# leopard-ai/betty

Measured on AMD Instinct MI355X. Metric: hypergradient-steps/sec (CG K=20, 10M inner params), higher is better.
Workload: dtype f32

## Files before the change

betty_amd/_native.py:

```python
from __future__ import annotations

import ctypes
import os
from ctypes import POINTER, c_char_p, c_double, c_float, c_int, c_int32, c_int64, c_size_t, c_void_p

_HERE = os.path.dirname(os.path.abspath(__file__))
LIB_PATH = os.environ.get("BHG_LIB") or os.path.join(_HERE, "csrc", "libbhg.so")
AB_LIB_PATH = os.environ.get("BHG_AB_LIB") or os.path.join(_HERE, "csrc", "libbhg_ab.so")

BHG_CHUNK_ELEMS = 4096
BHG_FLAT_ALIGN = 64
BHG_CG_AUTO, BHG_CG_STREAM, BHG_CG_RESIDENT = 0, 1, 2
BHG_CG_GLOBAL_CHAIN, BHG_CG_GLOBAL_UPDATE, BHG_CG_GLOBAL_DOTS = 0, 1, 2
BHG_CG_FX_BEGIN, BHG_CG_FX_CHAIN, BHG_CG_FX_GRAM, BHG_CG_FX_END = 0, 1, 2, 3


class NativeLibraryError(RuntimeError):
    """libbhg.so is missing or a call into it failed."""


class Chunk(ctypes.Structure):

    _fields_ = [
        ("flat_off", c_int64),
        ("src_off", c_int64),
        ("tensor", c_int32),
        ("len", c_int32),
    ]


BHG_MLP_MAX_LAYERS = 32


class Mlp(ctypes.Structure):

    _fields_ = [
        ("L", c_int32),
        ("B", c_int32),
        ("Bp", c_int32),
        ("dims", c_int32 * (BHG_MLP_MAX_LAYERS + 1)),
        ("W", c_void_p * BHG_MLP_MAX_LAYERS),
        ("h", c_void_p * BHG_MLP_MAX_LAYERS),
        ("mask", c_void_p * BHG_MLP_MAX_LAYERS),
        ("delta", c_void_p * BHG_MLP_MAX_LAYERS),
        ("prob", c_void_p),
        ("sd", c_void_p),
        ("Rh", c_void_p * BHG_MLP_MAX_LAYERS),
        ("Rd", c_void_p * BHG_MLP_MAX_LAYERS),
        ("partial", c_void_p),
        ("partial_floats", c_size_t),
        ("ridge2", c_float),
        ("prepacked", c_int32),
    ]


_PP = POINTER(c_void_p)
_CH = c_void_p

SYMBOLS = {
    "bhg_version": (c_int, []),
    "bhg_last_error": (c_char_p, []),
    "bhg_layout_flat_size": (c_int64, [POINTER(c_int64), c_int]),
    "bhg_layout_num_chunks": (c_int64, [POINTER(c_int64), c_int]),
    "bhg_layout_build": (c_int, [POINTER(c_int64), c_int, POINTER(c_int64), POINTER(Chunk)]),
    "bhg_workspace_bytes": (c_size_t, [c_int]),
    "bhg_flatten": (c_int, [_PP, c_int, _CH, c_int, c_void_p, c_float, c_void_p, c_void_p]),
    "bhg_scatter": (c_int, [c_void_p, _PP, c_int, _CH, c_int, c_float, c_void_p, c_void_p]),
    "bhg_neumann_init": (c_int, [_PP, c_int, _CH, c_int, c_void_p, c_void_p, c_void_p, c_void_p]),
    "bhg_neumann_step": (
        c_int,
        [_PP, c_int, _CH, c_int, c_void_p, c_void_p, c_float, c_float, c_float, c_void_p, c_void_p],
    ),
    "bhg_cg_init": (c_int, [_PP, c_int, _CH, c_int, c_void_p, c_void_p, c_void_p, c_void_p, c_void_p]),
    "bhg_cg_init_masked": (c_int, [_PP, c_int, _CH, c_int, c_void_p, c_void_p, c_void_p, ctypes.c_uint64, c_void_p, c_void_p]),
    "bhg_cg_step": (
        c_int,
        [_PP, c_int, _CH, c_int, c_void_p, c_void_p, c_void_p, c_float, c_int, c_float, c_float, c_int, c_void_p, c_void_p],
    ),
    "bhg_cg_phase": (
        c_int,
        [c_int, _PP, c_int, _CH, c_int, c_void_p, c_void_p, c_void_p, c_float, c_int, c_float, c_float, c_void_p, c_void_p],
    ),
    "bhg_cg_partials_dev": (c_void_p, [c_void_p, c_int, c_int]),
    "bhg_cg_partials_count": (c_int, []),
    "bhg_cg_resident_capacity_chunks": (c_int, []),
    "bhg_cg_resident_ok": (c_int, []),
    "bhg_cg_resident_usable": (c_int, [c_int]),
    "bhg_cg_scalars_dev": (c_void_p, [c_void_p]),
    "bhg_cg_timeout_flag_dev": (c_void_p, [c_void_p]),
    "bhg_scale_flat": (c_int, [c_void_p, c_int64, c_float, c_void_p]),
    "bhg_darts_eps": (c_int, [_PP, c_int, _CH, c_int, c_double, c_void_p, c_void_p, c_void_p, c_void_p]),
    "bhg_axpy_multi": (c_int, [_PP, _PP, c_int, _CH, c_int, c_void_p, c_float, c_void_p, c_void_p]),
    "bhg_fd_perturb": (c_int, [_PP, c_void_p, _PP, c_int, _CH, c_int, c_void_p, c_float, c_void_p, c_void_p]),
    "bhg_cg_step_fd": (
        c_int,
        [_PP, _PP, c_void_p, c_int, _CH, c_int, c_void_p, c_void_p, c_void_p, c_float, c_int, c_float, c_float, c_int, c_void_p, c_void_p],
    ),
    "bhg_neumann_step_fd": (
        c_int,
        [_PP, _PP, c_void_p, c_int, _CH, c_int, c_void_p, c_void_p, c_float, c_float, c_float, c_void_p, c_void_p],
    ),
    "bhg_sama_adam_precondition": (
        c_int,
        [_PP, _PP, _PP, _PP, c_int, _CH, c_int, c_void_p, c_double, c_double, c_double, c_double, c_void_p, c_void_p],
    ),
    "bhg_debug_set": (c_int, [c_char_p, c_int]),
    "bhg_debug_unset": (c_int, [c_char_p]),
    "bhg_debug_reset": (None, []),
    "bhg_debug_key_count": (c_int, []),
    "bhg_debug_key_name": (c_char_p, [c_int]),
    "bhg_is_ab_build": (c_int, []),
    "bhg_timing_enable": (c_int, [c_int]),
    "bhg_timing_read": (c_int, [c_int, POINTER(c_double), POINTER(c_int)]),
    "bhg_logreg_prepare": (c_int, [c_void_p, c_void_p, c_void_p, c_int, c_int, c_void_p]),
    "bhg_logreg_tmp_floats": (c_size_t, [c_int, c_int]),
    "bhg_logreg_hvp": (
        c_int,
        [c_void_p, c_void_p, c_void_p, c_void_p, c_void_p, c_void_p, c_int, c_int, c_void_p],
    ),
    "bhg_mlp_partial_floats": (c_size_t, [POINTER(Mlp)]),
    "bhg_mlp_hvp": (c_int, [POINTER(Mlp), _PP, _PP, c_void_p]),
    "bhg_mlp_hvp_mode": (c_int, [POINTER(Mlp), _PP, _PP, c_int, c_void_p]),
    "bhg_mlp_supports_native_prepare": (c_int, [POINTER(Mlp)]),
    "bhg_mlp_forward": (c_int, [POINTER(Mlp), _PP, c_void_p, c_void_p, c_void_p]),
    "bhg_mlp_backward": (c_int, [POINTER(Mlp), c_void_p, c_void_p]),
    "bhg_mlp_mixed_coeff": (c_int, [POINTER(Mlp), _PP, c_void_p, c_void_p, c_void_p]),
    "bhg_mlp_supports_fused_solve": (c_int, [POINTER(Mlp)]),
    "bhg_mlp_fused_ws_bytes": (c_size_t, [POINTER(Mlp)]),
    "bhg_mlp_cg_solve": (
        c_int,
        [POINTER(Mlp), c_void_p, c_void_p, c_void_p, POINTER(c_int64), _CH, c_int, c_int, c_float, c_float, c_void_p,
         c_void_p, c_size_t, c_void_p],
    ),
    "bhg_mlp_cg_state_mask": (ctypes.c_uint64, [POINTER(Mlp), c_int]),
    "bhg_mlp_cg_solve_rhs": (
        c_int,
        [POINTER(Mlp), c_void_p, c_void_p, c_void_p, POINTER(c_int64), _CH, c_int, c_int, c_float, c_float, c_void_p,
         c_void_p, c_size_t, _PP, c_void_p],
    ),
    "bhg_mlp_cg_global_phase": (
        c_int,
        [POINTER(Mlp), c_void_p, c_void_p, c_void_p, POINTER(c_int64), _CH, c_int, c_int, c_int, c_int, c_int, c_void_p, c_float,
         c_float, c_void_p, c_void_p, c_size_t, c_void_p],
    ),
    "bhg_mlp_fx_supported": (c_int, [POINTER(Mlp), c_int]),
    "bhg_mlp_fx_ws_bytes": (c_size_t, [POINTER(Mlp), c_int]),
    "bhg_mlp_fx_const_floats": (c_size_t, [POINTER(Mlp)]),
    "bhg_mlp_fx_slab_floats": (c_size_t, [POINTER(Mlp)]),
    "bhg_mlp_fx_scal_doubles": (c_size_t, [POINTER(Mlp)]),
    "bhg_mlp_cg_fx_phase": (
        c_int,
        [POINTER(Mlp), _PP, c_int, c_int, c_int, c_int, c_int, c_void_p, c_void_p, c_void_p, c_float, c_float, c_void_p, c_size_t,
         c_void_p, c_size_t, c_void_p],
    ),
    "bhg_mlp_neumann_fx_phase": (
        c_int,
        [POINTER(Mlp), _PP, c_int, c_int, c_int, c_int, c_int, c_void_p, c_void_p, c_void_p, c_float, c_float, c_void_p, c_size_t,
         c_void_p, c_size_t, c_void_p],
    ),
    "bhg_mlp_cg_mixed_coeff": (c_int, [POINTER(Mlp), c_void_p, c_void_p, c_float, c_void_p, c_size_t, c_void_p]),
    "bhg_mlp_timeout_flag_dev": (c_void_p, [POINTER(Mlp), c_void_p]),
    "bhg_mlp_stage_batch": (c_int, [POINTER(Mlp), c_void_p, c_void_p, c_void_p, c_void_p]),
    "bhg_mlp_supports_packed_prepare": (c_int, [POINTER(Mlp)]),
    "bhg_mlp_forward_packed": (c_int, [POINTER(Mlp), _PP, c_void_p, c_void_p, c_void_p, c_size_t, c_void_p]),
    "bhg_mlp_backward_packed": (c_int, [POINTER(Mlp), c_void_p, c_void_p, c_size_t, c_void_p]),
    "bhg_mwn_max_hidden": (c_int, []),
    "bhg_mlp_fd_ws_bytes": (c_size_t, [POINTER(c_int), c_int, c_int]),
    "bhg_mlp_fd_forward": (
        c_int,
        [c_void_p, c_void_p, c_int, POINTER(c_int), c_int, _PP, _PP, c_void_p, c_int, c_void_p, c_void_p, c_void_p, c_size_t, c_void_p],
    ),
    "bhg_mwn_fd_vjp": (
        c_int,
        [c_void_p, c_void_p, c_int, c_void_p, c_void_p, c_void_p, c_void_p, c_int, c_void_p, c_int, c_void_p, c_void_p, c_void_p, c_void_p,
         c_void_p],
    ),
    "bhg_quad_fd": (c_int, [_PP, _PP, _PP, c_int, _CH, c_int, c_void_p, c_float, c_int, c_int, c_int, c_void_p]),
    "bhg_mwn_forward": (c_int, [c_void_p, c_int, c_void_p, c_void_p, c_void_p, c_void_p, c_int, c_void_p, c_void_p, c_void_p]),
    "bhg_mwn_backward": (
        c_int,
        [c_void_p, c_void_p, c_int, c_void_p, c_void_p, c_void_p, c_void_p, c_int, c_float, c_void_p, c_void_p, c_void_p, c_void_p, c_void_p],
    ),
    "bhg_mlp_neumann_solve": (
        c_int,
        [POINTER(Mlp), c_void_p, c_void_p, c_void_p, POINTER(c_int64), c_int, c_float, c_float, c_void_p, c_size_t, POINTER(c_int), c_void_p],
    ),
    "bhg_mlp_wsk_launches": (c_int64, []),
    "bhg_mlp_hoist_launches": (c_int64, []),
    "bhg_mlp_proj_iterations": (c_int64, []),
    "bhg_mlp_lin_launches": (c_int64, []),
    "bhg_mlp_neumann_mixed_coeff": (c_int, [POINTER(Mlp), _PP, c_void_p, c_void_p, c_float, c_int, c_int, c_void_p, c_size_t, c_void_p]),
    "bhg_mlp_plan_describe": (c_int, [POINTER(Mlp), c_int, c_int, ctypes.c_char_p, c_size_t]),
    "bhg_copy2d": (c_int, [c_void_p, c_int64, c_void_p, c_int64, c_int64, c_int64, c_void_p]),
    "bhg_bn_ws_bytes": (c_size_t, [c_int]),
    "bhg_bn_backward_vjp": (
        c_int,
        [c_void_p, c_void_p, c_void_p, c_void_p, c_void_p, c_void_p, c_void_p, c_void_p, c_int, c_int, c_int, c_void_p, c_void_p, c_void_p,
         c_void_p, c_size_t, c_void_p],
    ),
}

_libs = {}
_current = [None]


_PY_ENV = {"BHG_LIB", "BHG_AB_LIB", "BHG_HVP_GRAPH", "BHG_ALL_RANKS_ON_GPU0"}
_warned_env = [False]


def _warn_legacy_env() -> None:
    if _warned_env[0]:
        return
    _warned_env[0] = True
    stale = sorted(k for k in os.environ if k.startswith("BHG_") and k not in _PY_ENV)
    if stale:
        import warnings

        warnings.warn("betty_amd: environment variable(s) " + ", ".join(stale) + " are IGNORED — libbhg reads no environment variable. "
                      "Measurement arms are selected with betty_amd._native.use_ab() + debug_set(key, int) (bench.py --debug KEY=INT) "
                      "on the measurement build libbhg_ab.so.", RuntimeWarning, stacklevel=3)


def _bind(path: str) -> ctypes.CDLL:
    lib = _libs.get(path)
    if lib is not None:
        return lib
    _warn_legacy_env()
    if not os.path.exists(path):
        raise NativeLibraryError(
            f"{path} not found: the HIP extension has not been built. Run "
            "`python -c 'import __graft_entry__ as g; g.build()'` or `make -C betty_amd/csrc`. "
            "betty_amd has no CPU fallback."
        )
    lib = ctypes.CDLL(path)
    for name, (restype, argtypes) in SYMBOLS.items():
        try:
            fn = getattr(lib, name)
        except AttributeError as exc:
            raise NativeLibraryError(f"{path} does not export {name}") from exc
        fn.restype = restype
        fn.argtypes = argtypes
    _libs[path] = lib
    return lib


def load() -> ctypes.CDLL:
    return _bind(_current[0] or LIB_PATH)


def current_lib_path() -> str:
    return _current[0] or LIB_PATH


def is_ab() -> bool:
    return bool(load().bhg_is_ab_build())


def use_ab(on: bool = True) -> None:
    if on:
        _bind(AB_LIB_PATH)
        _current[0] = AB_LIB_PATH
    else:
        _current[0] = None


def check(rc: int, what: str) -> None:
    if rc != 0:
        msg = load().bhg_last_error()
        raise NativeLibraryError(f"{what} failed with code {rc}: {msg.decode() if msg else ''}")


def _debug_key(key: str) -> bytes:
    k = key.strip()
    if k.upper().startswith("BHG_"):
        k = k[4:]
    return k.lower().encode()


def debug_set(key: str, value) -> None:
    lib = load()
    if value is not None and not lib.bhg_is_ab_build():
        raise NativeLibraryError(f"bhg_debug_set({key}): the product libbhg.so carries no measurement arm — call "
                                 "betty_amd._native.use_ab() first (libbhg_ab.so; the `bhg_debug` fixture and `bench.py --debug` do)")
    if value is None:
        check(lib.bhg_debug_unset(_debug_key(key)), f"bhg_debug_unset({key})")
    else:
        check(lib.bhg_debug_set(_debug_key(key), int(value)), f"bhg_debug_set({key})")


def debug_reset() -> None:
    load().bhg_debug_reset()


def debug_keys():
    lib = load()
    return [lib.bhg_debug_key_name(i).decode() for i in range(lib.bhg_debug_key_count())]


def ptr_array(ptrs):
    arr = (c_void_p * len(ptrs))(*ptrs)
    return ctypes.cast(arr, _PP), arr


def plan_describe(dims, B: int, algo: str = "cg", keep_solution: bool = False) -> dict:
    lib = load()
    d = Mlp()
    d.L, d.B, d.Bp = len(dims) - 1, int(B), (int(B) + 127) // 128 * 128
    for i, v in enumerate(dims):
        d.dims[i] = int(v)
    buf = ctypes.create_string_buffer(2048)
    check(lib.bhg_mlp_plan_describe(ctypes.byref(d), {"cg": 0, "neumann": 1}[algo], 1 if keep_solution else 0, buf, 2048), "bhg_mlp_plan_describe")
    out, text = {}, buf.value.decode()
    import re

    for key, quoted, plain in re.findall(r'(\w+)=(?:"([^"]*)"|(\S+))', text):
        val = quoted if quoted else plain
        out[key] = int(val) if re.fullmatch(r"-?\d+", val) else val
    return out
```

betty_amd/csrc/bhg_common.hpp:

```cpp
#pragma once
#include <hip/hip_runtime.h>
#include <stdint.h>
#include <stddef.h>
#include <stdio.h>
#include <string.h>

#include "bhg.h"

namespace bhg {

constexpr int kThreads = 256;
constexpr int kWaves = kThreads / 64;
constexpr int kChunk = BHG_CHUNK_ELEMS;
constexpr int kVecPerThread = kChunk / (kThreads * 4);
constexpr int kMaxBlocks = 1024;
constexpr int kInlineT = 32;
constexpr int kWriterT = 448;

constexpr size_t kWsScal = 0;
constexpr size_t kWsPartP = 128;
constexpr size_t kWsPartR = kWsPartP + 8 * kMaxBlocks;
constexpr size_t kWsBarrier = kWsPartR + 16 * kMaxBlocks;
constexpr size_t kWsTables = kWsBarrier + 256;
inline size_t ws_bytes(int T) {
  size_t b = kWsTables + 4 * sizeof(void*) * (size_t)(T > 0 ? T : 0);
  return (b + 255) & ~(size_t)255;
}

enum { S_RR_OLD = 0, S_PHP = 1, S_ALPHA = 2, S_RR_NEW = 3, S_BETA = 4, S_PP = 5 , S_ALPHA_RING = 10 ,
       S_NPART0 = 8  };

#define BHG_DBG_KEYS(X)                                                                                                      \
  X(mlp_wsk) X(mlp_wsk_maxk) X(mlp_wsk_depth) X(mlp_wsk_lds) X(wsl_depth) X(no_nt_slabs) X(gemm_no_xpose) X(mlp_no_fast)      \
  X(mlp_tn) X(split_target) X(split_cap) X(mlp_no_head) X(gram_ksplit) X(gram_kchunk) X(proj_graw_split) X(mlp_proj)         \
  X(mlp_hoist) X(hoist_wgs) X(proj_step_alone) X(mlp_no_side) X(mlp_no_fuse) X(mlp_no_outer_all) X(neumann_side)             \
  X(hoist_staged_mink) X(proj_alpha_alone) X(proj_small_alone) X(outer_order_by_work) X(outer_no_pre) X(outer_stagger)       \
  X(mlp_no_fused_solve) X(cg_eager_p) X(cg_x_every_iter) X(neumann_p_every_iter) X(head_no_prefetch) X(cg_spin_limit)        \
  X(packed_chain) X(packed_depth) X(packed_gram) X(proj_max_ratio) X(proj_ws_cap_mb) X(alpha_in_hoist) X(graw_v2) X(wskp_ragged) X(pstep_v2) X(pstep_unroll) X(rnew_in_graw) X(graw_cols) X(lin_first) X(lin_prio) X(lin_nub) X(lin_order) X(lin_update_next) X(lin_withhold_beta) X(neumann_vnew) X(cg_rhs_direct) X(packed_prepare) X(lin_deep) X(graw_kloop) X(lin_update_in_head) X(xcd_pairs) X(headu_head_first) X(fx_ksplit)
enum DbgKey : int {
#define BHG_DBG_ENUM(n) DBG_##n,
  BHG_DBG_KEYS(BHG_DBG_ENUM)
#undef BHG_DBG_ENUM
  DBG_COUNT
};
constexpr int kDbgUnset = INT32_MIN;
#ifdef BHG_AB
extern int g_dbg[DBG_COUNT];
inline bool dbg_is_set(DbgKey k) { return g_dbg[k] != kDbgUnset; }
inline int dbg(DbgKey k, int dflt) { return g_dbg[k] == kDbgUnset ? dflt : g_dbg[k]; }
#else
constexpr bool dbg_is_set(DbgKey) { return false; }
constexpr int dbg(DbgKey, int dflt) { return dflt; }
#endif

constexpr int kStampKernels = 4, kStampBlocks = 4096, kStampSlots = 8;
#ifdef BHG_STAMPS
#ifdef __HIPCC__
#define BHG_STAMP(kid, slot)                                                                                            \
  do {                                                                                                                  \
    if (threadIdx.x == 0 && blockIdx.x < ::bhg::kStampBlocks) {                                                         \
      unsigned long long* sp_ = ::bhg::d_stamps;                                                                        \
      if (sp_) sp_[((kid) * ::bhg::kStampBlocks + blockIdx.x) * ::bhg::kStampSlots + (slot)] = wall_clock64();          \
    }                                                                                                                   \
  } while (0)
#endif
#else
#define BHG_STAMP(kid, slot) do { } while (0)
#endif

void set_error(const char* fmt, ...);
#define BHG_HIP_CHECK(expr)                                                        \
  do {                                                                             \
    hipError_t _e = (expr);                                                        \
    if (_e != hipSuccess) {                                                        \
      ::bhg::set_error("%s failed: %s (%s:%d)", #expr, hipGetErrorString(_e), __FILE__, \
                       __LINE__);                                                  \
      return BHG_ERR_HIP;                                                          \
    }                                                                              \
  } while (0)
#define BHG_REQUIRE(cond, msg)                                                     \
  do {                                                                             \
    if (!(cond)) {                                                                 \
      ::bhg::set_error("%s: %s", __func__, msg);                                   \
      return BHG_ERR_ARG;                                                          \
    }                                                                              \
  } while (0)

struct PtrTab {
  const void* const* dev;
  const void* inl[kInlineT];
};

int make_table(PtrTab* out, const void* const* host_ptrs, int T, void* ws, int slot,
               hipStream_t stream);

bool span_begin(int kind, hipEvent_t* a, hipEvent_t* b);

#ifdef __HIPCC__
__device__ __forceinline__ float* tab_ptr(const PtrTab& t, int i) {
  const void* p = t.dev ? t.dev[i] : t.inl[i];
  return (float*)p;
}

__device__ __forceinline__ float4 ld4(const float* __restrict__ base, int e, int len) {
  if (e + 4 <= len) return *reinterpret_cast<const float4*>(base + e);
  float4 r = make_float4(0.f, 0.f, 0.f, 0.f);
  if (e < len) r.x = base[e];
  if (e + 1 < len) r.y = base[e + 1];
  if (e + 2 < len) r.z = base[e + 2];
  return r;
}
__device__ __forceinline__ void st4(float* __restrict__ base, int e, int len, float4 v) {
  if (e + 4 <= len) {
    *reinterpret_cast<float4*>(base + e) = v;
    return;
  }
  if (e < len) base[e] = v.x;
  if (e + 1 < len) base[e + 1] = v.y;
  if (e + 2 < len) base[e + 2] = v.z;
}

template <int BYTES>
__device__ __forceinline__ void kernarg_warm() {
  typedef const __attribute__((address_space(4))) unsigned* KP;
  KP kp = (KP)__builtin_amdgcn_kernarg_segment_ptr();
  unsigned acc = 0;
#pragma unroll
  for (int o = 0; o < BYTES; o += 64) acc |= kp[o / 4];
  asm volatile("" ::"s"(acc));
}
template <int U>
__device__ __forceinline__ double sum_strided(const double* __restrict__ p, const int n, const int t, const int stride) {
  double acc = 0.0;
  for (int i0 = t; i0 < n; i0 += U * stride) {
    double v[U];
#pragma unroll
    for (int u = 0; u < U; ++u) {
      const int i = i0 + u * stride;
      v[u] = p[i < n ? i : n - 1];
    }
#pragma unroll
    for (int u = 0; u < U; ++u)
      if (i0 + u * stride < n) acc += v[u];
  }
  return acc;
}

template <int U>
struct StridedRegs { double v[U]; };
template <int U>
__device__ __forceinline__ void strided_load(StridedRegs<U>& r, const double* __restrict__ p, const int n, const int t, const int stride,
                                             const double* __restrict__ dummy) {
  const double* q = (p && n > 0) ? p : dummy;
  const int last = (p && n > 0) ? n - 1 : 0;
#pragma unroll
  for (int u = 0; u < U; ++u) {
    const int i = t + u * stride;
    r.v[u] = q[i < n && i <= last ? i : last];
  }
}
template <int U>
__device__ __forceinline__ double strided_sum(const StridedRegs<U>& r, const int n, const int t, const int stride) {
  double acc = 0.0;
#pragma unroll
  for (int u = 0; u < U; ++u)
    if (t + u * stride < n) acc += r.v[u];
  return acc;
}

template <int CTRL>
__device__ __forceinline__ double dpp_mov_f64(const double v) {
  const unsigned long long u = __builtin_bit_cast(unsigned long long, v);
  const unsigned lo = (unsigned)__builtin_amdgcn_mov_dpp((int)(unsigned)u, CTRL, 0xf, 0xf, true);
  const unsigned hi = (unsigned)__builtin_amdgcn_mov_dpp((int)(unsigned)(u >> 32), CTRL, 0xf, 0xf, true);
  return __builtin_bit_cast(double, ((unsigned long long)hi << 32) | (unsigned long long)lo);
}
__device__ __forceinline__ double readlane_f64(const double v, const int lane) {
  const unsigned long long u = __builtin_bit_cast(unsigned long long, v);
  const unsigned lo = (unsigned)__builtin_amdgcn_readlane((int)(unsigned)u, lane);
  const unsigned hi = (unsigned)__builtin_amdgcn_readlane((int)(unsigned)(u >> 32), lane);
  return __builtin_bit_cast(double, ((unsigned long long)hi << 32) | (unsigned long long)lo);
}
__device__ __forceinline__ double wave_sum(double v) {
  v += dpp_mov_f64<0xB1>(v);
  v += dpp_mov_f64<0x4E>(v);
  v += dpp_mov_f64<0x141>(v);
  v += dpp_mov_f64<0x140>(v);
  const double r0 = readlane_f64(v, 0), r1 = readlane_f64(v, 16), r2 = readlane_f64(v, 32), r3 = readlane_f64(v, 48);
  return (r0 + r1) + (r2 + r3);
}
template <int CTRL>
__device__ __forceinline__ float dpp_mov_f32(const float v) {
  return __builtin_bit_cast(float, __builtin_amdgcn_mov_dpp(__builtin_bit_cast(int, v), CTRL, 0xf, 0xf, true));
}
__device__ __forceinline__ float wave_sum_f32(float v) {
  v += dpp_mov_f32<0xB1>(v);
  v += dpp_mov_f32<0x4E>(v);
  v += dpp_mov_f32<0x141>(v);
  v += dpp_mov_f32<0x140>(v);
  const float r0 = __builtin_bit_cast(float, __builtin_amdgcn_readlane(__builtin_bit_cast(int, v), 0));
  const float r1 = __builtin_bit_cast(float, __builtin_amdgcn_readlane(__builtin_bit_cast(int, v), 16));
  const float r2 = __builtin_bit_cast(float, __builtin_amdgcn_readlane(__builtin_bit_cast(int, v), 32));
  const float r3 = __builtin_bit_cast(float, __builtin_amdgcn_readlane(__builtin_bit_cast(int, v), 48));
  return (r0 + r1) + (r2 + r3);
}
__device__ __forceinline__ void block_sum3(double& a, double& b, double& c, double* red) {
  const double wa = wave_sum(a), wb = wave_sum(b), wc = wave_sum(c);
  const int lane = threadIdx.x & 63, w = threadIdx.x >> 6;
  __syncthreads();
  if (lane == 0) { red[w] = wa; red[kWaves + w] = wb; red[2 * kWaves + w] = wc; }
  __syncthreads();
  double sa = 0.0, sb = 0.0, sc = 0.0;
#pragma unroll
  for (int i = 0; i < kWaves; ++i) { sa += red[i]; sb += red[kWaves + i]; sc += red[2 * kWaves + i]; }
  a = sa; b = sb; c = sc;
}
__device__ __forceinline__ double block_sum(double v, double* red) {
  v = wave_sum(v);
  const int lane = threadIdx.x & 63, w = threadIdx.x >> 6;
  __syncthreads();
  if (lane == 0) red[w] = v;
  __syncthreads();
  double s = 0.0;
#pragma unroll
  for (int i = 0; i < kWaves; ++i) s += red[i];
  return s;
}
__device__ __forceinline__ double sum_partials(const double* __restrict__ part, int n,
                                               double* red) {
  double a = 0.0;
  for (int i = threadIdx.x; i < n; i += kThreads) a += part[i];
  return block_sum(a, red);
}
#endif

}
```

betty_amd/csrc/bhg_mlp.hip:

```cpp
#include <stdlib.h>
#include <vector>


#include "bhg_common.hpp"

#ifdef BHG_STAMPS
namespace bhg { __device__ unsigned long long* d_stamps = nullptr; }
#endif

namespace bhg {
namespace {
#include "mlp/gemm.inc"

#include "mlp/outer.inc"

#include "mlp/scalars.inc"

#include "mlp/head.inc"

#include "mlp/wsk.inc"

#include "mlp/wskp.inc"

inline int wsk_mode(int chain_mode, int unfused_hint) {
  if (dbg_is_set(DBG_mlp_wsk)) return dbg(DBG_mlp_wsk, 0);
  if (chain_mode == FUSE_CG) return 2;
  if (chain_mode == FUSE_NEUMANN) return 3;
  return unfused_hint;
}
inline bool wsk_wanted(int mode, int pairs, int K) {
  if (mode == 1) return true;
  if (mode != 2 && mode != 3) return false;
  return pairs * K <= dbg(DBG_mlp_wsk_maxk, 1024);
}
inline int wsk_depth() {
  const int d = dbg(DBG_mlp_wsk_depth, 3);
  return d == 2 ? 2 : 3;
}
inline bool wsk_eligible(const WskArgs& a) {
  if (a.pairs < 1 || a.pairs > 2) return false;
  bool ok = a.M % 32 == 0 && a.N % 32 == 0 && a.K % 32 == 0 && a.K >= 32;
  for (int i = 0; i < a.pairs; ++i) ok = ok && (a.pr[i].lda & 3) == 0 && (a.pr[i].ldb & 3) == 0;
  return ok;
}
int64_t g_wsk_launches = 0;
int64_t g_hoist_launches = 0;
int64_t g_proj_iterations = 0;
int64_t g_lin_launches = 0;
template <int LB>
void launch_gemm_wsk(const WskArgs& a_in, hipStream_t st, bool staged = false) {
  WskArgs a = a_in;
  ++g_wsk_launches;
  a.ntm = a.M / 32;
  a.ntn = a.N / 32;
  bool bf = false;
  for (int i = 0; i < a.pairs; ++i) bf = bf || a.pr[i].mix != 0;
  const dim3 grid(a.ntm * a.ntn), block(64 * kWskWaves);
  const int d = wsk_depth();
  const bool force_staged = dbg(DBG_mlp_wsk_lds, 0) != 0;
  if ((staged || force_staged) && !bf) {
    const int lds = (int)(sizeof(float) * kWslWaveFloats * kWskWaves);
    static bool attr_done = false;
    if (!attr_done) {
      (void)hipFuncSetAttribute(reinterpret_cast<const void*>(k_gemm_wsk<LB, false, 2, true>), hipFuncAttributeMaxDynamicSharedMemorySize, lds);
      attr_done = true;
    }
#ifdef BHG_AB
    const int wsl_depth = dbg(DBG_wsl_depth, 2);
    if (wsl_depth == 3) {
      static bool attr3 = false;
      if (!attr3) {
        (void)hipFuncSetAttribute(reinterpret_cast<const void*>(k_gemm_wsk<LB, false, 3, true>), hipFuncAttributeMaxDynamicSharedMemorySize, lds);
        attr3 = true;
      }
      hipLaunchKernelGGL((k_gemm_wsk<LB, false, 3, true>), grid, block, lds, st, a);
      return;
    }
#endif
    hipLaunchKernelGGL((k_gemm_wsk<LB, false, 2, true>), grid, block, lds, st, a);
    return;
  }
#define BHG_WSK(BFV, DV) hipLaunchKernelGGL((k_gemm_wsk<LB, BFV, DV>), grid, block, 0, st, a)
  if (bf) {
    if (d == 2 || LB == LAYOUT_RC) BHG_WSK(true, 2); else BHG_WSK(true, LB == LAYOUT_RC ? 2 : 3);
  } else {
#ifdef BHG_AB
    if (d == 2) BHG_WSK(false, 2); else
#endif
    BHG_WSK(false, 3);
  }
#undef BHG_WSK
}

#ifdef BHG_AB
void launch_wsk_group(const WskGroupArgs& g, int blocks, hipStream_t st) {
  const int lds = (int)(sizeof(float) * kWslWaveFloats * kWskWaves);
  static bool attr_done = false;
  if (!attr_done) {
    (void)hipFuncSetAttribute(reinterpret_cast<const void*>(k_wsk_group<2>), hipFuncAttributeMaxDynamicSharedMemorySize, lds);
#ifdef BHG_AB
    (void)hipFuncSetAttribute(reinterpret_cast<const void*>(k_wsk_group<3>), hipFuncAttributeMaxDynamicSharedMemorySize, lds);
#endif
    attr_done = true;
  }
#ifdef BHG_AB
  const int wsl_depth = dbg(DBG_wsl_depth, 2);
  if (wsl_depth == 3) { hipLaunchKernelGGL(k_wsk_group<3>, dim3(blocks), dim3(64 * kWskWaves), lds, st, g); return; }
#endif
  hipLaunchKernelGGL(k_wsk_group<2>, dim3(blocks), dim3(64 * kWskWaves), lds, st, g);
}
#endif

int chip_cus() {
  static int cus[64];
  int dev = 0;
  if (hipGetDevice(&dev) != hipSuccess || dev < 0 || dev >= 64) { (void)hipGetLastError(); return 256; }
  if (cus[dev] > 0) return cus[dev];
  int n = 0;
  if (hipDeviceGetAttribute(&n, hipDeviceAttributeMultiprocessorCount, dev) != hipSuccess || n <= 0) { (void)hipGetLastError(); n = 256; }
  return cus[dev] = n;
}
inline void wskp_tiling(WskpProb* q, bool ragged) {
  q->nfull = q->RA / 32;
  q->nstrip = 0;
  q->pairs = dbg(DBG_xcd_pairs, 1);
  if (!ragged || q->raw || q->nsplit != 1 || q->RB % 64 != 0) return;
  int nf = q->B / 32, rem = q->B % 32;
  if (rem > 16) { ++nf; rem = 0; }
  if (nf == 0) return;
  q->nfull = nf;
  q->nstrip = rem > 0 ? q->RB / 64 : 0;
}
struct WskpBuilder {
  WskpArgs g{};
  int blk = 0;
  bool add(const WskpProb& q_in) {
    if (g.n >= kWskpMax) return false;
    g.p[g.n++] = q_in;
    return true;
  }
  void tile(bool ragged) {
    blk = 0;
    for (int i = 0; i < g.n; ++i) {
      WskpProb& q = g.p[i];
      wskp_tiling(&q, ragged);
      g.blk0[i] = blk;
      blk += (((q.nfull * (q.RB / 32) + q.nstrip) * q.nsplit) + 7) & ~7;
    }
  }
  void launch(hipStream_t st) {
    if (!g.n) return;
    const int mode = dbg(DBG_wskp_ragged, 1);
    tile(mode == 2);
    if (mode == 1 && blk > chip_cus()) tile(true);
    g.blk0[g.n] = blk;
    const int d = dbg(DBG_packed_depth, 2);
    bool riders = g.n <= 3;
    for (int i = 1; i < g.n && riders; ++i) {
      const WskpProb& r = g.p[i];
      riders = r.raw && r.nsplit == 1 && r.RA == g.p[0].RA && r.RB == g.p[0].RA && r.B == g.p[0].B && !r.bias && !r.mask && !r.addend &&
               !r.partT2 && r.nstrip == 0 && r.nfull == r.RA / 32;
    }
    if (riders) {
      WskpcArgs c{};
      c.a = g.p[0];
      c.na = g.n >= 2 ? g.blk0[1] : blk;
      if (g.n >= 2) { c.r0 = {g.p[1].Ap, g.p[1].Bq, g.p[1].out, g.p[1].outp, g.p[1].K, 0}; c.nr0 = (g.n == 3 ? g.blk0[2] : blk) - g.blk0[1]; }
      if (g.n == 3) c.r1 = {g.p[2].Ap, g.p[2].Bq, g.p[2].out, g.p[2].outp, g.p[2].K, 0};
#ifdef BHG_AB
      if (d != 2) hipLaunchKernelGGL(k_wskpc<3>, dim3(blk), dim3(64 * kWskpWaves), 0, st, c); else
#endif
      hipLaunchKernelGGL(k_wskpc<2>, dim3(blk), dim3(64 * kWskpWaves), 0, st, c);
    } else {
#ifdef BHG_AB
      if (d != 2) hipLaunchKernelGGL(k_wskp<3>, dim3(blk), dim3(64 * kWskpWaves), 0, st, g); else
#endif
      hipLaunchKernelGGL(k_wskp<2>, dim3(blk), dim3(64 * kWskpWaves), 0, st, g);
    }
    (void)d;
    g = WskpArgs{};
    blk = 0;
  }
};

template <int LA, int LB>
void launch_gemm(const GemmArgs& a_in, int tn, hipStream_t st) {
  GemmArgs a = a_in;
  const bool nt_slabs = dbg(DBG_no_nt_slabs, 0) == 0;
  a.nt_out = (nt_slabs && (a.splits > 1 || a.out_rows > 0)) ? 1 : 0;
  const bool xpose = dbg(DBG_gemm_no_xpose, 0) == 0;
  a.xpose_out = xpose ? 1 : 0;
  dim3 grid((a.N + tn - 1) / tn, (a.M + kTM - 1) / kTM, a.splits);
  bool fast = a.M % kTM == 0 && a.N % tn == 0 && a.K % kTK == 0;
  bool bf = false;
  for (int i = 0; i < a.pairs; ++i) {
    fast = fast && (a.pr[i].lda & 3) == 0 && (a.pr[i].ldb & 3) == 0;
    bf = bf || a.pr[i].mix != 0;
  }
  if (bf)
    for (int i = 0; i < a.pairs; ++i)
      if (!a.pr[i].mix) a.pr[i].B2 = a.pr[i].B;
  const bool no_fast = dbg(DBG_mlp_no_fast, 0) != 0;
  if (no_fast) fast = false;
#define BHG_GEMM(TNV, F, BFV) hipLaunchKernelGGL((k_gemm<LA, LB, TNV, F, BFV>), grid, dim3(256), 0, st, a)
#ifdef BHG_AB
  if (tn == 64) {
    if (bf) { if (fast) BHG_GEMM(64, true, true); else BHG_GEMM(64, false, true); }
    else    { if (fast) BHG_GEMM(64, true, false); else BHG_GEMM(64, false, false); }
  } else
#endif
  {
    if (bf) { if (fast) BHG_GEMM(32, true, true); else BHG_GEMM(32, false, true); }
    else    { if (fast) BHG_GEMM(32, true, false); else BHG_GEMM(32, false, false); }
  }
#undef BHG_GEMM
}
inline int skinny_tile_n() {
  const int tn = dbg(DBG_mlp_tn, 32);
  return tn == 64 ? 64 : 32;
}

void launch_reduce_mask(hipStream_t st, const float* part, int splits, int slab, const float* bias,
                        const float* mask, float* out, int rows, int N, int B, float* relu_mask_out = nullptr,
                        float* outp = nullptr) {
  if ((N & 3) == 0) {
    int blocks = (slab / 4 + 255) / 256;
    if (blocks > 2048) blocks = 2048;
    hipLaunchKernelGGL(k_reduce_mask<4>, dim3(blocks), dim3(256), 0, st, part, splits, slab, bias, mask, out, rows, N, B,
                       relu_mask_out, outp);
  } else {
    int blocks = (slab + 255) / 256;
    if (blocks > 2048) blocks = 2048;
    hipLaunchKernelGGL(k_reduce_mask<1>, dim3(blocks), dim3(256), 0, st, part, splits, slab, bias, mask, out, rows, N, B,
                       relu_mask_out, (float*)nullptr);
  }
}

int pick_splits(int tiles, int K, int pairs) {
  const int ksteps = (K + kTK - 1) / kTK;
  const int target = dbg(DBG_split_target, 768);
  int s = (target + tiles - 1) / tiles;
  if (s > ksteps) s = ksteps;
  const int cap = dbg(DBG_split_cap, 16);
  if (s > cap) s = cap;
  if (s < 1) s = 1;
  if (ksteps % s != 0) {
    for (int d = 1; d <= 2; ++d) {
      if (s - d >= 1 && ksteps % (s - d) == 0) { s -= d; break; }
      if (s + d <= cap && s + d <= ksteps && ksteps % (s + d) == 0) { s += d; break; }
    }
  }
  return s;
}

#include "mlp/recurrence.inc"

#include "mlp/proj.inc"

#include "mlp/graw.inc"

#include "mlp/pstep.inc"
#include "mlp/wskpl.inc"
#include "mlp/headu.inc"

void launch_wskpu(const WskpProb& q_in, const PstepArgs& ps, int nu, hipStream_t st) {
  WskpuArgs u{};
  WskpProb q = q_in;
  const int mode = dbg(DBG_wskp_ragged, 1);
  wskp_tiling(&q, mode == 2);
  int blk = (((q.nfull * (q.RB / 32) + q.nstrip) * q.nsplit) + 7) & ~7;
  if (mode == 1 && blk > chip_cus()) {
    wskp_tiling(&q, true);
    blk = (((q.nfull * (q.RB / 32) + q.nstrip) * q.nsplit) + 7) & ~7;
  }
  u.c.a = q; u.c.na = blk;
  u.nu = nu; u.ps = ps;
  hipLaunchKernelGGL((k_wskpu<2, 4>), dim3(nu + blk), dim3(64 * kWskpWaves), 0, st, u);
}

struct SideState {
  hipStream_t side;
  hipEvent_t ev_rd[BHG_MLP_MAX_LAYERS];
  hipEvent_t ev_join;
};
int side_state(SideState** out) {
  static SideState per_device[64];
  int dev = 0;
  BHG_HIP_CHECK(hipGetDevice(&dev));
  BHG_REQUIRE(dev >= 0 && dev < 64, "device index out of range");
  SideState& ss = per_device[dev];
  if (!ss.side) {
    BHG_HIP_CHECK(hipStreamCreateWithFlags(&ss.side, hipStreamNonBlocking));
    const unsigned fl = hipEventDisableTiming | hipEventDisableSystemFence;
    for (int i = 0; i < BHG_MLP_MAX_LAYERS; ++i) BHG_HIP_CHECK(hipEventCreateWithFlags(&ss.ev_rd[i], fl));
    BHG_HIP_CHECK(hipEventCreateWithFlags(&ss.ev_join, fl));
#define BHG_OUTER_LDS(F, M) \
    BHG_HIP_CHECK(hipFuncSetAttribute(reinterpret_cast<const void*>(k_outer<F, M>), hipFuncAttributeMaxDynamicSharedMemorySize, 96 * 1024))
    BHG_OUTER_LDS(true, FUSE_NONE); BHG_OUTER_LDS(false, FUSE_NONE);
    BHG_OUTER_LDS(true, FUSE_CG); BHG_OUTER_LDS(false, FUSE_CG);
    BHG_OUTER_LDS(true, FUSE_NEUMANN); BHG_OUTER_LDS(false, FUSE_NEUMANN);
#undef BHG_OUTER_LDS
#ifdef BHG_AB
    BHG_HIP_CHECK(hipFuncSetAttribute(reinterpret_cast<const void*>(k_outer_all<FUSE_CG, false>), hipFuncAttributeMaxDynamicSharedMemorySize, 96 * 1024));
    BHG_HIP_CHECK(hipFuncSetAttribute(reinterpret_cast<const void*>(k_outer_all<FUSE_NEUMANN, false>), hipFuncAttributeMaxDynamicSharedMemorySize, 96 * 1024));
#endif
    BHG_HIP_CHECK(hipFuncSetAttribute(reinterpret_cast<const void*>(k_outer_all<FUSE_CG, true>), hipFuncAttributeMaxDynamicSharedMemorySize, 96 * 1024));
    BHG_HIP_CHECK(hipFuncSetAttribute(reinterpret_cast<const void*>(k_outer_all<FUSE_NEUMANN, true>), hipFuncAttributeMaxDynamicSharedMemorySize, 96 * 1024));
// ... 1265 lines not shown
  c->scal = reinterpret_cast<double*>(wsb + kWsScal);
  c->partR0 = reinterpret_cast<const double*>(wsb + kWsPartR);
  c->n_init = n_chunks < kMaxBlocks ? n_chunks : kMaxBlocks;
  for (int i = 0; i < 2 * m->L; ++i) c->dir[i] = p + starts[i];
  c->pgrid = n_chunks < kMaxBlocks ? n_chunks : kMaxBlocks;
  const bool eager = dbg(DBG_cg_eager_p, 0) != 0;
  c->lazy = global || !eager;
  BetaArgs& ba = c->ba;
  ba = BetaArgs{};
  int small_total = 0;
  {
    const bool head = use_head(m);
    ba.stride = c->w.nRR; ba.n = c->w.nRR; ba.scal = c->scal; ba.r = r; ba.p = p;
    for (int l = 0; l < m->L; ++l) {
      ba.off[ba.nt] = starts[2 * l + 1]; ba.len[ba.nt] = m->dims[l + 1]; small_total += ba.len[ba.nt]; ++ba.nt;
    }
    if (head) {
      ba.off[ba.nt] = starts[2 * (m->L - 1)]; ba.len[ba.nt] = m->dims[m->L] * m->dims[m->L - 1]; small_total += ba.len[ba.nt]; ++ba.nt;
    }
  }
  c->bgrid = small_total > 0 ? (small_total + kThreads - 1) / kThreads : 1;
  c->hplan.ok = false;
  if (c->lazy && hoist_mode() != 0) hoist_plan(m, &c->hplan);
  c->hoist = c->lazy && c->hplan.ok;
  c->proj_level = (!c->hoist || !c->hplan.proj_ok || proj_mode() == 0 || global) ? 0 : ((proj_mode() == 9 || x) ? 1 : 2);
  c->lin = c->proj_level == 2 && c->hplan.lin_ok && packed_chain_on(c->w) && dbg(DBG_packed_gram, 1) != 0 && dbg(DBG_graw_v2, 1) != 0 &&
           graw_batch_ok(m->Bp) && dbg(DBG_proj_small_alone, 0) == 0 && dbg(DBG_alpha_in_hoist, 1) != 0 && dbg(DBG_rnew_in_graw, 1) != 0 &&
           c->ba.nt <= 16 && proj_step_merged() && dbg(DBG_pstep_v2, 1) != 0 && dbg(DBG_lin_first, 1) != 0;
  c->lin_head = c->lin && m->L == 4 && dbg(DBG_lin_update_next, 1) != 0 && dbg(DBG_lin_update_in_head, 1) != 0 && dbg(DBG_lin_nub, 0) == 0 &&
                m->dims[m->L] <= 12 && m->dims[m->L - 1] <= 512 && dbg(DBG_head_no_prefetch, 0) == 0;
}
static int cg_iteration(CgCtx* c, int k, int gphase, double* php, double inv_world, hipStream_t st) {
  const bhg_mlp* m = c->m;
  FusedWs& w = c->w;
  const int K = c->K;
  const bool lazy = c->lazy, hoist = c->hoist;
  hipEvent_t ta, tb, tc, td;
  const bool timed = gphase == 0 && span_begin(BHG_TIMING_MLP_HVP, &ta, &tb);
  const bool timed_it = gphase == 0 && span_begin(BHG_TIMING_MLP_CG_ITER, &tc, &td);
  if (timed_it) BHG_HIP_CHECK(hipEventRecord(tc, st));
  if (lazy && k > 0 && gphase != 2) {
    c->ba.part = w.partRR[k & 1];
    if (!hoist || c->proj_level == 1) hipLaunchKernelGGL(k_cg_beta, dim3(c->bgrid), dim3(kThreads), 0, st, c->ba);
  }
  if (timed) BHG_HIP_CHECK(hipEventRecord(ta, st));
  ChainMode cm{};
  cm.mode = FUSE_CG;
  cm.fa = c->r; cm.fb = c->x; cm.fd = c->p; cm.starts = c->starts;
  cm.shift = c->shift; cm.cg_alpha = c->cg_alpha;
  cm.apply_out = k == K - 1; cm.out_scale = -c->cg_alpha;
  cm.ws = &w; cm.scal = c->scal;
  cm.partRR_old = c->partR0;
  cm.nRR_old = k == 0 ? c->n_init : 0;
  cm.partPP = k == 0 ? c->partR0 : w.partPP;
  cm.nPP = k == 0 ? c->n_init : (lazy ? 0 : c->pgrid);
  cm.partRR_new = w.partRR[(k + 1) & 1];
  cm.lazy = lazy;
  const bool x_every = dbg(DBG_cg_x_every_iter, 0) != 0;
  cm.x_mode = (lazy && !x_every) ? ((k & 1) ? 2 : (k + 1 < K ? 1 : 0)) : 0;
  if (!c->x) cm.x_mode = 1;
  cm.skip_outputs = (!c->x && k == K - 1) ? 1 : 0;
  cm.first = k == 0;
  cm.kpar = k & 1;
  cm.hoist = hoist ? &c->hplan : nullptr;
  cm.beta = &c->ba; cm.beta_blocks = c->bgrid;
  cm.proj = c->proj_level;
  cm.gphase = gphase; cm.php = php; cm.inv_world = inv_world;
  cm.second = k == 1;
  if (c->proj_level == 2 && proj_step_merged())
    c->dir[1] = k == 0 ? static_cast<const void*>(c->p + c->starts[1]) : static_cast<const void*>(w.pb0[k & 1]);
  if (c->lin) c->dir[3] = k == 0 ? static_cast<const void*>(c->p + c->starts[3]) : static_cast<const void*>(w.pb1[k & 1]);
  cm.lin = c->lin ? 1 : 0;
  cm.lin_head = c->lin_head ? 1 : 0;
  cm.rhs = c->rhs;
  if (int rc = run_chain(m, c->dir, cm, st)) return rc;
  if (timed) BHG_HIP_CHECK(hipEventRecord(tb, st));
#ifdef BHG_AB
  if (!lazy && k + 1 < K)
    hipLaunchKernelGGL(k_cg_pdir, dim3(c->pgrid), dim3(kThreads), 0, st, c->chunks_dev, c->n_chunks, (const float*)c->r, c->p,
                       (const double*)w.partRR[(k + 1) & 1], w.nRR, w.partPP, c->scal);
#endif
  if (timed_it) BHG_HIP_CHECK(hipEventRecord(td, st));
  return BHG_OK;
}

int bhg_mlp_cg_solve(const bhg_mlp* m, float* x, float* r, float* p, const int64_t* starts,
                     const bhg_chunk* chunks_dev, int n_chunks, int K, float cg_alpha, float hvp_shift, void* ws,
                     void* fws, size_t fws_bytes, void* stream) {
  return bhg_mlp_cg_solve_rhs(m, x, r, p, starts, chunks_dev, n_chunks, K, cg_alpha, hvp_shift, ws, fws, fws_bytes, nullptr, stream);
}

unsigned long long bhg_mlp_cg_state_mask(const bhg_mlp* m, int has_x) {
  if (!m || m->L < 1 || m->L > BHG_MLP_MAX_LAYERS || 2 * m->L > 64 || has_x || !bhg_mlp_supports_fused_solve(m)) return ~0ull;
  HoistPlan hp;
  hp.ok = false;
  if (dbg(DBG_cg_eager_p, 0) == 0 && hoist_mode() != 0) hoist_plan(m, &hp);
  const bool level2 = hp.ok && hp.proj_ok && proj_mode() != 0 && proj_mode() != 9;
  if (!level2 || dbg(DBG_cg_rhs_direct, 1) == 0) return ~0ull;
  unsigned long long mask = 0ull;
  for (int l = 0; l < m->L; ++l) mask |= 1ull << (2 * l + 1);
  mask |= 1ull << (2 * (m->L - 1));
  return mask;
}

int bhg_mlp_cg_solve_rhs(const bhg_mlp* m, float* x, float* r, float* p, const int64_t* starts,
                         const bhg_chunk* chunks_dev, int n_chunks, int K, float cg_alpha, float hvp_shift, void* ws,
                         void* fws, size_t fws_bytes, const void* const* rhs, void* stream) {
  if (int rc = solve_common_checks(m, starts, fws, fws_bytes)) return rc;
  BHG_REQUIRE(r && p && ws && chunks_dev, "NULL argument");
  BHG_REQUIRE(K >= 0 && n_chunks > 0, "bad size");
  if (K == 0) return BHG_OK;
  hipStream_t st = static_cast<hipStream_t>(stream);
  CgCtx c;
  cg_ctx_init(&c, m, x, r, p, starts, chunks_dev, n_chunks, K, cg_alpha, hvp_shift, ws, fws, false);
  BHG_REQUIRE(!rhs || c.proj_level == 2, "rhs names the right-hand side for the FULLY PROJECTED solver only (see bhg_mlp_cg_state_mask)");
  if (rhs)
    for (int l = 0; l + 1 < m->L; ++l) BHG_REQUIRE(rhs[2 * l] && ((uintptr_t)rhs[2 * l] & 15) == 0, "rhs tensors must be 16-byte aligned device pointers");
  c.rhs = rhs;
  if (c.hoist && packed_chain_on(c.w) && !m->prepacked)
    if (int rc = pack_operands(m, c.w, st)) return rc;
  for (int k = 0; k < K; ++k)
    if (int rc = cg_iteration(&c, k, 0, nullptr, 1.0, st)) return rc;
  BHG_HIP_CHECK(hipGetLastError());
  return BHG_OK;
}

int bhg_mlp_cg_global_phase(const bhg_mlp* m, float* x, float* r, float* p, const int64_t* starts, const bhg_chunk* chunks_dev,
                            int n_chunks, int k, int K, int phase, int world, double* php, float cg_alpha, float hvp_shift,
                            void* ws, void* fws, size_t fws_bytes, void* stream) {
  if (int rc = solve_common_checks(m, starts, fws, fws_bytes)) return rc;
  BHG_REQUIRE(r && p && ws && chunks_dev && php, "NULL argument");
  BHG_REQUIRE(K > 0 && k >= 0 && k < K && n_chunks > 0 && world >= 1, "bad size");
  BHG_REQUIRE(phase == BHG_CG_GLOBAL_CHAIN || phase == BHG_CG_GLOBAL_UPDATE || phase == BHG_CG_GLOBAL_DOTS, "unknown phase");
  hipStream_t st = static_cast<hipStream_t>(stream);
  CgCtx c;
  cg_ctx_init(&c, m, x, r, p, starts, chunks_dev, n_chunks, K, cg_alpha, hvp_shift, ws, fws, true);
  if (phase == BHG_CG_GLOBAL_DOTS) {
    BHG_REQUIRE(k + 1 < K, "the last iteration has no direction update");
    int grid = n_chunks < c.w.nRR ? n_chunks : c.w.nRR;
    if (grid > kMaxBlocks) grid = kMaxBlocks;
    hipLaunchKernelGGL(k_cg_global_dots, dim3(grid), dim3(kThreads), 0, st, chunks_dev, n_chunks, (const float*)r, (const float*)p,
                       c.w.partRR[(k + 1) & 1], c.w.nRR, c.w.nRR);
    BHG_HIP_CHECK(hipGetLastError());
    return BHG_OK;
  }
  if (k == 0 && phase == BHG_CG_GLOBAL_CHAIN && c.hoist && packed_chain_on(c.w) && !m->prepacked)
    if (int rc = pack_operands(m, c.w, st)) return rc;
  if (int rc = cg_iteration(&c, k, phase == BHG_CG_GLOBAL_CHAIN ? 1 : 2, php, 1.0 / (double)world, st)) return rc;
  BHG_HIP_CHECK(hipGetLastError());
  return BHG_OK;
}

int bhg_mlp_fx_supported(const bhg_mlp* m, int world) {
  if (!m || m->L < 1 || m->L > BHG_MLP_MAX_LAYERS || m->Bp <= 0 || m->Bp % kTM != 0 || !bhg_mlp_supports_fused_solve(m)) return 0;
  FxPlan fp;
  fx_plan(m, world, &fp);
  return fp.ok && dbg(DBG_packed_chain, 1) != 0 ? 1 : 0;
}
size_t bhg_mlp_fx_ws_bytes(const bhg_mlp* m, int world) {
  if (!bhg_mlp_fx_supported(m, world)) return 0;
  FxPlan fp; fx_plan(m, world, &fp);
  FxWs x; fx_carve(m, fp, nullptr, &x);
  return x.bytes;
}
size_t bhg_mlp_fx_const_floats(const bhg_mlp* m) {
  if (!bhg_mlp_fx_supported(m, 1)) return 0;
  FxPlan fp; fx_plan(m, 1, &fp);
  return fp.const_floats;
}
size_t bhg_mlp_fx_slab_floats(const bhg_mlp* m) {
  if (!bhg_mlp_fx_supported(m, 1)) return 0;
  FxPlan fp; fx_plan(m, 1, &fp);
  return fp.slab_floats;
}
size_t bhg_mlp_fx_scal_doubles(const bhg_mlp* m) {
  if (!bhg_mlp_fx_supported(m, 1)) return 0;
  FxPlan fp; fx_plan(m, 1, &fp);
  return fp.scal_doubles;
}
static int fx_phase(int algo, const bhg_mlp* m, const void* const* rhs, int k, int K, int phase, int world, int rank, float* const_all,
                    float* slab_all, double* scal_all, float alpha, float hvp_shift, void* fws, size_t fws_bytes, void* xws, size_t xws_bytes,
                    void* stream) {
  if (int rc = check_mlp(m)) return rc;
  const bool neumann = algo == 1;
  BHG_REQUIRE(world >= 1 && rank >= 0 && rank < world, "bad world size / rank");
  BHG_REQUIRE(bhg_mlp_fx_supported(m, world), "this network does not take the factor-exchange form (bhg_mlp_fx_supported)");
  BHG_REQUIRE(phase == BHG_CG_FX_BEGIN || phase == BHG_CG_FX_CHAIN || phase == BHG_CG_FX_GRAM || phase == BHG_CG_FX_END, "unknown phase");
  BHG_REQUIRE(K > 0 && k >= 0 && (k < K || (neumann && k == K && (phase == BHG_CG_FX_CHAIN || phase == BHG_CG_FX_END))), "bad iteration index");
  BHG_REQUIRE(const_all && slab_all && scal_all && fws && xws, "NULL argument");
  BHG_REQUIRE(m->partial && m->partial_floats >= bhg_mlp_partial_floats(m), "split-K scratch too small");
  BHG_REQUIRE(fws_bytes >= bhg_mlp_fused_ws_bytes(m), "fused workspace too small");
  BHG_REQUIRE(xws_bytes >= bhg_mlp_fx_ws_bytes(m, world), "factor-exchange workspace too small");
  hipStream_t st = static_cast<hipStream_t>(stream);
  FxPlan fp;
  fx_plan(m, world, &fp);
  FusedWs w;
  carve_fused_ws(m, fws, &w);
  FxWs x;
  fx_carve(m, fp, xws, &x);
  const bhg_mlp ml = fx_local(m, fp, slab_all, rank);
  double* scal_mine = scal_all + (size_t)rank * fp.scal_doubles;
  if (phase == BHG_CG_FX_BEGIN) {
    BHG_REQUIRE(k == 0, "BEGIN belongs to iteration 0");
    return fx_begin(m, fp, const_all, rank, st);
  }
  if (phase == BHG_CG_FX_CHAIN) {
    if (k == 0) {
      BHG_REQUIRE(rhs, "iteration 0 reads the right-hand side");
      for (int l = 0; l + 1 < m->L; ++l) BHG_REQUIRE(rhs[2 * l] && ((uintptr_t)rhs[2 * l] & 15) == 0, "rhs tensors must be 16-byte aligned device pointers");
      for (int i = 0; i < 2 * m->L; ++i) BHG_REQUIRE(rhs[i], "rhs holds 2 L device pointers");
      if (int rc = fx_first(m, &ml, fp, w, x, rhs, const_all, rank, st, neumann)) return rc;
    } else {
      if (int rc = fx_step(&ml, fp, w, x, scal_all, k - 1, false, alpha, hvp_shift, st, neumann)) return rc;
    }
    return fx_chain(&ml, fp, w, x, k & 1, st, neumann && k == K);
  }
  if (phase == BHG_CG_FX_GRAM) {
    BHG_REQUIRE(k < K, "GRAM belongs to iterations 0 .. K-1");
    return fx_gram(&ml, fp, w, x, slab_all, const_all, scal_mine, k & 1, hvp_shift, st);
  }
  BHG_REQUIRE(k == (neumann ? K : K - 1), "END belongs to the last iteration");
  return fx_step(&ml, fp, w, x, scal_all, k, true, alpha, hvp_shift, st, neumann);
}
int bhg_mlp_cg_fx_phase(const bhg_mlp* m, const void* const* rhs, int k, int K, int phase, int world, int rank, float* const_all,
                        float* slab_all, double* scal_all, float cg_alpha, float hvp_shift, void* fws, size_t fws_bytes, void* xws,
                        size_t xws_bytes, void* stream) {
  return fx_phase(0, m, rhs, k, K, phase, world, rank, const_all, slab_all, scal_all, cg_alpha, hvp_shift, fws, fws_bytes, xws, xws_bytes, stream);
}
int bhg_mlp_neumann_fx_phase(const bhg_mlp* m, const void* const* rhs, int k, int K, int phase, int world, int rank, float* const_all,
                             float* slab_all, double* scal_all, float alpha, float hvp_shift, void* fws, size_t fws_bytes, void* xws,
                             size_t xws_bytes, void* stream) {
  return fx_phase(1, m, rhs, k, K, phase, world, rank, const_all, slab_all, scal_all, alpha, hvp_shift, fws, fws_bytes, xws, xws_bytes, stream);
}

int bhg_mlp_neumann_solve(const bhg_mlp* m, float* v0, float* v1, float* p, const int64_t* starts, int K, float alpha,
                          float hvp_shift, void* fws, size_t fws_bytes, int* projected_out, void* stream) {
  if (int rc = solve_common_checks(m, starts, fws, fws_bytes)) return rc;
  BHG_REQUIRE(v0 && v1, "NULL argument");
  BHG_REQUIRE(K >= 0, "bad size");
  BHG_REQUIRE(p || use_head(m), "the accumulator-free Neumann solver needs the narrow-head kernels");
  hipStream_t st = static_cast<hipStream_t>(stream);
  FusedWs w;
  carve_fused_ws(m, fws, &w);
  HoistPlan hplan;
  hplan.ok = false;
  const bool want_proj = !p && K > 0 && proj_mode() != 0 && hoist_mode() != 0;
  if (hoist_mode() == 2 || want_proj) hoist_plan(m, &hplan);
  const bool proj = want_proj && hplan.ok && hplan.proj_ok && use_head(m);
  if (projected_out) *projected_out = proj ? 1 : 0;
  if (hplan.ok && K > 0 && packed_chain_on(w) && !m->prepacked)
    if (int rc = pack_operands(m, w, st)) return rc;
  for (int k = 0; k < K; ++k) {
    float* vin = (k & 1) ? v1 : v0;
    float* vout = (k & 1) ? v0 : v1;
    const void* dir[2 * BHG_MLP_MAX_LAYERS];
    for (int i = 0; i < 2 * m->L; ++i) dir[i] = vin + starts[i];
    hipEvent_t ta, tb;
    const bool timed = span_begin(BHG_TIMING_MLP_HVP, &ta, &tb);
    if (timed) BHG_HIP_CHECK(hipEventRecord(ta, st));
    ChainMode cm{};
    cm.mode = FUSE_NEUMANN;
    cm.fa = vout; cm.fb = p; cm.fd = vin; cm.starts = starts;
    cm.alpha = alpha; cm.shift = hvp_shift;
    cm.apply_out = k == K - 1; cm.out_scale = -alpha;
    const bool p_every = dbg(DBG_neumann_p_every_iter, 0) != 0;
    cm.x_mode = p_every ? 0 : ((k & 1) ? 2 : (k + 1 < K ? 1 : 0));
    cm.first = k == 0;
    if (!p) { cm.x_mode = 1; cm.rzx_acc = w.rzx; }
    cm.ws = &w;
    cm.hoist = hplan.ok ? &hplan : nullptr;
    cm.proj = proj ? 1 : 0;
    cm.nk = k;
    if (int rc = run_chain(m, dir, cm, st)) return rc;
    if (timed) BHG_HIP_CHECK(hipEventRecord(tb, st));
  }
  if (proj) {
    float* vin = (K & 1) ? v1 : v0;
    const void* dir[2 * BHG_MLP_MAX_LAYERS];
    for (int i = 0; i < 2 * m->L; ++i) dir[i] = vin + starts[i];
    ChainMode cm{};
    cm.mode = FUSE_NEUMANN;
    cm.fa = (K & 1) ? v0 : v1; cm.fb = nullptr; cm.fd = vin; cm.starts = starts;
    cm.alpha = alpha; cm.shift = hvp_shift;
    cm.x_mode = 1; cm.rzx_acc = w.rzx; cm.first = 0;
    cm.ws = &w; cm.hoist = &hplan; cm.proj = 1; cm.stop_after_head = 1; cm.nk = K;
    if (int rc = run_chain(m, dir, cm, st)) return rc;
  }
  return BHG_OK;
}

int bhg_mlp_cg_mixed_coeff(const bhg_mlp* m, const int64_t* labels, float* coeff, float cg_alpha, void* fws,
                           size_t fws_bytes, void* stream) {
  if (int rc = check_mlp(m)) return rc;
  BHG_REQUIRE(labels && coeff && fws, "NULL argument");
  BHG_REQUIRE(fws_bytes >= bhg_mlp_fused_ws_bytes(m), "fused workspace too small");
  FusedWs w;
  carve_fused_ws(m, fws, &w);
  hipLaunchKernelGGL(k_coeff_from_rzx, dim3((m->Bp + kThreads - 1) / kThreads), dim3(kThreads), 0, static_cast<hipStream_t>(stream),
                     (const double*)w.rzx, m->prob, labels, coeff, m->Bp, m->dims[m->L], m->B, -cg_alpha, 0.f);
  BHG_HIP_CHECK(hipGetLastError());
  return BHG_OK;
}

static int check_head_problem(const bhg_mlp* m) {
  BHG_REQUIRE(m, "NULL descriptor");
  BHG_REQUIRE(m->L >= 1 && m->L <= BHG_MLP_MAX_LAYERS, "unsupported layer count");
  BHG_REQUIRE(m->Bp > 0 && m->Bp % kTM == 0 && m->B >= 1 && m->B <= m->Bp, "Bp must be a multiple of 128 rows >= B");
  BHG_REQUIRE(m->partial && m->partial_floats >= bhg_mlp_partial_floats(m), "split-K scratch too small");
  return BHG_OK;
}
static bool narrow_head(const bhg_mlp* m) { return m->dims[m->L] <= kSmallC && (m->dims[m->L - 1] & 3) == 0; }

int bhg_mlp_supports_native_prepare(const bhg_mlp* m) {
  return m && m->L >= 1 && m->L <= BHG_MLP_MAX_LAYERS && m->Bp > 0 && m->Bp % kTM == 0;
}

}
namespace bhg {
namespace {
__global__ __launch_bounds__(kThreads) void k_softmax_ce_rows(float* __restrict__ z, const int64_t* __restrict__ labels,
                                                              float* __restrict__ ce, int C, int B) {
  __shared__ double red[kWaves];
  __shared__ float redf[kWaves];
  const int b = blockIdx.x, t = threadIdx.x;
  float* row = z + (int64_t)b * C;
  if (b >= B) {
    for (int c = t; c < C; c += kThreads) row[c] = 0.f;
    if (t == 0) ce[b] = 0.f;
    return;
  }
  float mx = -INFINITY;
  for (int c = t; c < C; c += kThreads) mx = fmaxf(mx, row[c]);
  for (int o = 32; o > 0; o >>= 1) mx = fmaxf(mx, __shfl_xor(mx, o));
  if ((t & 63) == 0) redf[t >> 6] = mx;
  __syncthreads();
  mx = redf[0];
  for (int w = 1; w < kWaves; ++w) mx = fmaxf(mx, redf[w]);
  double s = 0.0;
  for (int c = t; c < C; c += kThreads) s += (double)expf(row[c] - mx);
  s = block_sum(s, red);
  const float lse = mx + logf((float)s);
  const float zy = row[(int)labels[b]];
  __syncthreads();
  for (int c = t; c < C; c += kThreads) row[c] = expf(row[c] - lse);
  if (t == 0) ce[b] = lse - zy;
}
__global__ __launch_bounds__(kThreads) void k_coeff_rows(const float* __restrict__ prob, const float* __restrict__ rz,
                                                         const int64_t* __restrict__ labels, float* __restrict__ coeff, int C, int B) {
  __shared__ double red[kWaves];
  const int b = blockIdx.x, t = threadIdx.x;
  if (b >= B) { if (t == 0) coeff[b] = 0.f; return; }
  const int y = (int)labels[b];
  double s = 0.0;
  for (int c = t; c < C; c += kThreads) s += (double)((prob[(int64_t)b * C + c] - (c == y ? 1.f : 0.f)) * rz[(int64_t)b * C + c]);
  s = block_sum(s, red);
  if (t == 0) coeff[b] = (float)(s / (double)B);
}
}
}
using namespace bhg;
extern "C" {

int bhg_mlp_forward(const bhg_mlp* m, const void* const* bias, const int64_t* labels, float* ce, void* stream) {
  if (int rc = check_head_problem(m)) return rc;
  BHG_REQUIRE(bias && labels && ce, "NULL argument");
  hipStream_t st = static_cast<hipStream_t>(stream);
  const int L = m->L, Bp = m->Bp, B = m->B;
  for (int l = 0; l < L; ++l) {
    const int K = m->dims[l], N = m->dims[l + 1];
    const float* b = static_cast<const float*>(bias[l]);
    if (l == L - 1 && narrow_head(m)) {
      launch_head_forward(st, Bp, nullptr, m->h[l], m->W[l] , m->W[l], b, nullptr, nullptr,
                          const_cast<float*>(m->prob), K, N, B, HEAD_LOGITS, labels, ce, nullptr, nullptr, nullptr);
      break;
    }
    GemmArgs a{};
    a.pr[0] = {m->h[l], m->W[l], K, K};
    a.pairs = 1;
    a.M = Bp; a.N = N; a.K = K;
    const int tn = skinny_tile_n();
    a.splits = pick_splits((N + tn - 1) / tn, K, 1);
    a.out = m->partial; a.ldo = N; a.out_rows = Bp;
    launch_gemm<LAYOUT_KC, LAYOUT_KC>(a, tn, st);
    if (l == L - 1) {
      launch_reduce_mask(st, m->partial, a.splits, Bp * N, b, nullptr, const_cast<float*>(m->prob), Bp, N, B);
      hipLaunchKernelGGL(k_softmax_ce_rows, dim3(Bp), dim3(kThreads), 0, st, const_cast<float*>(m->prob), labels, ce, N, B);
      break;
    }
    launch_reduce_mask(st, m->partial, a.splits, Bp * N, b, nullptr, const_cast<float*>(m->h[l + 1]), Bp, N, B,
                       const_cast<float*>(m->mask[l]));
  }
  BHG_HIP_CHECK(hipGetLastError());
  return BHG_OK;
}

int bhg_mlp_backward(const bhg_mlp* m, const int64_t* labels, void* stream) {
  if (int rc = check_head_problem(m)) return rc;
  BHG_REQUIRE(labels, "NULL argument");
  hipStream_t st = static_cast<hipStream_t>(stream);
  const int L = m->L, Bp = m->Bp, B = m->B;
  const int C = m->dims[L];
  hipLaunchKernelGGL(k_delta_top, dim3((Bp * C + 255) / 256), dim3(256), 0, st, m->prob, m->sd, labels,
                     const_cast<float*>(m->delta[L - 1]), Bp, C, B);
  for (int l = L - 1; l >= 1; --l) {
    const int K = m->dims[l + 1], N = m->dims[l];
    if (l == L - 1 && narrow_head(m)) {
      const int blocks = (Bp * (N / 4) + 255) / 256;
      hipLaunchKernelGGL(k_head_backward, dim3(blocks), dim3(256), 0, st, (const float*)nullptr, m->delta[l], m->W[l],
                         (const float*)nullptr, m->mask[l - 1], const_cast<float*>(m->delta[l - 1]), N, K, B, Bp);
      continue;
    }
    GemmArgs a{};
    a.pr[0] = {m->delta[l], m->W[l], K, N};
    a.pairs = 1;
    a.M = Bp; a.N = N; a.K = K;
    const int tn = skinny_tile_n();
    a.splits = pick_splits((N + tn - 1) / tn, K, 1);
    a.out = m->partial; a.ldo = N; a.out_rows = Bp;
    launch_gemm<LAYOUT_KC, LAYOUT_RC>(a, tn, st);
    launch_reduce_mask(st, m->partial, a.splits, Bp * N, nullptr, m->mask[l - 1], const_cast<float*>(m->delta[l - 1]), Bp,
                       N, B);
  }
  BHG_HIP_CHECK(hipGetLastError());
  return BHG_OK;
}

int bhg_mlp_supports_packed_prepare(const bhg_mlp* m) {
  if (!bhg_mlp_supports_native_prepare(m) || !bhg_mlp_supports_fused_solve(m) || dbg(DBG_packed_prepare, 1) == 0) return 0;
  HoistPlan hp;
  hoist_plan(m, &hp);
  return hp.ok && dbg(DBG_packed_chain, 1) != 0 ? 1 : 0;
}

int bhg_mlp_forward_packed(const bhg_mlp* m, const void* const* bias, const int64_t* labels, float* ce, void* fws, size_t fws_bytes,
                           void* stream) {
  if (int rc = check_head_problem(m)) return rc;
  BHG_REQUIRE(narrow_head(m), "the packed once-per-step passes need a narrow classifier head (<= 256 classes, feature width % 4 == 0)");
  BHG_REQUIRE(bias && labels && ce && fws, "NULL argument");
  BHG_REQUIRE(bhg_mlp_supports_packed_prepare(m), "this network does not take the packed form (bhg_mlp_supports_packed_prepare)");
  BHG_REQUIRE(fws_bytes >= bhg_mlp_fused_ws_bytes(m), "fused workspace too small");
  hipStream_t st = static_cast<hipStream_t>(stream);
  const int L = m->L, Bp = m->Bp, B = m->B;
  FusedWs w;
  carve_fused_ws(m, fws, &w);
  if (int rc = pack_operands(m, w, st, true)) return rc;
  {
    const int K = m->dims[0], N = m->dims[1];
    GemmArgs a{};
    a.pr[0] = {m->h[0], m->W[0], K, K};
    a.pairs = 1;
    a.M = Bp; a.N = N; a.K = K;
    const int tn = skinny_tile_n();
    a.splits = pick_splits((N + tn - 1) / tn, K, 1);
    a.out = m->partial; a.ldo = N; a.out_rows = Bp;
    launch_gemm<LAYOUT_KC, LAYOUT_KC>(a, tn, st);
    launch_reduce_mask(st, m->partial, a.splits, Bp * N, static_cast<const float*>(bias[0]), nullptr, const_cast<float*>(m->h[1]), Bp, N, B,
                       const_cast<float*>(m->mask[0]), w.hpk[1]);
  }
  for (int l = 1; l + 1 < L; ++l) {
    WskpfArgs f{};
    WskpProb& q = f.a;
    q.Ap = w.hpk[l]; q.Bq = w.Wf[l]; q.RA = Bp; q.RB = m->dims[l + 1]; q.K = m->dims[l]; q.B = B; q.nsplit = 1;
    q.bias = static_cast<const float*>(bias[l]);
    q.out = const_cast<float*>(m->h[l + 1]);
    q.outp = l + 2 < L ? w.hpk[l + 1] : nullptr;
    f.relu_mask = const_cast<float*>(m->mask[l]);
    wskp_tiling(&q, false);
    const int blk = q.nfull * (q.RB / 32) + q.nstrip;
    hipLaunchKernelGGL(k_wskpf<2>, dim3(blk), dim3(64 * kWskpWaves), 0, st, f);
  }
  launch_head_forward(st, Bp, nullptr, m->h[L - 1], m->W[L - 1] , m->W[L - 1], static_cast<const float*>(bias[L - 1]),
                      nullptr, nullptr, const_cast<float*>(m->prob), m->dims[L - 1], m->dims[L], B, HEAD_LOGITS, labels, ce, nullptr,
                      nullptr, nullptr);
  BHG_HIP_CHECK(hipGetLastError());
  return BHG_OK;
}

int bhg_mlp_backward_packed(const bhg_mlp* m, const int64_t* labels, void* fws, size_t fws_bytes, void* stream) {
  if (int rc = check_head_problem(m)) return rc;
  BHG_REQUIRE(narrow_head(m), "the packed once-per-step passes need a narrow classifier head (<= 256 classes, feature width % 4 == 0)");
  BHG_REQUIRE(labels && fws, "NULL argument");
  BHG_REQUIRE(bhg_mlp_supports_packed_prepare(m), "this network does not take the packed form (bhg_mlp_supports_packed_prepare)");
  BHG_REQUIRE(fws_bytes >= bhg_mlp_fused_ws_bytes(m), "fused workspace too small");
  hipStream_t st = static_cast<hipStream_t>(stream);
  const int L = m->L, Bp = m->Bp, B = m->B;
  const int C = m->dims[L];
  FusedWs w;
  carve_fused_ws(m, fws, &w);
  hipLaunchKernelGGL(k_delta_top, dim3((Bp * C + 255) / 256), dim3(256), 0, st, m->prob, m->sd, labels,
                     const_cast<float*>(m->delta[L - 1]), Bp, C, B);
  {
    const int l = L - 1, K = m->dims[l + 1], N = m->dims[l];
    const int blocks = (Bp * (N / 4) + 255) / 256;
    hipLaunchKernelGGL(k_head_backward, dim3(blocks), dim3(256), 0, st, (const float*)nullptr, m->delta[l], m->W[l],
                       (const float*)nullptr, m->mask[l - 1], const_cast<float*>(m->delta[l - 1]), N, K, B, Bp, w.dpk[l - 1]);
  }
  for (int l = L - 2; l >= 1; --l) {
    WskpBuilder wb;
    WskpProb q{};
    q.Ap = w.dpk[l]; q.Bq = w.Wb[l]; q.RA = Bp; q.RB = m->dims[l]; q.K = m->dims[l + 1]; q.B = B; q.nsplit = 1;
    q.mask = m->mask[l - 1]; q.out = const_cast<float*>(m->delta[l - 1]);
    q.outp = l >= 2 ? w.dpk[l - 1] : nullptr;
    wb.add(q);
    wb.launch(st);
  }
  BHG_HIP_CHECK(hipGetLastError());
  return BHG_OK;
}

__global__ __launch_bounds__(256) void k_stage_batch(const float* __restrict__ x, const int64_t* __restrict__ y, float* __restrict__ h0,
                                                     int64_t* __restrict__ labels, int64_t n4, int B) {
  for (int64_t i = (int64_t)blockIdx.x * 256 + threadIdx.x; i < n4; i += (int64_t)gridDim.x * 256)
    reinterpret_cast<float4*>(h0)[i] = reinterpret_cast<const float4*>(x)[i];
  if (blockIdx.x == 0)
    for (int b = threadIdx.x; b < B; b += 256) labels[b] = y[b];
}
int bhg_mlp_stage_batch(const bhg_mlp* m, const float* x, const int64_t* y, int64_t* labels, void* stream) {
  if (int rc = check_mlp(m)) return rc;
  BHG_REQUIRE(x && y && labels && m->h[0], "NULL argument");
  BHG_REQUIRE((m->dims[0] & 3) == 0 && ((uintptr_t)x & 15) == 0, "the input batch must be 16-byte aligned with a width that is a multiple of 4");
  const int64_t n4 = (int64_t)m->B * m->dims[0] / 4;
  int blocks = (int)((n4 + 255) / 256);
  if (blocks > 2048) blocks = 2048;
  if (blocks < 1) blocks = 1;
  hipLaunchKernelGGL(k_stage_batch, dim3(blocks), dim3(256), 0, static_cast<hipStream_t>(stream), x, y, const_cast<float*>(m->h[0]), labels, n4, m->B);
  BHG_HIP_CHECK(hipGetLastError());
  return BHG_OK;
}

int bhg_mlp_mixed_coeff(const bhg_mlp* m, const void* const* dir, const int64_t* labels, float* coeff, void* stream) {
  if (int rc = check_head_problem(m)) return rc;
  BHG_REQUIRE(dir && labels && coeff, "NULL argument");
  hipStream_t st = static_cast<hipStream_t>(stream);
  const int L = m->L, Bp = m->Bp, B = m->B;
  for (int l = 0; l < L; ++l) {
    const int K = m->dims[l], N = m->dims[l + 1];
    const float* V = static_cast<const float*>(dir[2 * l]);
    const float* c = static_cast<const float*>(dir[2 * l + 1]);
    if (l == L - 1 && narrow_head(m)) {
      launch_head_forward(st, Bp, l > 0 ? (const float*)m->Rh[l - 1] : nullptr, m->h[l], m->W[l], V, c, m->prob, nullptr,
                          nullptr, K, N, B, HEAD_COEFF, labels, coeff, nullptr, nullptr, nullptr);
      break;
    }
    GemmArgs a{};
    a.pr[0] = {m->h[l], V, K, K};
    a.pairs = 1;
    if (l > 0) { a.pr[1] = {m->Rh[l - 1], m->W[l], K, K}; a.pairs = 2; }
    a.M = Bp; a.N = N; a.K = K;
    const int tn = skinny_tile_n();
    a.splits = pick_splits((N + tn - 1) / tn, K, a.pairs);
    a.out = m->partial; a.ldo = N; a.out_rows = Bp;
    launch_gemm<LAYOUT_KC, LAYOUT_KC>(a, tn, st);
    if (l == L - 1) {
      launch_reduce_mask(st, m->partial, a.splits, Bp * N, c, nullptr, m->Rd[l], Bp, N, B);
      hipLaunchKernelGGL(k_coeff_rows, dim3(Bp), dim3(kThreads), 0, st, m->prob, (const float*)m->Rd[l], labels, coeff, N, B);
      break;
    }
    launch_reduce_mask(st, m->partial, a.splits, Bp * N, c, m->mask[l], m->Rh[l], Bp, N, B);
  }
  BHG_HIP_CHECK(hipGetLastError());
  return BHG_OK;
}

int bhg_mlp_plan_describe(const bhg_mlp* m, int algo, int keep_solution, char* buf, size_t buf_bytes) {
  if (int rc = check_mlp(m)) return rc;
  BHG_REQUIRE(buf && buf_bytes >= 64, "output buffer too small");
  BHG_REQUIRE(algo == 0 || algo == 1, "algo: 0 = cg, 1 = neumann");
  const int L = m->L;
  const bool fused = bhg_mlp_supports_fused_solve(m) != 0;
  HoistPlan hp;
  hoist_plan(m, &hp);
  const char* form = "unfused";
  int hoist = 0, proj_level = 0, lin = 0, lin_head = 0, upd_first = 0;
  const char* closing = "k_outer_all";
  if (fused) {
    int64_t numel[2 * BHG_MLP_MAX_LAYERS], starts[2 * BHG_MLP_MAX_LAYERS];
    for (int l = 0; l < L; ++l) { numel[2 * l] = (int64_t)m->dims[l] * m->dims[l + 1]; numel[2 * l + 1] = m->dims[l + 1]; }
    const int64_t nch = bhg_layout_num_chunks(numel, 2 * L);
    std::vector<bhg_chunk> chunks((size_t)(nch > 0 ? nch : 1));
    if (int rc = bhg_layout_build(numel, 2 * L, starts, chunks.data())) return rc;
    float* const fake = reinterpret_cast<float*>((uintptr_t)1 << 30);
    if (algo == 0) {
      static CgCtx c;
      cg_ctx_init(&c, m, keep_solution ? fake : nullptr, fake, fake, starts, nullptr, (int)nch, 2, 1.f, 0.f, fake, fake, false);
      hoist = c.hoist ? 1 : 0; proj_level = c.proj_level; lin = c.lin ? 1 : 0; lin_head = c.lin_head ? 1 : 0;
      upd_first = (c.lin && L > 4) ? 1 : 0;
      form = !c.lazy ? "classic-eager" : (!c.hoist ? "classic" : (c.proj_level == 0 ? "hoisted" : (c.proj_level == 1 ? "projected-keep-state" :
             (c.lin ? (c.lin_head ? "six-launch (k_wskpl .. k_headu .. k_graw)" : "six-launch-class (k_wskpl first, recurrences beside the chain)") :
              "fully-projected (k_pstep launch)"))));
      if (c.proj_level >= 1) closing = graw_batch_ok(m->Bp) ? (m->Bp == 128 ? "k_graw" : "k_grawk") : "k_hoist+k_proj_update";
    } else {
      const bool want_proj = !keep_solution && proj_mode() != 0 && hoist_mode() != 0;
      const bool proj = want_proj && hp.ok && hp.proj_ok && use_head(m);
      hoist = (hp.ok && (hoist_mode() == 2 || want_proj)) ? 1 : 0;
      proj_level = proj ? 1 : 0;
      form = proj ? "projected-neumann (update inside k_graw)" : (hoist ? "hoisted" : "classic");
      if (proj) closing = graw_batch_ok(m->Bp) ? (m->Bp == 128 ? "k_graw" : "k_grawk") : "k_hoist+k_proj_update";
    }
  }
  size_t gram = 0;
  if (hp.ok && hp.proj_ok)
    for (int l = 0; l + 1 < L; ++l) gram += (size_t)m->Bp * m->Bp * (l >= 1 ? (2 + 2 * kGramSplitMax + 6) : 2);
  const int n = snprintf(buf, buf_bytes,
                         "algo=%s keep_solution=%d fused=%d form=\"%s\" hoist=%d proj_level=%d lin=%d lin_head=%d upd_first=%d closing=%s "
                         "plan_ok=%d proj_ok=%d lin_ok=%d hoist_products=%d hoist_wgs=%d gram_floats=%zu fused_ws_bytes=%zu narrow_head=%d packed_prepare=%d "
                         "global_form=%s fx_slab_bytes=%zu fx_ws_bytes_world8=%zu",
                         algo == 0 ? "cg" : "neumann", keep_solution ? 1 : 0, fused ? 1 : 0, form, hoist, proj_level, lin, lin_head, upd_first, closing,
                         hp.ok ? 1 : 0, hp.proj_ok ? 1 : 0, hp.lin_ok ? 1 : 0, hp.n, hp.ok ? hp.blk0[hp.n] : 0, gram,
                         fused ? bhg_mlp_fused_ws_bytes(m) : (size_t)0, narrow_head(m) ? 1 : 0, bhg_mlp_supports_packed_prepare(m),
                         (algo == 0 && !keep_solution && bhg_mlp_fx_supported(m, 1)) ? "factor-exchange" : (fused ? "one-pass" : "sharded"),
                         sizeof(float) * bhg_mlp_fx_slab_floats(m), bhg_mlp_fx_ws_bytes(m, 8));
  BHG_REQUIRE(n > 0 && (size_t)n < buf_bytes, "output buffer too small");
  return BHG_OK;
}

#ifdef BHG_STAMPS
static unsigned long long* g_stamps_dev = nullptr;
int bhg_debug_stamps_enable(int on) {
  const size_t bytes = sizeof(unsigned long long) * bhg::kStampKernels * bhg::kStampBlocks * bhg::kStampSlots;
  if (on && !g_stamps_dev) {
    BHG_HIP_CHECK(hipMalloc(&g_stamps_dev, bytes));
  }
  if (g_stamps_dev) BHG_HIP_CHECK(hipMemset(g_stamps_dev, 0, bytes));
  unsigned long long* p = on ? g_stamps_dev : nullptr;
  BHG_HIP_CHECK(hipMemcpyToSymbol(HIP_SYMBOL(bhg::d_stamps), &p, sizeof(p)));
  return BHG_OK;
}
int bhg_debug_stamps_read(unsigned long long* host, size_t count) {
  BHG_REQUIRE(g_stamps_dev && host, "stamps are not enabled");
  const size_t total = (size_t)bhg::kStampKernels * bhg::kStampBlocks * bhg::kStampSlots;
  BHG_HIP_CHECK(hipDeviceSynchronize());
  BHG_HIP_CHECK(hipMemcpy(host, g_stamps_dev, sizeof(unsigned long long) * (count < total ? count : total), hipMemcpyDeviceToHost));
  return BHG_OK;
}
#endif

}

#ifndef BHG_LAYOUT_PAD
#define BHG_LAYOUT_PAD 8
#endif
namespace bhg {
namespace {
#define BHG_STR2(x) #x
#define BHG_STR(x) BHG_STR2(x)
__global__ __attribute__((aligned(16384))) void k_layout_anchor() {
#if BHG_LAYOUT_PAD > 0
  asm volatile(".rept " BHG_STR(BHG_LAYOUT_PAD) " * 64 - 8\n s_nop 0\n .endr");
#endif
}
}
}
```

betty_amd/csrc/bhg_mwn.hip:

```cpp
#include "bhg_common.hpp"

namespace bhg {
namespace {

constexpr int kMwnMaxH = 2048;
constexpr int kMwnChunk = 1024;

__device__ __forceinline__ float mwn_sigmoid(float z) { return 1.f / (1.f + expf(-z)); }

__global__ __launch_bounds__(kThreads) void k_mwn_forward(const float* __restrict__ ce, int B, const float* __restrict__ w1,
                                                          const float* __restrict__ b1, const float* __restrict__ w2,
                                                          const float* __restrict__ b2, int H, float* __restrict__ s,
                                                          float* __restrict__ sd) {
  extern __shared__ float sp[];
  for (int j = threadIdx.x; j < H; j += kThreads) { sp[j] = w1[j]; sp[H + j] = b1[j]; sp[2 * H + j] = w2[j]; }
  __syncthreads();
  const int i = blockIdx.x * kThreads + threadIdx.x;
  if (i >= B) return;
  const float c = ce[i];
  float z = b2[0];
  for (int j = 0; j < H; ++j) {
    const float a = fmaf(sp[j], c, sp[H + j]);
    z = fmaf(sp[2 * H + j], a > 0.f ? a : 0.f, z);
  }
  const float v = mwn_sigmoid(z);
  if (s) s[i] = v;
  if (sd) sd[i] = v / (float)B;
}

__global__ __launch_bounds__(kThreads) void k_mwn_backward(const float* __restrict__ ce, const float* __restrict__ coeff, int B,
                                                           const float* __restrict__ w1, const float* __restrict__ b1,
                                                           const float* __restrict__ w2, const float* __restrict__ b2, int H,
                                                           float scale, float* __restrict__ gw1, float* __restrict__ gb1,
                                                           float* __restrict__ gw2, float* __restrict__ gb2) {
  extern __shared__ float sp[];
  __shared__ float red[kWaves];
  float* sdz = sp + 3 * H;
  float* sce = sdz + kMwnChunk;
  for (int j = threadIdx.x; j < H; j += kThreads) { sp[j] = w1[j]; sp[H + j] = b1[j]; sp[2 * H + j] = w2[j]; }
  const float bias2 = b2[0];
  constexpr int kPer = kMwnMaxH / kThreads;
  float a_w1[kPer], a_b1[kPer], a_w2[kPer];
#pragma unroll
  for (int u = 0; u < kPer; ++u) a_w1[u] = a_b1[u] = a_w2[u] = 0.f;
  float a_b2 = 0.f;
  constexpr int kSPer = kMwnChunk / kThreads;
  float c_pre[kSPer], k_pre[kSPer];
#pragma unroll
  for (int u = 0; u < kSPer; ++u) {
    const int t = threadIdx.x + kThreads * u;
    c_pre[u] = ce[t < B ? t : 0];
    k_pre[u] = coeff[t < B ? t : 0];
  }
  __syncthreads();
  for (int i0 = 0; i0 < B; i0 += kMwnChunk) {
    const int n = B - i0 < kMwnChunk ? B - i0 : kMwnChunk;
#pragma unroll
    for (int u = 0; u < kSPer; ++u) {
      const int t = threadIdx.x + kThreads * u;
      if (t >= n) continue;
      const float c = i0 == 0 ? c_pre[u] : ce[i0 + t];
      const float kc = i0 == 0 ? k_pre[u] : coeff[i0 + t];
      float z = bias2;
      for (int j = 0; j < H; ++j) {
        const float a = fmaf(sp[j], c, sp[H + j]);
        z = fmaf(sp[2 * H + j], a > 0.f ? a : 0.f, z);
      }
      const float v = mwn_sigmoid(z);
      const float dz = kc * (v * (1.f - v));
      sdz[t] = dz;
      sce[t] = c;
      a_b2 += dz;
    }
    __syncthreads();
#pragma unroll
    for (int u = 0; u < kPer; ++u) {
      const int j = threadIdx.x + kThreads * u;
      if (j < H) {
        const float wj = sp[j], bj = sp[H + j], vj = sp[2 * H + j];
        for (int t = 0; t < n; ++t) {
          const float c = sce[t], dz = sdz[t];
          const float a = fmaf(wj, c, bj);
          const bool on = a > 0.f;
          a_w2[u] = fmaf(dz, on ? a : 0.f, a_w2[u]);
          const float g1 = on ? dz * vj : 0.f;
          a_b1[u] += g1;
          a_w1[u] = fmaf(g1, c, a_w1[u]);
        }
      }
    }
    __syncthreads();
  }
#pragma unroll
  for (int u = 0; u < kPer; ++u) {
    const int j = threadIdx.x + kThreads * u;
    if (j < H) { gw1[j] = scale * a_w1[u]; gb1[j] = scale * a_b1[u]; gw2[j] = scale * a_w2[u]; }
  }
#pragma unroll
  for (int off = 32; off > 0; off >>= 1) a_b2 += __shfl_down(a_b2, off, 64);
  if ((threadIdx.x & 63) == 0) red[threadIdx.x >> 6] = a_b2;
  __syncthreads();
  if (threadIdx.x == 0) gb2[0] = scale * ((red[0] + red[1]) + (red[2] + red[3]));
}

int check_mwn(const float* ce, int B, const float* w1, const float* b1, const float* w2, const float* b2, int H) {
  BHG_REQUIRE(ce && w1 && b1 && w2 && b2, "NULL argument");
  BHG_REQUIRE(B >= 1 && H >= 1 && H <= kMwnMaxH, "the closed-form meta-weight-net takes 1 <= hidden width <= 2048");
  return BHG_OK;
}

}
}

using namespace bhg;

extern "C" {

int bhg_mwn_max_hidden(void) { return kMwnMaxH; }

int bhg_mwn_forward(const float* ce, int B, const float* w1, const float* b1, const float* w2, const float* b2, int H, float* s,
                    float* sd, void* stream) {
  if (int rc = check_mwn(ce, B, w1, b1, w2, b2, H)) return rc;
  BHG_REQUIRE(s || sd, "no output requested");
  hipLaunchKernelGGL(k_mwn_forward, dim3((B + kThreads - 1) / kThreads), dim3(kThreads), sizeof(float) * 3 * (size_t)H,
                     static_cast<hipStream_t>(stream), ce, B, w1, b1, w2, b2, H, s, sd);
  BHG_HIP_CHECK(hipGetLastError());
  return BHG_OK;
}

int bhg_mwn_backward(const float* ce, const float* coeff, int B, const float* w1, const float* b1, const float* w2, const float* b2,
                     int H, float scale, float* gw1, float* gb1, float* gw2, float* gb2, void* stream) {
  if (int rc = check_mwn(ce, B, w1, b1, w2, b2, H)) return rc;
  BHG_REQUIRE(coeff && gw1 && gb1 && gw2 && gb2, "NULL argument");
  hipLaunchKernelGGL(k_mwn_backward, dim3(1), dim3(kThreads), sizeof(float) * (3 * (size_t)H + 2 * kMwnChunk),
                     static_cast<hipStream_t>(stream), ce, coeff, B, w1, b1, w2, b2, H, scale, gw1, gb1, gw2, gb2);
  BHG_HIP_CHECK(hipGetLastError());
  return BHG_OK;
}

}
```

betty_amd/hypergradient/_mlp_hip.py:

```python
from __future__ import annotations

import ctypes
import weakref

import torch

from .. import _native

TILE_M = 128

_BUFFERS = weakref.WeakKeyDictionary()



class _Buffers:

    def __init__(self, dims, BP, device, lib):
        L = len(dims) - 1
        self.BP = BP
        self.dims, self.L = dims, L
        z = lambda *shape: torch.zeros(*shape, dtype=torch.float32, device=device)
        self.h = [z(BP, dims[l]) for l in range(L)]
        self.mask = [z(BP, dims[l + 1]) for l in range(L - 1)]
        self.delta = [z(BP, dims[l + 1]) for l in range(L)]
        self.prob = z(BP, dims[L])
        self.sd = z(BP)
        self.ce = z(BP)
        self.coeff = z(BP)
        self.labels = torch.zeros(BP, dtype=torch.int64, device=device)
        self.Rh = [z(BP, dims[l + 1]) for l in range(L - 1)]
        self.Rd = [z(BP, dims[l + 1]) for l in range(L)]
        d = _native.Mlp()
        d.L, d.Bp = L, BP
        for i, v in enumerate(dims):
            d.dims[i] = v
        for l in range(L):
            d.h[l] = self.h[l].data_ptr()
            d.delta[l] = self.delta[l].data_ptr()
            d.Rd[l] = self.Rd[l].data_ptr()
            if l + 1 < L:
                d.mask[l] = self.mask[l].data_ptr()
                d.Rh[l] = self.Rh[l].data_ptr()
        d.prob, d.sd = self.prob.data_ptr(), self.sd.data_ptr()
        d.ridge2 = 0.0
        d.B = 1
        n_part = int(lib.bhg_mlp_partial_floats(ctypes.byref(d)))
        self.partial = torch.empty(max(n_part, 1), dtype=torch.float32, device=device)
        d.partial, d.partial_floats = self.partial.data_ptr(), n_part
        self.desc = d
        self.out = None
        self.native_prepare = bool(lib.bhg_mlp_supports_native_prepare(ctypes.byref(d)))


def _stream() -> int:
    return int(torch.cuda.current_stream().cuda_stream)


def _native_weight_net(lib, wn, upper, device):
    if wn is None:
        return None
    slots = wn.slots(list(upper))
    ts = [t.detach() for t in wn.tensors()]
    if (slots is None or ts[0].shape[0] > int(lib.bhg_mwn_max_hidden())
            or not all(t.is_cuda and t.device == device and t.dtype == torch.float32 and t.is_contiguous() for t in ts)):
        return None
    return ts, slots


def _flat_upper(upper, slots, device):
    sizes = [p.numel() for p in upper]
    flat = torch.empty(sum(sizes), dtype=torch.float32, device=device)
    views, off = [], 0
    for p, n in zip(upper, sizes):
        views.append(flat[off: off + n].view(p.shape))
        off += n
    return flat, views, [views[i] for i in slots]


class FusedSolve:

    __slots__ = ("kind", "alpha", "K", "layout", "v_last", "materialised", "projected")

    def __init__(self, kind, alpha, K, layout, v_last=None, materialised=True, projected=0):
        self.kind, self.alpha, self.K, self.layout, self.v_last, self.materialised = kind, alpha, K, layout, v_last, materialised
        self.projected = projected

    def __bool__(self):
        return True


class HipMLPState:
    def __init__(self, spec, x, y):
        if not x.is_cuda:
            raise _native.NativeLibraryError("WeightedCEMLP(impl='hip') needs CUDA/HIP tensors; there is no CPU fallback")
        self.lib = lib = _native.load()
        self.spec = spec
        Ws = [lin.weight.detach() for lin in spec.layers]
        bs = [lin.bias.detach() for lin in spec.layers]
        L, B = len(Ws), x.shape[0]
        BP = (B + TILE_M - 1) // TILE_M * TILE_M
        if L > _native.BHG_MLP_MAX_LAYERS:
            raise ValueError("too many layers")
        for t in Ws + bs:
            if t.dtype != torch.float32 or not t.is_contiguous() or t.data_ptr() % 16 != 0:
                raise ValueError("weights and biases must be contiguous, 16-byte aligned fp32 tensors")
        dims = tuple([Ws[0].shape[1]] + [W.shape[0] for W in Ws])
        key = (dims, BP, str(x.device))
        owner = _BUFFERS.setdefault(spec.layers[0], {})
        buf = owner.get(key)
        if buf is None:
            buf = owner[key] = _Buffers(dims, BP, x.device, lib)
        self.buf, self.B, self.L, self.Ws = buf, B, L, Ws
        d = buf.desc
        d.B = B
        for l in range(L):
            d.W[l] = Ws[l].data_ptr()
        self.desc = d
        if getattr(buf, "last_B", B) > B:
            buf.h[0][B:].zero_()
        buf.last_B = B
        xs, ys = x.detach().reshape(B, -1), y.detach().reshape(-1)
        same_dev = (xs.device == buf.h[0].device and ys.device == xs.device and xs.is_cuda
                    and torch.cuda.current_device() == (xs.device.index if xs.device.index is not None else torch.cuda.current_device()))
        if (same_dev and xs.dtype == torch.float32 and xs.is_contiguous() and xs.data_ptr() % 16 == 0 and dims[0] % 4 == 0
                and ys.dtype == torch.int64 and ys.is_contiguous()):
            _native.check(lib.bhg_mlp_stage_batch(ctypes.byref(d), xs.data_ptr(), ys.data_ptr(), buf.labels.data_ptr(), _stream()),
                          "bhg_mlp_stage_batch")
        else:
            buf.h[0][:B].copy_(xs.to(torch.float32))
            buf.labels[:B].copy_(ys)

        d.prepacked = 0
        self.packed_prepare = bool(buf.native_prepare and lib.bhg_mlp_supports_packed_prepare(ctypes.byref(d)))
        if self.packed_prepare:
            fws = self._fused_ws(x.device)
            bias_tab, self._bias_keep = _native.ptr_array([b.data_ptr() for b in bs])
            _native.check(lib.bhg_mlp_forward_packed(ctypes.byref(d), bias_tab, buf.labels.data_ptr(), buf.ce.data_ptr(), fws.data_ptr(),
                                                     fws.numel(), _stream()), "bhg_mlp_forward_packed")
            ce = buf.ce[:B]
        elif buf.native_prepare:
            bias_tab, self._bias_keep = _native.ptr_array([b.data_ptr() for b in bs])
            _native.check(lib.bhg_mlp_forward(ctypes.byref(d), bias_tab, buf.labels.data_ptr(), buf.ce.data_ptr(), _stream()),
                          "bhg_mlp_forward")
            ce = buf.ce[:B]
        else:
            raise _native.NativeLibraryError("bhg_mlp_supports_native_prepare refused this network (layer count / batch padding): there is no ATen path")
        native = _native_weight_net(lib, spec.weight_net, spec.prev.trainable_parameters(), x.device)
        self.native_upper, self.sample_weight = native is not None, None
        if self.native_upper:
            self._wn, self._upper_slots = native
            ts = self._wn
            _native.check(lib.bhg_mwn_forward(buf.ce.data_ptr(), B, ts[0].data_ptr(), ts[1].data_ptr(), ts[2].data_ptr(), ts[3].data_ptr(),
                                              ts[0].shape[0], None, buf.sd.data_ptr(), _stream()), "bhg_mwn_forward")
        else:
            self.sample_weight = spec.weight_fn(ce.detach().clone())
            buf.sd[:B].copy_(self.sample_weight.detach().reshape(-1).to(torch.float32) / B)
        if self.packed_prepare:
            _native.check(lib.bhg_mlp_backward_packed(ctypes.byref(d), buf.labels.data_ptr(), buf.fws.data_ptr(), buf.fws.numel(), _stream()),
                          "bhg_mlp_backward_packed")
            d.prepacked = 1
        else:
            _native.check(lib.bhg_mlp_backward(ctypes.byref(d), buf.labels.data_ptr(), _stream()), "bhg_mlp_backward")
        if buf.out is None:
            buf.out = []
            for lin in spec.layers:
                buf.out += [torch.empty_like(lin.weight), torch.empty_like(lin.bias)]
            buf.out_tab, buf.out_keep = _native.ptr_array([t.data_ptr() for t in buf.out])
        self.out = buf.out
        self._out_tab = buf.out_tab

    def upper_vjp(self, coeff, upper, scale: float = 1.0, retain_graph: bool = False, with_flat: bool = False):
        if not self.native_upper:
            sw = self.sample_weight
            out = list(torch.autograd.grad(sw, upper, grad_outputs=coeff.reshape(sw.shape), retain_graph=retain_graph, allow_unused=retain_graph))
            return (out, None) if with_flat else out
        ts, B = self._wn, self.B
        H = ts[0].shape[0]
        flat, views, g = _flat_upper(upper, self._upper_slots, ts[0].device)
        coeff = coeff if (coeff.dtype == torch.float32 and coeff.is_contiguous()) else coeff.to(torch.float32).contiguous()
        _native.check(
            self.lib.bhg_mwn_backward(self.buf.ce.data_ptr(), coeff.data_ptr(), B, ts[0].data_ptr(), ts[1].data_ptr(), ts[2].data_ptr(),
                                      ts[3].data_ptr(), H, float(scale), g[0].data_ptr(), g[1].data_ptr(), g[2].data_ptr(),
                                      g[3].data_ptr(), _stream()), "bhg_mwn_backward")
        return (views, flat) if with_flat else views

    @staticmethod
    def _dir_table(direction_views):
        dirs = []
        for t in direction_views:
            if not (t.is_cuda and t.dtype == torch.float32 and t.is_contiguous() and t.data_ptr() % 16 == 0):
                t = t.detach().to(torch.float32).contiguous().clone()
            dirs.append(t)
        tab, keep = _native.ptr_array([t.data_ptr() for t in dirs])
        return tab, (dirs, keep)

    def hvp(self, direction_views):
        self._solve = None
        key = tuple(map(id, direction_views))
        cached = getattr(self, "_dir_cache", None)
        if cached is None or cached[0] != key:
            tab, keep = self._dir_table(direction_views)
            cached = (key, tab, keep, list(direction_views))
            self._dir_cache = cached if all(a is b for a, b in zip(keep[0], direction_views)) else None
        mode = 3 if getattr(getattr(self.spec.curr, "config", None), "type", None) == "neumann" else 0
        _native.check(self.lib.bhg_mlp_hvp_mode(ctypes.byref(self.desc), cached[1], self._out_tab, mode, _stream()), "bhg_mlp_hvp_mode")
        return self.out

    def fused_supported(self, layout) -> bool:
        if not self.lib.bhg_mlp_supports_fused_solve(ctypes.byref(self.desc)):
            return False
        want = []
        for W in self.Ws:
            want += [W.numel(), W.shape[0]]
        return tuple(want) == tuple(layout.numels) and str(layout.device) == str(self.Ws[0].device)

    def _fused_ws(self, device):
        buf = self.buf
        if getattr(buf, "fws", None) is None:
            n = int(self.lib.bhg_mlp_fused_ws_bytes(ctypes.byref(self.desc)))
            buf.fws = torch.zeros(max(n, 256), dtype=torch.uint8, device=device)
            addr = self.lib.bhg_mlp_timeout_flag_dev(ctypes.byref(self.desc), buf.fws.data_ptr())
            if addr:
                off = int(addr) - buf.fws.data_ptr()
                buf.fws_flag = buf.fws[off: off + 4].view(torch.int32)
                from ..backend import get_backend

                get_backend().watch_fused_workspace(buf.fws_flag)
        return buf.fws

    def _fused_args(self, layout):
        fws = self._fused_ws(layout.device)
        starts = (ctypes.c_int64 * len(layout.starts))(*layout.starts)
        return fws, starts

    def cg_state_mask(self):
        mask = int(self.lib.bhg_mlp_cg_state_mask(ctypes.byref(self.desc), 0))
        return None if mask == (1 << 64) - 1 else mask

    def cg_solve(self, layout, x, r, p, K: int, cg_alpha: float, shift: float, keep_x: bool = True, rhs=None) -> FusedSolve:
        fws, starts = self._fused_args(layout)
        rhs_tab, _rhs_keep = (None, None) if rhs is None else _native.ptr_array([t.data_ptr() for t in rhs])
        _native.check(
            self.lib.bhg_mlp_cg_solve_rhs(ctypes.byref(self.desc), x.data_ptr() if keep_x else None, r.data_ptr(), p.data_ptr(), starts,
                                          layout.chunks_dev.data_ptr(), layout.n_chunks, int(K), float(cg_alpha), float(shift),
                                          layout.workspace.data_ptr(), fws.data_ptr(), fws.numel(), rhs_tab, _stream()),
            "bhg_mlp_cg_solve_rhs",
        )
        self._rhs_keep = (rhs, _rhs_keep)
        self._solve = FusedSolve("cg", float(cg_alpha), int(K), layout, materialised=keep_x)
        return self._solve

    solution_free = True

    def cg_global_phase(self, layout, x, r, p, k: int, K: int, phase: int, world: int, php, cg_alpha: float, shift: float,
                        keep_x: bool = True) -> None:
        fws, starts = self._fused_args(layout)
        if k == 0 and phase == _native.BHG_CG_GLOBAL_CHAIN:
            self._solve = None
        _native.check(
            self.lib.bhg_mlp_cg_global_phase(ctypes.byref(self.desc), x.data_ptr() if keep_x else None, r.data_ptr(), p.data_ptr(),
                                             starts, layout.chunks_dev.data_ptr(), layout.n_chunks, int(k), int(K), int(phase),
                                             int(world), php.data_ptr(), float(cg_alpha), float(shift),
                                             layout.workspace.data_ptr(), fws.data_ptr(), fws.numel(), _stream()),
            "bhg_mlp_cg_global_phase",
        )

    def cg_global_finish(self, layout, K: int, cg_alpha: float, keep_x: bool = True) -> FusedSolve:
        self._solve = FusedSolve("cg", float(cg_alpha), int(K), layout, materialised=keep_x)
        return self._solve

    def fx_supported(self, layout, world: int) -> bool:
        return bool(self.fused_supported(layout) and self.lib.bhg_mlp_fx_supported(ctypes.byref(self.desc), int(world)))

    def fx_buffers(self, world: int):
        buf = self.buf
        held = getattr(buf, "fx", None)
        if held is None:
            held = buf.fx = {}
        got = held.get(world)
        if got is None:
            d, lib, dev = ctypes.byref(self.desc), self.lib, buf.h[0].device
            z = lambda n, dt: torch.zeros(int(n), dtype=dt, device=dev)
            got = held[world] = {
                "const": z(world * lib.bhg_mlp_fx_const_floats(d), torch.float32).view(world, -1),
                "slab": z(world * lib.bhg_mlp_fx_slab_floats(d), torch.float32).view(world, -1),
                "scal": z(world * lib.bhg_mlp_fx_scal_doubles(d), torch.float64).view(world, -1),
                "xws": z(max(int(lib.bhg_mlp_fx_ws_bytes(d, world)), 256), torch.uint8),
            }
        return got

    def _fx_phase(self, symbol: str, rhs, k: int, K: int, phase: int, world: int, rank: int, alpha: float, shift: float) -> None:
        b = self.fx_buffers(world)
        fws = self._fused_ws(self.buf.h[0].device)
        if phase == _native.BHG_CG_FX_BEGIN:
            self._solve = None
            self._fx_rhs = _native.ptr_array([t.data_ptr() for t in rhs]) + (list(rhs),)
        _native.check(
            getattr(self.lib, symbol)(ctypes.byref(self.desc), self._fx_rhs[0], int(k), int(K), int(phase), int(world), int(rank),
                                      b["const"].data_ptr(), b["slab"].data_ptr(), b["scal"].data_ptr(), float(alpha), float(shift),
                                      fws.data_ptr(), fws.numel(), b["xws"].data_ptr(), b["xws"].numel(), _stream()),
            symbol,
        )

    def cg_fx_phase(self, rhs, k: int, K: int, phase: int, world: int, rank: int, cg_alpha: float, shift: float) -> None:
        self._fx_phase("bhg_mlp_cg_fx_phase", rhs, k, K, phase, world, rank, cg_alpha, shift)

    def neumann_fx_phase(self, rhs, k: int, K: int, phase: int, world: int, rank: int, alpha: float, shift: float) -> None:
        self._fx_phase("bhg_mlp_neumann_fx_phase", rhs, k, K, phase, world, rank, alpha, shift)

    def neumann_fx_finish(self, layout, K: int, alpha: float) -> FusedSolve:
        self._solve = FusedSolve("neumann", float(alpha), int(K), layout, v_last=None, materialised=False, projected=1)
        return self._solve

    def cg_fx_finish(self, layout, K: int, cg_alpha: float) -> FusedSolve:
        self._solve = FusedSolve("cg", float(cg_alpha), int(K), layout, materialised=False)
        return self._solve

    def neumann_solve(self, layout, v0, v1, p, K: int, alpha: float, shift: float, keep_p: bool = True) -> FusedSolve:
        fws, starts = self._fused_args(layout)
        projected = ctypes.c_int(0)
        _native.check(
            self.lib.bhg_mlp_neumann_solve(ctypes.byref(self.desc), v0.data_ptr(), v1.data_ptr(), p.data_ptr() if keep_p else None,
                                           starts, int(K), float(alpha), float(shift), fws.data_ptr(), fws.numel(), ctypes.byref(projected),
                                           _stream()),
            "bhg_mlp_neumann_solve",
        )
        self._solve = FusedSolve("neumann", float(alpha), int(K), layout, v_last=v0 if K % 2 == 0 else v1, materialised=keep_p)
        self._solve.projected = int(projected.value)
        return self._solve

    def mixed_coeff(self, dir_views, solve: FusedSolve = None):
        buf = self.buf
        if solve is not None and solve is not getattr(self, "_solve", None):
            raise RuntimeError("stale fused-solve token: another solve or a hand-driven HVP has reused this state's workspace")
        if solve is not None and solve.kind == "neumann" and not solve.materialised:
            lay, v_last = solve.layout, solve.v_last
            if v_last is None:
                tab, _keep = None, None
            else:
                views = [v_last[s: s + n] for s, n in zip(lay.starts, lay.numels)]
                tab, _keep = self._dir_table(views)
            _native.check(
                self.lib.bhg_mlp_neumann_mixed_coeff(ctypes.byref(self.desc), tab, buf.labels.data_ptr(), buf.coeff.data_ptr(),
                                                     solve.alpha, solve.K, int(getattr(solve, "projected", 0)), buf.fws.data_ptr(),
                                                     buf.fws.numel(), _stream()),
                "bhg_mlp_neumann_mixed_coeff",
            )
        elif solve is not None and solve.kind == "cg":
            _native.check(
                self.lib.bhg_mlp_cg_mixed_coeff(ctypes.byref(self.desc), buf.labels.data_ptr(), buf.coeff.data_ptr(), solve.alpha,
                                                buf.fws.data_ptr(), buf.fws.numel(), _stream()),
                "bhg_mlp_cg_mixed_coeff",
            )
        else:
            tab, _keep = self._dir_table(dir_views)
            _native.check(
                self.lib.bhg_mlp_mixed_coeff(ctypes.byref(self.desc), tab, buf.labels.data_ptr(), buf.coeff.data_ptr(), _stream()),
                "bhg_mlp_mixed_coeff",
            )
        coeff = buf.coeff[:self.B]
        return coeff if self.native_upper else coeff.clone()


PAD_WIDTHS_TO_32 = True
_TWINS = weakref.WeakKeyDictionary()


def _pad32(n: int) -> int:
    return (int(n) + 31) // 32 * 32


def padded_dims(dims):
    return tuple(_pad32(d) for d in dims[:-1]) + (int(dims[-1]),)


class _TwinLayer:

    __slots__ = ("weight", "bias", "__weakref__")

    def __init__(self, out_f, in_f, device):
        self.weight = torch.zeros(out_f, in_f, dtype=torch.float32, device=device)
        self.bias = torch.zeros(out_f, dtype=torch.float32, device=device)


class _Twin:
    def __init__(self, dims, pdims, device):
        self.layers = [_TwinLayer(pdims[l + 1], pdims[l], device) for l in range(len(dims) - 1)]
        self.x = None
        self.dirs = [t for lay in self.layers for t in (torch.zeros_like(lay.weight), torch.zeros_like(lay.bias))]
        self.rhs = [torch.zeros_like(t) for t in self.dirs]


def _copy2d(lib, dst, ldd, src, lds, rows, cols):
    _native.check(lib.bhg_copy2d(dst.data_ptr(), int(ldd), src.data_ptr(), int(lds), int(rows), int(cols), _stream()), "bhg_copy2d")


class _TwinSpec:

    def __init__(self, spec, twin):
        self._spec, self.layers = spec, twin.layers

    def __getattr__(self, name):
        return getattr(self._spec, name)


class PaddedHipMLPState:

    solution_free = True

    def __init__(self, spec, x, y):
        if not x.is_cuda:
            raise _native.NativeLibraryError("WeightedCEMLP(impl='hip') needs CUDA/HIP tensors; there is no CPU fallback")
        self.lib = lib = _native.load()
        self.spec = spec
        real = [lin for lin in spec.layers]
        self.real_Ws = [lin.weight.detach() for lin in real]
        self.real_bs = [lin.bias.detach() for lin in real]
        for t in self.real_Ws + self.real_bs:
            if t.dtype != torch.float32 or not t.is_contiguous():
                raise ValueError("weights and biases must be contiguous fp32 tensors")
        dims = tuple([self.real_Ws[0].shape[1]] + [W.shape[0] for W in self.real_Ws])
        self.dims, self.pdims = dims, padded_dims(dims)
        self.shapes = [s for W in self.real_Ws for s in ((W.shape[0], W.shape[1]), (1, W.shape[0]))]
        self.pcols = [c for l in range(len(dims) - 1) for c in (self.pdims[l], self.pdims[l + 1])]
        owner = _TWINS.setdefault(spec.layers[0], {})
        key = (self.pdims, str(x.device))
        twin = owner.get(key)
        if twin is None:
            twin = owner[key] = _Twin(dims, self.pdims, x.device)
        self.twin = twin
        for l, (W, b) in enumerate(zip(self.real_Ws, self.real_bs)):
            _copy2d(lib, twin.layers[l].weight, self.pdims[l], W, dims[l], W.shape[0], W.shape[1])
            _copy2d(lib, twin.layers[l].bias, self.pdims[l + 1], b, dims[l + 1], 1, b.shape[0])
        B = x.shape[0]
        xs = x.detach().reshape(B, -1)
        xs = xs if (xs.dtype == torch.float32 and xs.is_contiguous()) else xs.to(torch.float32).contiguous()
        if twin.x is None or twin.x.shape[0] != B:
            twin.x = torch.zeros(B, self.pdims[0], dtype=torch.float32, device=x.device)
        _copy2d(lib, twin.x, self.pdims[0], xs, dims[0], B, dims[0])
        self.inner = HipMLPState(_TwinSpec(spec, twin), twin.x, y)
        self.B = B
        self.out = None

    @property
    def native_upper(self):
        return self.inner.native_upper

    @property
    def sample_weight(self):
        return self.inner.sample_weight

    def upper_vjp(self, *a, **k):
        return self.inner.upper_vjp(*a, **k)

    def _pad(self, tensors, into):
        for t, dst, (rows, cols), ldd in zip(tensors, into, self.shapes, self.pcols):
            if not (t.is_cuda and t.dtype == torch.float32 and t.is_contiguous()):
                t = t.detach().to(torch.float32).contiguous()
            _copy2d(self.lib, dst, ldd, t, cols, rows, cols)
        return into

    def _unpad(self, padded, into):
        for src, t, (rows, cols), lds in zip(padded, into, self.shapes, self.pcols):
            _copy2d(self.lib, t, cols, src, lds, rows, cols)
        return into

    def _real_views(self, layout, flat):
        like = [t for W, b in zip(self.real_Ws, self.real_bs) for t in (W, b)]
        return layout.views(flat, like)

    def _twin_layout(self):
        from ..backend import get_backend

        return get_backend().layout(self.twin.dirs)

    def hvp(self, direction_views):
        out_p = self.inner.hvp(self._pad(direction_views, self.twin.dirs))
        if self.out is None:
            self.out = [torch.empty_like(t) for W, b in zip(self.real_Ws, self.real_bs) for t in (W, b)]
        return self._unpad(out_p, self.out)

    def fused_supported(self, layout) -> bool:
        want = [n for W in self.real_Ws for n in (W.numel(), W.shape[0])]
        return (tuple(want) == tuple(layout.numels) and str(layout.device) == str(self.real_Ws[0].device)
                and self.inner.fused_supported(self._twin_layout()))

    def cg_solve(self, layout, x, r, p, K: int, cg_alpha: float, shift: float, keep_x: bool = True, rhs=None) -> FusedSolve:
        from ..backend import get_backend

        be, play = get_backend(), self._twin_layout()
        self._pad(self._real_views(layout, r), self.twin.rhs)
        px, pr, pp = play.state(3)
        skip_x = not keep_x
        mask = self.inner.cg_state_mask() if skip_x else None
        ts = be.cg_init(play, self.twin.rhs, None if skip_x else px, pr, pp, keep_mask=mask) if mask is not None else \
            be.cg_init(play, self.twin.rhs, None if skip_x else px, pr, pp)
        token = self.inner.cg_solve(play, px, pr, pp, K, cg_alpha, shift, keep_x=keep_x, rhs=ts if mask is not None else None)
        if keep_x:
            self._unpad(play.views(px, self.twin.dirs), self._real_views(layout, x))
        return token

    def neumann_solve(self, layout, v0, v1, p, K: int, alpha: float, shift: float, keep_p: bool = True) -> FusedSolve:
        from ..backend import get_backend

        be, play = get_backend(), self._twin_layout()
        self._pad(self._real_views(layout, v0), self.twin.rhs)
        pv0, pv1, pp = play.state(3)
        be.neumann_init(play, self.twin.rhs, pv0, pp if keep_p else None)
        token = self.inner.neumann_solve(play, pv0, pv1, pp, K, alpha, shift, keep_p=keep_p)
        self._twin_p = (token, play, pp) if keep_p else None
        if keep_p:
            self._unpad(play.views(pp, self.twin.dirs), self._real_views(layout, p))
        return token

    def mixed_coeff(self, dir_views, solve: FusedSolve = None):
        if solve is not None:
            held = getattr(self, "_twin_p", None)
            if solve.kind == "neumann" and solve.materialised and held is not None and held[0] is solve:
                return self.inner.mixed_coeff(held[1].views(held[2], self.twin.dirs), solve)
            return self.inner.mixed_coeff(None, solve)
        return self.inner.mixed_coeff(self._pad(dir_views, self.twin.dirs))


def make_state(spec, x, y):
    Ws = [lin.weight for lin in spec.layers]
    dims = tuple([Ws[0].shape[1]] + [W.shape[0] for W in Ws])
    if (PAD_WIDTHS_TO_32 and spec.pad_widths and len(Ws) >= 3 and dims[-1] <= 256 and padded_dims(dims) != dims and x.is_cuda):
        return PaddedHipMLPState(spec, x, y)
    return HipMLPState(spec, x, y)


_FD_WS = weakref.WeakKeyDictionary()


def fd_hop(spec, vector, eps32, two_eps, x, y, upper, sync: bool, restore: bool):
    lib = _native.load()
    params = [t for lin in spec.layers for t in (lin.weight, lin.bias)]
    L, B = len(spec.layers), int(x.shape[0])
    dims = [spec.layers[0].weight.shape[1]] + [lin.weight.shape[0] for lin in spec.layers]
    dims_c = (ctypes.c_int * len(dims))(*dims)
    dev = params[0].device
    xs = x.detach().reshape(B, -1)
    xs = xs if (xs.dtype == torch.float32 and xs.is_contiguous()) else xs.to(torch.float32).contiguous()
    ys = y.detach().reshape(-1).to(device=dev, dtype=torch.int64).contiguous()
    dirs = [v if (v.dtype == torch.float32 and v.is_contiguous()) else v.detach().to(torch.float32).contiguous() for v in vector]
    owner = _FD_WS.setdefault(spec.layers[0], {})
    key = (tuple(dims), B, str(dev))
    ws = owner.get(key)
    if ws is None:
        n = int(lib.bhg_mlp_fd_ws_bytes(dims_c, L, B))
        if n <= 0:
            raise _native.NativeLibraryError(f"bhg_mlp_fd_ws_bytes refused widths {dims} at batch {B}")
        ws = owner[key] = torch.empty(n, dtype=torch.uint8, device=dev)
    ce = torch.empty(2, B, dtype=torch.float32, device=dev)
    eps = eps32 if (eps32.dtype == torch.float32 and eps32.device == dev) else eps32.to(device=dev, dtype=torch.float32)
    ptab, _pk = _native.ptr_array([p.data.data_ptr() for p in params])
    dtab, _dk = _native.ptr_array([d.data_ptr() for d in dirs])
    _native.check(lib.bhg_mlp_fd_forward(xs.data_ptr(), ys.data_ptr(), B, dims_c, L, ptab, dtab, eps.data_ptr(), int(restore),
                                         ce[0].data_ptr(), ce[1].data_ptr(), ws.data_ptr(), ws.numel(), _stream()), "bhg_mlp_fd_forward")
    native = _native_weight_net(lib, spec.weight_net, upper, dev)
    if native is None:
        return spec.fd_upper_autograd(ce[0], ce[1], two_eps, upper, sync)
    ts, slots = native
    if sync:
        for p in upper:
            if p.grad is None:
                p.grad = torch.zeros_like(p, memory_format=torch.contiguous_format)
            elif not (p.grad.dtype == torch.float32 and p.grad.is_contiguous()):
                p.grad = p.grad.to(torch.float32).contiguous()
        outs = [p.grad for p in upper]
        g = [outs[i] for i in slots]
    else:
        _flat, outs, g = _flat_upper(upper, slots, dev)
    _native.check(lib.bhg_mwn_fd_vjp(ce[0].data_ptr(), ce[1].data_ptr(), B, ts[0].data_ptr(), ts[1].data_ptr(), ts[2].data_ptr(),
                                     ts[3].data_ptr(), ts[0].shape[0], two_eps.data_ptr(), int(sync), g[0].data_ptr(), g[1].data_ptr(),
                                     g[2].data_ptr(), g[3].data_ptr(), _stream()), "bhg_mwn_fd_vjp")
    return None if sync else outs
```

betty_amd/hypergradient/structured.py:

```python
from __future__ import annotations

from typing import Callable, List, Optional, Sequence

import math
import warnings

import torch
import torch.nn.functional as F

from ._common import _uses_ddp, is_fsdp, precision_of


class StructureMismatchError(RuntimeError):
    """The declared closed form does not describe the problem's actual ``training_step``."""


VERIFY_STRUCTURE = True
VERIFY_RTOL = 1e-3
VERIFY_KINK_MARGIN = 1e-6
VERIFY_RTOL_ON_A_KINK = 3e-2
VERIFY_KINK_RETRIES = 3


AUTO_STRUCTURE = False
# ... 116 lines not shown
        self.curr, self.prev = curr, prev
        self.weight_net = weight_net
        self.verify = bool(verify)
        self.layers = list(layers)
        self.weight_fn = weight_fn
        self.ridge = float(ridge)
        self.hvp_shift = 2.0 * self.ridge
        self.batch = batch
        self.impl = impl
        self.fused = bool(fused)
        self.keep_solution = bool(keep_solution)
        self.pad_widths, self.expects_data_parallel_mean = True, False
        params = list(curr.parameters())
        expect = []
        for lin in self.layers:
            expect += [lin.weight, lin.bias]
        if len(params) != len(expect) or any(a is not b for a, b in zip(params, expect)):
            raise ValueError("WeightedCEMLP: curr.parameters() must be [W1, b1, W2, b2, ...] of `layers`")

    def prepare(self):
        x, y = self.batch if self.batch is not None else self.curr.cur_batch
        impl = self.impl or "hip"
        if impl == "hip":
            from ._mlp_hip import make_state

            self._state = make_state(self, x, y)
        elif impl == "torch":
            from ._mlp_torch import _TorchMLPState

            self._state = _TorchMLPState(self, x, y)
        else:
            raise ValueError(f"unknown impl {impl!r}")
        if self.verify and VERIFY_STRUCTURE:
            self._verify_against_autograd(x, y)
        return self._state.hvp

    def _autograd_second_order(self, params, upper):
        gen = torch.Generator(device="cpu").manual_seed(20240926)
        direction = [torch.randn(p.shape, generator=gen).to(device=p.device, dtype=p.dtype) for p in params]
        devs = [params[0].device] if params and params[0].is_cuda else []
        with torch.random.fork_rng(devices=devs), torch.enable_grad():
            loss = self.curr.training_step_exec(self.batch if self.batch is not None else self.curr.cur_batch)
            grads = torch.autograd.grad(loss, params, create_graph=True)
            dot = sum((g * d).sum() for g, d in zip(grads, direction))
            second = torch.autograd.grad(dot, params + upper, allow_unused=True)
        return direction, second[:len(params)], second[len(params):]

    def _estimate_ridge(self) -> float:
        params = list(self.curr.parameters())
        direction, hv_auto, _ = self._autograd_second_order(params, list(self.prev.trainable_parameters()))
        hv0 = [h.detach().clone() for h in self._state.hvp(direction)]
        num = sum(float(((a.double() - b.double()) * d.double()).sum()) for a, b, d in zip(hv_auto, hv0, direction))
        den = sum(float((d.double() ** 2).sum()) for d in direction)
        c = num / den
        res = sum(float(((a.double() - b.double() - c * d.double()) ** 2).sum()) for a, b, d in zip(hv_auto, hv0, direction)) ** 0.5
        ref = sum(float((a.double() ** 2).sum()) for a in hv_auto) ** 0.5
        if c <= 0.0 or res > VERIFY_RTOL * max(ref, 1e-300) or c * den ** 0.5 <= 1e-5 * ref:
            return 0.0
        rho = 0.5 * c
        for digits in range(1, 7):
            r = round(rho, digits)
            if r > 0 and abs(r - rho) <= 2e-4 * rho:
                return float(r)
        return float(rho)

    def _verify_against_autograd(self, x, y):
        params = list(self.curr.parameters())
        key = (tuple(tuple(p.shape) for p in params), int(x.shape[0]), self.ridge, type(self._state).__name__)
        done = self.curr.__dict__.setdefault("_bhg_structure_verified", set()) if hasattr(self.curr, "__dict__") else set()
        if key in done:
            return
        upper = list(self.prev.trainable_parameters())
        direction, hv_auto, mixed_auto = self._autograd_second_order(params, upper)
        hv = [h.detach().clone() + self.hvp_shift * d for h, d in zip(self._state.hvp(direction), direction)]
        coeff = self._state.mixed_coeff(direction)
        mixed = self._state.upper_vjp(coeff, upper, retain_graph=True)
        mixed = [torch.zeros_like(p) if g is None else g for g, p in zip(mixed, upper)]

        def rel(got, want):
            num = sum(float(((a.double() - (b.double() if b is not None else 0.0)) ** 2).sum()) for a, b in zip(got, want)) ** 0.5
            den = sum(float((b.double() ** 2).sum()) for b in want if b is not None) ** 0.5
            return num / den if den > 0 else num

        e_hvp, e_mix = rel(hv, hv_auto), rel(mixed, mixed_auto)
        tol, relaxed = VERIFY_RTOL, False
        if precision_of(self.curr) in ("fp16", "bf16"):
            tol = max(tol, 5e-2)
        if not (e_hvp <= tol and e_mix <= tol):
            with torch.no_grad():
                h, margin = x.detach().reshape(x.shape[0], -1).to(self.layers[0].weight.dtype), float("inf")
                for lin in self.layers[:-1]:
                    a = torch.addmm(lin.bias, h, lin.weight.t())
                    margin = min(margin, float(a.abs().min() / a.abs().mean().clamp_min(1e-30)))
                    h = torch.relu(a)
            if margin < VERIFY_KINK_MARGIN:
                tol = VERIFY_RTOL_ON_A_KINK
                relaxed = True
        bad = not (e_hvp <= tol and e_mix <= tol)
        import torch.distributed as dist

        if dist.is_available() and dist.is_initialized() and dist.get_world_size() > 1:
            flag = torch.tensor([1.0 if bad else 0.0, 1.0 if relaxed else 0.0], device=params[0].device if dist.get_backend() == "nccl" else "cpu")
            dist.all_reduce(flag, op=dist.ReduceOp.MAX)
            bad, relaxed = bool(flag[0].item() > 0), bool(flag[1].item() > 0)
        if bad:
            raise StructureMismatchError(
                f"hypergradient_structure of problem {getattr(self.curr, 'name', '?')!r} declares {type(self).__name__}, but its "
                f"training_step disagrees with that closed form on a random direction: Hessian-vector product off by {e_hvp:.2e}, "
                f"mixed second derivative by {e_mix:.2e} (tolerance {tol:g}).  Typical causes: label smoothing, dropout, a "
                f"reduction other than the batch mean, a ridge that is not `ridge * sum(w^2)`, layers missing from `layers`.")
        if relaxed:
            tries = self.curr.__dict__.setdefault("_bhg_structure_relaxed", {}) if hasattr(self.curr, "__dict__") else {}
            tries[key] = tries.get(key, 0) + 1
            final = tries[key] >= VERIFY_KINK_RETRIES
            if tries[key] == 1 or final:
                warnings.warn(
                    f"betty_amd: structure check of problem {getattr(self.curr, 'name', '?')!r} passed only under the ReLU-kink tolerance "
                    f"({tol:g}; Hessian-vector product off by {e_hvp:.2e}, mixed second derivative by {e_mix:.2e}: some hidden "
                    "pre-activation of this batch sits within 1e-6 of zero) — " +
                    (f"accepted after {tries[key]} such batches" if final else "not cached, the next batch is checked again"),
                    RuntimeWarning, stacklevel=3)
            if not final:
                return
        done.add(key)

    def _fused_ready(self, K: int, layout, *methods: str, world: Optional[int] = None, skips_solution: bool = False) -> bool:
        st = self._state
        if not (K > 0 and self.fused) or (skips_solution and self.keep_solution):
            return False
        for m in methods:
            if not hasattr(st, m):
                return False
        return bool(st.fused_supported(layout) if world is None else st.fx_supported(layout, world))

    def fused_cg_ready(self, layout, K: int) -> bool:
        return self._fused_ready(K, layout, "cg_solve")

    def fused_cg_skips_solution(self, layout, K: int) -> bool:
        return self._fused_ready(K, layout, "cg_solve", skips_solution=True)

    def fused_cg_state_mask(self, layout, K: int):
        if not self._fused_ready(K, layout, "cg_solve", "cg_state_mask", skips_solution=True):
            return None
        return self._state.cg_state_mask()

    def fused_cg(self, layout, x, r, p, K: int, cg_alpha: float, rhs=None):
        if not self.fused_cg_ready(layout, K):
            return False
        return self._state.cg_solve(layout, x, r, p, K, cg_alpha, self.hvp_shift, keep_x=self.keep_solution, rhs=rhs)

    def fused_cg_global_ready(self, layout, K: int) -> bool:
        return self._fused_ready(K, layout, "cg_global_phase")

    def fused_cg_global_skips_solution(self, layout, K: int) -> bool:
        return self._fused_ready(K, layout, "cg_global_phase", skips_solution=True) and self._state.solution_free

    def cg_global_phase(self, layout, x, r, p, k: int, K: int, phase: int, world: int, php, cg_alpha: float) -> None:
        keep = not self.fused_cg_global_skips_solution(layout, K)
        self._state.cg_global_phase(layout, x, r, p, k, K, phase, world, php, cg_alpha, self.hvp_shift, keep_x=keep)

    def cg_global_finish(self, layout, K: int, cg_alpha: float):
        keep = not self.fused_cg_global_skips_solution(layout, K)
        return self._state.cg_global_finish(layout, K, cg_alpha, keep_x=keep)

    def fused_cg_fx_ready(self, layout, K: int, world: int) -> bool:
        return self._fused_ready(K, layout, "cg_fx_phase", world=world, skips_solution=True)

    def fused_neumann_fx_ready(self, layout, K: int, world: int) -> bool:
        return self._fused_ready(K, layout, "neumann_fx_phase", world=world, skips_solution=True)

    def fx_buffers(self, world: int):
        return self._state.fx_buffers(world)

    def local_batch_size(self) -> int:
        return self._state.B

    def _fx(self, method: str, *args):
        return getattr(self._state, method)(*args)

    def cg_fx_phase(self, rhs, k: int, K: int, phase: int, world: int, rank: int, cg_alpha: float) -> None:
        self._fx("cg_fx_phase", rhs, k, K, phase, world, rank, cg_alpha, self.hvp_shift)

    def cg_fx_finish(self, layout, K: int, cg_alpha: float):
        return self._fx("cg_fx_finish", layout, K, cg_alpha)

    def neumann_fx_phase(self, rhs, k: int, K: int, phase: int, world: int, rank: int, alpha: float) -> None:
        self._fx("neumann_fx_phase", rhs, k, K, phase, world, rank, alpha, self.hvp_shift)

    def neumann_fx_finish(self, layout, K: int, alpha: float):
        return self._fx("neumann_fx_finish", layout, K, alpha)

    def fused_neumann_ready(self, layout, K: int) -> bool:
        return self._fused_ready(K, layout, "neumann_solve")

    def fused_neumann_skips_solution(self, layout, K: int) -> bool:
        return self._fused_ready(K, layout, "neumann_solve", skips_solution=True)

    def fused_neumann(self, layout, v, p, K: int, alpha: float):
        if not self.fused_neumann_ready(layout, K):
            return False
        v_alt = next(t for t in layout.state(3) if t is not v and t is not p)
        return self._state.neumann_solve(layout, v, v_alt, p, K, alpha, self.hvp_shift, keep_p=self.keep_solution)

    def _fd_applies(self, layout, vector):
        curr, prev = self.curr, self.prev
        if is_fsdp(curr):
            return "fsdp"
        if precision_of(curr) != "fp32":
            return "autocast"
        params = list(curr.parameters())
        if (why := _fd_parameters_blocker(curr, params, layout, vector)) is not None:
            return why
        if _uses_ddp(prev):
            return "ddp"
        import torch.distributed as dist

        if dist.is_available() and dist.is_initialized() and dist.get_world_size() > 1:
            return "multi-rank"
        wn = self.weight_net
        if wn is not None and (wn.average_over is not None or wn.slots(list(prev.trainable_parameters())) is None):
            return "upper parameters"
        x, y = self.batch if self.batch is not None else curr.cur_batch
        if not (torch.is_tensor(x) and torch.is_tensor(y)):
            return "batch"
        tensors = params + list(vector) + [x]
        if (self.impl or "hip") == "hip":
            if not all(t.is_cuda and t.dtype == torch.float32 and t.device == params[0].device for t in tensors):
                return "not fp32 cuda"
            if not all(p.is_contiguous() for p in params) or not (1 <= x.shape[0] <= 512):
                return "shape"
        elif not all(t.dtype == torch.float32 for t in tensors):
            return "not fp32"
        return None

    def _fd_guard(self, x):
        if not (self.verify and VERIFY_STRUCTURE):
            return
        params = list(self.curr.parameters())
        head = (tuple(tuple(p.shape) for p in params), int(x.shape[0]), self.ridge)
        done = self.curr.__dict__.get("_bhg_structure_verified", set()) if hasattr(self.curr, "__dict__") else set()
        if any(k[:3] == head for k in done):
            return
        self.prepare()

    def finite_difference(self, layout, vector, eps32, eps64, sync: bool, restore: bool = True):
        vector = list(vector)
        if self._fd_applies(layout, vector) is not None:
            return NotImplemented
        x, y = self.batch if self.batch is not None else self.curr.cur_batch
        self._fd_guard(x)
        two_eps = (2.0 * eps64).to(torch.float32)
        upper = list(self.prev.trainable_parameters())
        if (self.impl or "hip") == "hip":
            from ._mlp_hip import fd_hop

            return fd_hop(self, vector, eps32, two_eps, x, y, upper, bool(sync), bool(restore))
        from ..backend import get_backend

        be = get_backend()
        weights = [p.data for p in self.curr.parameters()]
        with torch.no_grad():
            be.axpy_multi(layout, weights, vector, eps32, 1.0)
            ce_p = self._torch_ce(x, y)
            be.axpy_multi(layout, weights, vector, eps32, -2.0)
            ce_m = self._torch_ce(x, y)
            if restore:
                be.axpy_multi(layout, weights, vector, eps32, 1.0)
        return self.fd_upper_autograd(ce_p, ce_m, two_eps, upper, bool(sync))

    def _torch_ce(self, x, y):
        h = x.detach().reshape(x.shape[0], -1)
        for l, lin in enumerate(self.layers):
            h = F.linear(h, lin.weight.detach(), lin.bias.detach())
            if l + 1 < len(self.layers):
                h = torch.relu(h)
        return F.cross_entropy(h, y.reshape(-1), reduction="none")

    def fd_upper_autograd(self, ce_p, ce_m, two_eps, upper, sync: bool):
        B = ce_p.shape[0]

        def point(ce, scale=None):
            ce = ce.detach().clone()
            with torch.enable_grad():
                s = self.weight_fn(ce)
            seed = torch.full((), 1.0, dtype=ce.dtype, device=ce.device) if scale is None else 1.0 / scale
            return s, ((seed / B) * ce).reshape(s.shape)

        def zero_fill(gs):
            return [torch.zeros_like(p) if g is None else g for g, p in zip(gs, upper)]

        s_p, c_p = point(ce_p)
        g_p = zero_fill(torch.autograd.grad(s_p, upper, grad_outputs=c_p, allow_unused=True))
        if sync:
            self.prev.set_grads(upper, [-(g / two_eps) for g in g_p])
            s_m, c_m = point(ce_m, two_eps)
            torch.autograd.backward(s_m, grad_tensors=c_m, inputs=upper)
            return None
        s_m, c_m = point(ce_m)
        g_m = zero_fill(torch.autograd.grad(s_m, upper, grad_outputs=c_m, allow_unused=True))
        return [(gn - gp) / two_eps for gn, gp in zip(g_m, g_p)]

    def mixed_vjp(self, neg_x_views, sync: bool, solve=None):
        st = self._state
        coeff = st.mixed_coeff(neg_x_views, solve) if solve is not None else st.mixed_coeff(neg_x_views)
        upper = self.prev.trainable_parameters()
        if st.native_upper:
            wn = self.weight_net
            world, group = 1, None
            if sync:
                import torch.distributed as dist

                if dist.is_available() and dist.is_initialized():
                    from ..distributed import ddp_process_group_of

                    if wn.average_over is not None:
                        group = None if wn.average_over is True else wn.average_over
                        world = dist.get_world_size(group)
                    else:
                        wrapped, group = ddp_process_group_of(getattr(self.prev, "fwd", None), getattr(self.prev, "module", None))
                        if wrapped:
                            world = dist.get_world_size(group)
                        elif dist.get_world_size() > 1 and self.expects_data_parallel_mean:
                            raise RuntimeError(
                                "cg_global(sync=True) with a closed-form weight net: declare SigmoidMLPWeightNet(average_over=True) (or a "
                                "process group) or wrap the upper module in DistributedDataParallel — otherwise every rank would "
                                "accumulate the hypergradient of its own batch share only")
            grads, flat = st.upper_vjp(coeff, upper, scale=1.0 / world, with_flat=True)
            if sync:
                from ..distributed import defer_grad_sync, fence_grads, install_optimizer_fence

                fence_grads()
            if world > 1:
                if wn.overlap and sync:
                    if all(p_.grad is None for p_ in upper):
                        work = dist.all_reduce(flat, op=dist.ReduceOp.SUM, group=group, async_op=True)
                        from ..backend import get_backend

                        defer_grad_sync(work, flat, get_backend())
                        install_optimizer_fence(getattr(self.prev, "optimizer", None))
                    else:
                        dist.all_reduce(flat, op=dist.ReduceOp.SUM, group=group)
                else:
                    dist.all_reduce(flat, op=dist.ReduceOp.SUM, group=group)
            if sync:
                for p_, g_ in zip(upper, grads):
                    p_.grad = g_ if p_.grad is None else p_.grad + g_
                return None
            return grads
        if sync:
            torch.autograd.backward(st.sample_weight, grad_tensors=coeff.reshape(st.sample_weight.shape), inputs=upper)
            return None
        return list(torch.autograd.grad(st.sample_weight, upper, grad_outputs=coeff.reshape(st.sample_weight.shape)))


def _fd_parameters_blocker(curr, params, layout, vector):
    meta = list(curr.meta_trainable_parameters()) if hasattr(curr, "meta_trainable_parameters") else params
    if len(meta) != len(params) or any(a is not b for a, b in zip(meta, params)) or len(vector) != len(params):
        return "parameters"
    if tuple(layout.numels) != tuple(p.numel() for p in params) or any(v.shape != p.shape for v, p in zip(vector, params)):
        return "layout"
    return None


def _forward_has_side_effects(module) -> bool:
    for m in module.modules():
        if not m.training:
            continue
        if isinstance(m, torch.nn.modules.dropout._DropoutNd) or next(m.buffers(recurse=False), None) is not None:
            return True
    return False


def _graph_leaves(t) -> set:
    if t.grad_fn is None:
        return {id(t)} if t.requires_grad else set()
    seen, stack, leaves = set(), [t.grad_fn], set()
    while stack:
        fn = stack.pop()
        if fn is None or fn in seen:
            continue
        seen.add(fn)
        var = getattr(fn, "variable", None)
        if var is not None:
            leaves.add(id(var))
        stack.extend(nxt for nxt, _ in fn.next_functions)
    return leaves


class _QuadraticFD:

    impl: Optional[str] = None
    closed_form_fd: Optional[bool] = None
    _fd_side_effects: Optional[bool] = None

    def _quad_fd_blocker(self, layout, vector):
        curr, prev = self.curr, self.prev
        if self.closed_form_fd is False:
            return "declined"
        if is_fsdp(curr) or is_fsdp(prev):
            return "fsdp"
        if precision_of(curr) != "fp32" or torch.is_autocast_enabled("cuda") or torch.is_autocast_enabled("cpu"):
            return "autocast"
        params = list(curr.parameters())
        if not params:
            return "parameters"
        if (why := _fd_parameters_blocker(curr, params, layout, vector)) is not None:
            return why
        hip = (self.impl or "hip") == "hip"
        for t in [p.data for p in params] + list(vector):
            if t.dtype != torch.float32 or t.device != params[0].device or not t.is_contiguous():
                return "not contiguous fp32"
            if hip and not (t.is_cuda and t.data_ptr() % 16 == 0):
                return "not an aligned cuda tensor"
        if self.closed_form_fd is None:
            if self._fd_side_effects is None:
                module = getattr(curr, "module", None)
                self._fd_side_effects = not isinstance(module, torch.nn.Module) or _forward_has_side_effects(module)
            if self._fd_side_effects:
                return "the forward passes have side effects"
        return None

    def _quad_fd_launch(self, layout, vector, out, eps32, scale: float, mode: int, restore: bool, accumulate: bool):
        from ..backend import get_backend

        be = get_backend()
        weights = [p.data for p in self.curr.parameters()]
        if (self.impl or "hip") == "hip":
            be.quad_fd(layout, weights, vector, out, eps32, scale, mode, restore, accumulate)
            return
        if self.impl != "torch":
            raise ValueError(f"unknown impl {self.impl!r}")
        with torch.no_grad():
            res = [float(scale) * v for v in vector] if mode == 0 else [-(w * v) for w, v in zip(weights, vector)]
            be.axpy_multi(layout, weights, vector, eps32, 1.0)
            be.axpy_multi(layout, weights, vector, eps32, -2.0)
            if restore:
                be.axpy_multi(layout, weights, vector, eps32, 1.0)
            for o, r in zip(out, res):
                o.add_(r) if accumulate else o.copy_(r)


class LogisticRegressionL2(_QuadraticFD):

    def __init__(self, curr, prev, weight: torch.nn.Parameter, lam_fn: Callable, batch=None, impl: Optional[str] = None,
                 closed_form_fd: Optional[bool] = None):
        self.curr, self.prev, self.weight, self.lam_fn, self.batch = curr, prev, weight, lam_fn, batch
        self.impl, self.closed_form_fd = impl, closed_form_fd
        params = list(curr.parameters())
        if len(params) != 1 or params[0] is not weight:
            raise ValueError("LogisticRegressionL2: curr.parameters() must be [weight]")

    def prepare(self):
        from .. import _native

        x, _y = self.batch if self.batch is not None else self.curr.cur_batch
        if not x.is_cuda:
            raise _native.NativeLibraryError("LogisticRegressionL2 needs CUDA/HIP tensors; there is no CPU fallback")
        self.lib = _native.load()
        self.X = x.detach().to(torch.float32).contiguous()
        n, d = self.X.shape
        self.n, self.d = n, d
        self.lam = self.lam_fn()
        self.lam_d = self.lam.detach().to(torch.float32).contiguous()
        self.w = self.weight.detach().to(torch.float32).contiguous()
        self.s = torch.empty(n, device=x.device)
        self.tmp = torch.empty(int(self.lib.bhg_logreg_tmp_floats(n, d)), device=x.device)
        self.out = torch.empty(d, device=x.device)
        self._stream = lambda: int(torch.cuda.current_stream().cuda_stream)
        _native.check(self.lib.bhg_logreg_prepare(self.X.data_ptr(), self.w.data_ptr(), self.s.data_ptr(), n, d, self._stream()),
                      "bhg_logreg_prepare")
        self._native = _native
        return self.hvp

    def hvp(self, direction_views):
        (p,) = direction_views
        p = p.detach().to(torch.float32).contiguous()
        self._native.check(
            self.lib.bhg_logreg_hvp(self.X.data_ptr(), self.s.data_ptr(), self.lam_d.data_ptr(), p.data_ptr(),
                                    self.out.data_ptr(), self.tmp.data_ptr(), self.n, self.d, self._stream()),
            "bhg_logreg_hvp",
        )
        return [self.out.view(self.weight.shape)]

    def mixed_vjp(self, neg_x_views, sync: bool):
        coeff = (self.w * neg_x_views[0].reshape(-1)).reshape(self.lam.shape)
        upper = self.prev.trainable_parameters()
        if sync:
            torch.autograd.backward(self.lam, grad_tensors=coeff, inputs=upper)
            return None
        return list(torch.autograd.grad(self.lam, upper, grad_outputs=coeff))

    def finite_difference(self, layout, vector, eps32, eps64, sync: bool, restore: bool = True):
        vector = list(vector)
        if self._quad_fd_blocker(layout, vector) is not None:
            return NotImplemented
        upper = list(self.prev.trainable_parameters())
        lam = self.lam_fn()
        if not torch.is_tensor(lam) or lam.dtype != torch.float32 or lam.numel() != self.weight.numel() or lam.device != self.weight.device:
            return NotImplemented
        leaves = _graph_leaves(lam)
        if not upper or any(id(p) not in leaves for p in upper):
            return NotImplemented
        coeff = torch.empty_like(self.weight.data)
        self._quad_fd_launch(layout, vector, [coeff], eps32, 0.0, 1, bool(restore), False)
        coeff = coeff.reshape(lam.shape)
        if sync:
            torch.autograd.backward(lam, grad_tensors=coeff, inputs=upper)
            return None
        return list(torch.autograd.grad(lam, upper, grad_outputs=coeff))


class ProximalRegularized(_QuadraticFD):

    hvp_is_autograd = True

    def __init__(self, curr, prev, data_loss: Callable, reg: float, batch=None, impl: Optional[str] = None,
                 closed_form_fd: Optional[bool] = None):
        self.curr, self.prev, self.data_loss, self.reg, self.batch = curr, prev, data_loss, float(reg), batch
        self.impl, self.closed_form_fd = impl, closed_form_fd
        self.hvp_shift = 2.0 * self.reg
        inner, upper = list(curr.parameters()), list(prev.trainable_parameters())
        if len(inner) != len(upper) or any(a.shape != b.shape for a, b in zip(inner, upper)):
            raise ValueError("ProximalRegularized: upper and inner parameters must match one-to-one")

    def prepare(self):
        import warnings

        batch = self.batch if self.batch is not None else self.curr.cur_batch
        loss = self.data_loss(batch)
        with warnings.catch_warnings():
            warnings.simplefilter("ignore")
            self._in_grad = torch.autograd.grad(loss, self.curr.trainable_parameters(), create_graph=True)
        params = list(self.curr.parameters())

        def hvp(direction_views):
            return torch.autograd.grad(self._in_grad, params, grad_outputs=direction_views, retain_graph=True)

        return hvp

    def first_order_loss(self):
        return lambda: self.data_loss(self.batch if self.batch is not None else self.curr.cur_batch)

    def mixed_vjp(self, neg_x_views, sync: bool):
        self._in_grad = None
        grads = [(-2.0 * self.reg) * t for t in neg_x_views]
        if sync:
            torch.autograd.backward(list(self.prev.trainable_parameters()), grad_tensors=grads)
            return None
        return grads

    def finite_difference(self, layout, vector, eps32, eps64, sync: bool, restore: bool = True):
        vector = list(vector)
        if self._quad_fd_blocker(layout, vector) is not None:
            return NotImplemented
        upper = list(self.prev.trainable_parameters())
        if len(upper) != len(vector) or any(
                p.shape != v.shape or p.dtype != torch.float32 or p.device != v.device for p, v in zip(upper, vector)):
            return NotImplemented
        if not math.isfinite(self.reg):
            return NotImplemented
        scale = 2.0 * self.reg
        if sync:
            grads = [p.grad for p in upper]
            hip = (self.impl or "hip") == "hip"
            if not _uses_ddp(self.prev) and all(g is not None and g.dtype == torch.float32 and g.shape == p.shape and g.device == p.device
                               and g.is_contiguous() and (not hip or g.data_ptr() % 16 == 0) for g, p in zip(grads, upper)):
                self._quad_fd_launch(layout, vector, grads, eps32, scale, 0, bool(restore), True)
                return None
        out = layout.views(torch.empty(layout.flat_size, dtype=torch.float32, device=vector[0].device), vector)
        self._quad_fd_launch(layout, vector, out, eps32, scale, 0, bool(restore), False)
        if sync:
            torch.autograd.backward(upper, grad_tensors=out)
            return None
        return out
```

include/bhg.h:

```cpp
#ifndef BHG_H_
#define BHG_H_

#include <stddef.h>
#include <stdint.h>

#ifdef __cplusplus
extern "C" {
#endif

#define BHG_VERSION 1
#define BHG_CHUNK_ELEMS 4096
#define BHG_FLAT_ALIGN 64

#define BHG_OK 0
#define BHG_ERR_ARG (-1)
#define BHG_ERR_HIP (-2)
#define BHG_ERR_WS (-3)
#define BHG_ERR_CAPACITY (-4)

typedef struct bhg_chunk {
  int64_t flat_off;
  int64_t src_off;
  int32_t tensor;
  int32_t len;
} bhg_chunk;

int bhg_version(void);
const char* bhg_last_error(void);

int64_t bhg_layout_flat_size(const int64_t* numel, int T);
int64_t bhg_layout_num_chunks(const int64_t* numel, int T);
int bhg_layout_build(const int64_t* numel, int T, int64_t* starts, bhg_chunk* chunks);
size_t bhg_workspace_bytes(int T);

int bhg_flatten(const void* const* src, int T, const bhg_chunk* chunks_dev, int n_chunks,
                float* flat, float scale, void* ws, void* stream);
int bhg_scatter(const float* flat, void* const* dst, int T, const bhg_chunk* chunks_dev,
                int n_chunks, float scale, void* ws, void* stream);

int bhg_neumann_init(const void* const* vec, int T, const bhg_chunk* chunks_dev, int n_chunks,
                     float* v, float* p, void* ws, void* stream);
int bhg_neumann_step(const void* const* hvp, int T, const bhg_chunk* chunks_dev, int n_chunks,
                     float* v, float* p, float alpha, float out_scale, float hvp_shift, void* ws,
                     void* stream);

#define BHG_CG_AUTO 0
#define BHG_CG_STREAM 1
#define BHG_CG_RESIDENT 2
int bhg_cg_init(const void* const* vec, int T, const bhg_chunk* chunks_dev, int n_chunks,
                float* x, float* r, float* p, void* ws, void* stream);
int bhg_cg_init_masked(const void* const* vec, int T, const bhg_chunk* chunks_dev, int n_chunks,
                       float* x, float* r, float* p, unsigned long long keep_mask, void* ws, void* stream);
int bhg_cg_step(const void* const* hvp, int T, const bhg_chunk* chunks_dev, int n_chunks,
                float* x, float* r, float* p, float cg_alpha, int iter, float out_scale,
                float hvp_shift , int variant,
                void* ws, void* stream);
int bhg_cg_resident_capacity_chunks(void);
int bhg_cg_resident_ok(void);
int bhg_cg_resident_usable(int n_chunks);
const double* bhg_cg_scalars_dev(const void* ws);
const unsigned* bhg_cg_timeout_flag_dev(const void* ws);

int bhg_cg_phase(int phase, const void* const* hvp, int T, const bhg_chunk* chunks_dev, int n_chunks, float* x,
                 float* r, float* p, float cg_alpha, int iter, float out_scale, float hvp_shift, void* ws, void* stream);
double* bhg_cg_partials_dev(void* ws, int which, int iter);
int bhg_cg_partials_count(void);

int bhg_scale_flat(float* flat, int64_t n, float scale, void* stream);

int bhg_darts_eps(const void* const* vec, int T, const bhg_chunk* chunks_dev, int n_chunks,
                  double R, double* out_dev, float* eps_f32_dev, void* ws, void* stream);
int bhg_axpy_multi(void* const* dst, const void* const* src, int T, const bhg_chunk* chunks_dev,
                   int n_chunks, const float* coef_dev, float mul, void* ws, void* stream);

int bhg_fd_perturb(void* const* w, const float* w0_flat, const void* const* dir, int T, const bhg_chunk* chunks_dev,
                   int n_chunks, const float* eps_dev, float sign, void* ws, void* stream);
int bhg_cg_step_fd(const void* const* grad_plus, const void* const* grad_minus, const float* two_eps_dev, int T,
                   const bhg_chunk* chunks_dev, int n_chunks, float* x, float* r, float* p, float cg_alpha, int iter,
                   float out_scale, float hvp_shift, int variant, void* ws, void* stream);
int bhg_neumann_step_fd(const void* const* grad_plus, const void* const* grad_minus, const float* two_eps_dev, int T,
                        const bhg_chunk* chunks_dev, int n_chunks, float* v, float* p, float alpha, float out_scale,
                        float hvp_shift, void* ws, void* stream);

int bhg_sama_adam_precondition(const void* const* vec, const void* const* last_grad,
                               const void* const* exp_avg, const void* const* exp_avg_sq, int T,
                               const bhg_chunk* chunks_dev, int n_chunks, float* out_flat,
                               double beta1, double beta2, double eps, double lr, void* ws, void* stream);

int bhg_debug_set(const char* key, int value);
int bhg_debug_unset(const char* key);
void bhg_debug_reset(void);
int bhg_debug_key_count(void);
const char* bhg_debug_key_name(int i);
int bhg_is_ab_build(void);

#define BHG_TIMING_CG_STEP 0
#define BHG_TIMING_NEUMANN_STEP 1
#define BHG_TIMING_MLP_HVP 2
#define BHG_TIMING_MLP_CG_ITER 3
int bhg_timing_enable(int on);
int bhg_timing_read(int kind, double* total_ms, int* launches);

int bhg_logreg_prepare(const float* X, const float* w, float* s, int n, int d, void* stream);
size_t bhg_logreg_tmp_floats(int n, int d);
int bhg_logreg_hvp(const float* X, const float* s, const float* lam, const float* p, float* out,
                   float* tmp, int n, int d, void* stream);

#define BHG_MLP_MAX_LAYERS 32
typedef struct bhg_mlp {
  int32_t L, B, Bp;
  int32_t dims[BHG_MLP_MAX_LAYERS + 1];
  const float* W[BHG_MLP_MAX_LAYERS];
  const float* h[BHG_MLP_MAX_LAYERS];
  const float* mask[BHG_MLP_MAX_LAYERS];
  const float* delta[BHG_MLP_MAX_LAYERS];
  const float* prob;
  const float* sd;
  float* Rh[BHG_MLP_MAX_LAYERS];
  float* Rd[BHG_MLP_MAX_LAYERS];
  float* partial;
  size_t partial_floats;
  float ridge2;
  int32_t prepacked;
} bhg_mlp;
size_t bhg_mlp_partial_floats(const bhg_mlp* m);
int bhg_mlp_hvp(const bhg_mlp* m, const void* const* dir, void* const* out, void* stream);
int bhg_mlp_hvp_mode(const bhg_mlp* m, const void* const* dir, void* const* out, int gemm_mode, void* stream);

int bhg_mlp_supports_native_prepare(const bhg_mlp* m);
int bhg_mlp_forward(const bhg_mlp* m, const void* const* bias, const int64_t* labels, float* ce, void* stream);
int bhg_mlp_backward(const bhg_mlp* m, const int64_t* labels, void* stream);
int bhg_mlp_mixed_coeff(const bhg_mlp* m, const void* const* dir, const int64_t* labels, float* coeff, void* stream);

int bhg_mlp_supports_fused_solve(const bhg_mlp* m);
size_t bhg_mlp_fused_ws_bytes(const bhg_mlp* m);
int bhg_mlp_cg_solve(const bhg_mlp* m, float* x, float* r, float* p, const int64_t* starts,
                     const bhg_chunk* chunks_dev, int n_chunks, int K, float cg_alpha, float hvp_shift, void* ws,
                     void* fws, size_t fws_bytes, void* stream);
int bhg_mlp_neumann_solve(const bhg_mlp* m, float* v0, float* v1, float* p, const int64_t* starts, int K,
                          float alpha, float hvp_shift, void* fws, size_t fws_bytes, int* projected_out, void* stream);
#define BHG_CG_GLOBAL_CHAIN 0
#define BHG_CG_GLOBAL_UPDATE 1
#define BHG_CG_GLOBAL_DOTS 2
int bhg_mlp_cg_global_phase(const bhg_mlp* m, float* x, float* r, float* p, const int64_t* starts, const bhg_chunk* chunks_dev,
                            int n_chunks, int k, int K, int phase, int world, double* php, float cg_alpha, float hvp_shift,
                            void* ws, void* fws, size_t fws_bytes, void* stream);
#define BHG_CG_FX_BEGIN 0
#define BHG_CG_FX_CHAIN 1
#define BHG_CG_FX_GRAM 2
#define BHG_CG_FX_END 3
int bhg_mlp_fx_supported(const bhg_mlp* m, int world);
size_t bhg_mlp_fx_ws_bytes(const bhg_mlp* m, int world);
size_t bhg_mlp_fx_const_floats(const bhg_mlp* m);
size_t bhg_mlp_fx_slab_floats(const bhg_mlp* m);
size_t bhg_mlp_fx_scal_doubles(const bhg_mlp* m);
int bhg_mlp_cg_fx_phase(const bhg_mlp* m, const void* const* rhs, int k, int K, int phase, int world, int rank, float* const_all,
                        float* slab_all, double* scal_all, float cg_alpha, float hvp_shift, void* fws, size_t fws_bytes, void* xws,
                        size_t xws_bytes, void* stream);
int bhg_mlp_neumann_fx_phase(const bhg_mlp* m, const void* const* rhs, int k, int K, int phase, int world, int rank, float* const_all,
                             float* slab_all, double* scal_all, float alpha, float hvp_shift, void* fws, size_t fws_bytes, void* xws,
                             size_t xws_bytes, void* stream);
unsigned long long bhg_mlp_cg_state_mask(const bhg_mlp* m, int has_x);
int bhg_mlp_cg_solve_rhs(const bhg_mlp* m, float* x, float* r, float* p, const int64_t* starts, const bhg_chunk* chunks_dev,
                         int n_chunks, int K, float cg_alpha, float hvp_shift, void* ws, void* fws, size_t fws_bytes,
                         const void* const* rhs, void* stream);
int bhg_mlp_cg_mixed_coeff(const bhg_mlp* m, const int64_t* labels, float* coeff, float cg_alpha, void* fws,
                           size_t fws_bytes, void* stream);
int64_t bhg_mlp_wsk_launches(void);
int64_t bhg_mlp_hoist_launches(void);
int64_t bhg_mlp_proj_iterations(void);
int64_t bhg_mlp_lin_launches(void);
int bhg_mlp_neumann_mixed_coeff(const bhg_mlp* m, const void* const* v_last, const int64_t* labels, float* coeff,
                                float alpha, int K, int projected, void* fws, size_t fws_bytes, void* stream);

int bhg_mlp_stage_batch(const bhg_mlp* m, const float* x, const int64_t* y, int64_t* labels, void* stream);
int bhg_mlp_supports_packed_prepare(const bhg_mlp* m);
int bhg_mlp_forward_packed(const bhg_mlp* m, const void* const* bias, const int64_t* labels, float* ce, void* fws, size_t fws_bytes,
                           void* stream);
int bhg_mlp_backward_packed(const bhg_mlp* m, const int64_t* labels, void* fws, size_t fws_bytes, void* stream);

void* bhg_mlp_timeout_flag_dev(const bhg_mlp* m, void* fws);

int bhg_mwn_max_hidden(void);
int bhg_mwn_forward(const float* ce, int B, const float* w1, const float* b1, const float* w2, const float* b2, int H, float* s,
                    float* sd, void* stream);
int bhg_mwn_backward(const float* ce, const float* coeff, int B, const float* w1, const float* b1, const float* w2, const float* b2,
                     int H, float scale, float* gw1, float* gb1, float* gw2, float* gb2, void* stream);

int bhg_mlp_plan_describe(const bhg_mlp* m, int algo, int keep_solution, char* buf, size_t buf_bytes);

int bhg_copy2d(float* dst, int64_t ldd, const float* src, int64_t lds, int64_t rows, int64_t cols, void* stream);

size_t bhg_bn_ws_bytes(int C);
int bhg_bn_backward_vjp(const float* x, const float* gy, const float* a, const float* gamma, const float* mean, const float* invstd,
                        const float* b, const float* c, int N, int C, int HW, float* dx, float* dgy, float* dgamma, void* ws,
                        size_t ws_bytes, void* stream);

size_t bhg_mlp_fd_ws_bytes(const int* dims, int L, int B);
int bhg_mlp_fd_forward(const float* x, const int64_t* labels, int B, const int* dims, int L, void* const* params, const void* const* dir,
                       const float* eps_dev, int restore, float* ce_plus, float* ce_minus, void* ws, size_t ws_bytes, void* stream);
int bhg_mwn_fd_vjp(const float* ce_plus, const float* ce_minus, int B, const float* w1, const float* b1, const float* w2, const float* b2,
                   int H, const float* two_eps_dev, int accumulate, float* gw1, float* gb1, float* gw2, float* gb2, void* stream);

int bhg_quad_fd(void* const* w, const void* const* dir, void* const* out, int T, const bhg_chunk* chunks_dev, int n_chunks,
                const float* eps_dev, float scale, int mode, int restore, int accumulate, void* stream);

#ifdef __cplusplus
}
#endif
#endif
```

Before: 767.8.

## Fuse classifier head, meta-weight-net and first backward layer into one tail kernel

Adds a per-row tail kernel that computes head logits, softmax/CE, the closed-form meta-weight-net sample weight, the top delta and the first hidden-layer backward (with packed output), replacing several separate launches in the prepare step. Also fuses the CG mixed-coefficient computation into the MWN backward so the hypergradient hop uses one launch instead of two. The intent is to cut launch count and intermediate global round-trips per step. In exchange it adds a new code path with one block per row, which may use the GPU less efficiently than the old GEMM-style head kernels for wide features.

```diff
diff --git a/betty_amd/_native.py b/betty_amd/_native.py
--- a/betty_amd/_native.py
+++ b/betty_amd/_native.py
@@ -164,6 +164,18 @@
     "bhg_mlp_supports_packed_prepare": (c_int, [POINTER(Mlp)]),
     "bhg_mlp_forward_packed": (c_int, [POINTER(Mlp), _PP, c_void_p, c_void_p, c_void_p, c_size_t, c_void_p]),
     "bhg_mlp_backward_packed": (c_int, [POINTER(Mlp), c_void_p, c_void_p, c_size_t, c_void_p]),
+    "bhg_mlp_supports_fused_tail": (c_int, [POINTER(Mlp)]),
+    "bhg_mlp_forward_packed_hidden": (c_int, [POINTER(Mlp), _PP, c_void_p, c_size_t, c_void_p]),
+    "bhg_mlp_tail_packed": (
+        c_int,
+        [POINTER(Mlp), c_void_p, c_void_p, c_void_p, c_void_p, c_void_p, c_void_p, c_void_p, c_int, c_void_p, c_size_t, c_void_p],
+    ),
+    "bhg_mlp_backward_packed_hidden": (c_int, [POINTER(Mlp), c_void_p, c_size_t, c_void_p]),
+    "bhg_mlp_cg_mixed_mwn_backward": (
+        c_int,
+        [POINTER(Mlp), c_void_p, c_void_p, c_float, c_void_p, c_size_t, c_void_p, c_void_p, c_void_p, c_void_p, c_void_p, c_int, c_float,
+         c_void_p, c_void_p, c_void_p, c_void_p, c_void_p],
+    ),
     "bhg_mwn_max_hidden": (c_int, []),
     "bhg_mlp_fd_ws_bytes": (c_size_t, [POINTER(c_int), c_int, c_int]),
     "bhg_mlp_fd_forward": (
diff --git a/betty_amd/csrc/bhg_common.hpp b/betty_amd/csrc/bhg_common.hpp
--- a/betty_amd/csrc/bhg_common.hpp
+++ b/betty_amd/csrc/bhg_common.hpp
@@ -36,7 +36,7 @@
   X(mlp_hoist) X(hoist_wgs) X(proj_step_alone) X(mlp_no_side) X(mlp_no_fuse) X(mlp_no_outer_all) X(neumann_side)             \
   X(hoist_staged_mink) X(proj_alpha_alone) X(proj_small_alone) X(outer_order_by_work) X(outer_no_pre) X(outer_stagger)       \
   X(mlp_no_fused_solve) X(cg_eager_p) X(cg_x_every_iter) X(neumann_p_every_iter) X(head_no_prefetch) X(cg_spin_limit)        \
-  X(packed_chain) X(packed_depth) X(packed_gram) X(proj_max_ratio) X(proj_ws_cap_mb) X(alpha_in_hoist) X(graw_v2) X(wskp_ragged) X(pstep_v2) X(pstep_unroll) X(rnew_in_graw) X(graw_cols) X(lin_first) X(lin_prio) X(lin_nub) X(lin_order) X(lin_update_next) X(lin_withhold_beta) X(neumann_vnew) X(cg_rhs_direct) X(packed_prepare) X(lin_deep) X(graw_kloop) X(lin_update_in_head) X(xcd_pairs) X(headu_head_first) X(fx_ksplit)
+  X(packed_chain) X(packed_depth) X(packed_gram) X(proj_max_ratio) X(proj_ws_cap_mb) X(alpha_in_hoist) X(graw_v2) X(wskp_ragged) X(pstep_v2) X(pstep_unroll) X(rnew_in_graw) X(graw_cols) X(lin_first) X(lin_prio) X(lin_nub) X(lin_order) X(lin_update_next) X(lin_withhold_beta) X(neumann_vnew) X(cg_rhs_direct) X(packed_prepare) X(lin_deep) X(graw_kloop) X(lin_update_in_head) X(xcd_pairs) X(headu_head_first) X(fx_ksplit) X(fused_tail)
 enum DbgKey : int {
 #define BHG_DBG_ENUM(n) DBG_##n,
   BHG_DBG_KEYS(BHG_DBG_ENUM)
diff --git a/betty_amd/csrc/bhg_mlp.hip b/betty_amd/csrc/bhg_mlp.hip
--- a/betty_amd/csrc/bhg_mlp.hip
+++ b/betty_amd/csrc/bhg_mlp.hip
@@ -3,6 +3,7 @@
 
 
 #include "bhg_common.hpp"
+#include "bhg_tail.hpp"
 
 #ifdef BHG_STAMPS
 namespace bhg { __device__ unsigned long long* d_stamps = nullptr; }
@@ -1874,6 +1875,20 @@
   return BHG_OK;
 }
 
+int bhg_mlp_cg_mixed_mwn_backward(const bhg_mlp* m, const int64_t* labels, float* coeff, float cg_alpha, void* fws, size_t fws_bytes,
+                                  const float* ce, const float* w1, const float* b1, const float* w2, const float* b2, int H,
+                                  float scale, float* gw1, float* gb1, float* gw2, float* gb2, void* stream) {
+  if (int rc = check_mlp(m)) return rc;
+  BHG_REQUIRE(labels && coeff && fws, "NULL argument");
+  BHG_REQUIRE(fws_bytes >= bhg_mlp_fused_ws_bytes(m), "fused workspace too small");
+  FusedWs w;
+  carve_fused_ws(m, fws, &w);
+  MwnRzx q{};
+  q.rzx = w.rzx; q.prob = m->prob; q.labels = labels; q.coeff_out = coeff;
+  q.C = m->dims[m->L]; q.rows = m->Bp; q.scale = -cg_alpha;
+  return launch_mwn_backward_rzx(ce, q, m->B, w1, b1, w2, b2, H, scale, gw1, gb1, gw2, gb2, static_cast<hipStream_t>(stream));
+}
+
 static int check_head_problem(const bhg_mlp* m) {
   BHG_REQUIRE(m, "NULL descriptor");
   BHG_REQUIRE(m->L >= 1 && m->L <= BHG_MLP_MAX_LAYERS, "unsupported layer count");
@@ -2004,17 +2019,21 @@
   return hp.ok && dbg(DBG_packed_chain, 1) != 0 ? 1 : 0;
 }
 
-int bhg_mlp_forward_packed(const bhg_mlp* m, const void* const* bias, const int64_t* labels, float* ce, void* fws, size_t fws_bytes,
-                           void* stream) {
+int bhg_mlp_supports_fused_tail(const bhg_mlp* m) {
+  return bhg_mlp_supports_packed_prepare(m) && dbg(DBG_fused_tail, 1) != 0 ? 1 : 0;
+}
+
+}
+static int packed_checks(const bhg_mlp* m, const void* fws, size_t fws_bytes) {
   if (int rc = check_head_problem(m)) return rc;
   BHG_REQUIRE(narrow_head(m), "the packed once-per-step passes need a narrow classifier head (<= 256 classes, feature width % 4 == 0)");
-  BHG_REQUIRE(bias && labels && ce && fws, "NULL argument");
+  BHG_REQUIRE(fws, "NULL argument");
   BHG_REQUIRE(bhg_mlp_supports_packed_prepare(m), "this network does not take the packed form (bhg_mlp_supports_packed_prepare)");
   BHG_REQUIRE(fws_bytes >= bhg_mlp_fused_ws_bytes(m), "fused workspace too small");
-  hipStream_t st = static_cast<hipStream_t>(stream);
+  return BHG_OK;
+}
+static int forward_packed_hidden(const bhg_mlp* m, const void* const* bias, const FusedWs& w, hipStream_t st) {
   const int L = m->L, Bp = m->Bp, B = m->B;
-  FusedWs w;
-  carve_fused_ws(m, fws, &w);
   if (int rc = pack_operands(m, w, st, true)) return rc;
   {
     const int K = m->dims[0], N = m->dims[1];
@@ -2041,6 +2060,19 @@
     const int blk = q.nfull * (q.RB / 32) + q.nstrip;
     hipLaunchKernelGGL(k_wskpf<2>, dim3(blk), dim3(64 * kWskpWaves), 0, st, f);
   }
+  return BHG_OK;
+}
+extern "C" {
+
+int bhg_mlp_forward_packed(const bhg_mlp* m, const void* const* bias, const int64_t* labels, float* ce, void* fws, size_t fws_bytes,
+                           void* stream) {
+  if (int rc = packed_checks(m, fws, fws_bytes)) return rc;
+  BHG_REQUIRE(bias && labels && ce, "NULL argument");
+  hipStream_t st = static_cast<hipStream_t>(stream);
+  const int L = m->L, Bp = m->Bp, B = m->B;
+  FusedWs w;
+  carve_fused_ws(m, fws, &w);
+  if (int rc = forward_packed_hidden(m, bias, w, st)) return rc;
   launch_head_forward(st, Bp, nullptr, m->h[L - 1], m->W[L - 1] , m->W[L - 1], static_cast<const float*>(bias[L - 1]),
                       nullptr, nullptr, const_cast<float*>(m->prob), m->dims[L - 1], m->dims[L], B, HEAD_LOGITS, labels, ce, nullptr,
                       nullptr, nullptr);
@@ -2048,12 +2080,59 @@
   return BHG_OK;
 }
 
+}
+static void backward_packed_hidden(const bhg_mlp* m, const FusedWs& w, hipStream_t st) {
+  const int L = m->L, Bp = m->Bp, B = m->B;
+  for (int l = L - 2; l >= 1; --l) {
+    WskpBuilder wb;
+    WskpProb q{};
+    q.Ap = w.dpk[l]; q.Bq = w.Wb[l]; q.RA = Bp; q.RB = m->dims[l]; q.K = m->dims[l + 1]; q.B = B; q.nsplit = 1;
+    q.mask = m->mask[l - 1]; q.out = const_cast<float*>(m->delta[l - 1]);
+    q.outp = l >= 2 ? w.dpk[l - 1] : nullptr;
+    wb.add(q);
+    wb.launch(st);
+  }
+}
+extern "C" {
+
+int bhg_mlp_forward_packed_hidden(const bhg_mlp* m, const void* const* bias, void* fws, size_t fws_bytes, void* stream) {
+  if (int rc = packed_checks(m, fws, fws_bytes)) return rc;
+  BHG_REQUIRE(bias, "NULL argument");
+  FusedWs w;
+  carve_fused_ws(m, fws, &w);
+  if (int rc = forward_packed_hidden(m, bias, w, static_cast<hipStream_t>(stream))) return rc;
+  BHG_HIP_CHECK(hipGetLastError());
+  return BHG_OK;
+}
+
+int bhg_mlp_tail_packed(const bhg_mlp* m, const float* head_bias, const int64_t* labels, float* ce, const float* w1, const float* b1,
+                        const float* w2, const float* b2, int H, void* fws, size_t fws_bytes, void* stream) {
+  if (int rc = packed_checks(m, fws, fws_bytes)) return rc;
+  BHG_REQUIRE(head_bias && labels && ce, "NULL argument");
+  const int L = m->L;
+  FusedWs w;
+  carve_fused_ws(m, fws, &w);
+  TailArgs a{};
+  a.h = m->h[L - 1]; a.W = m->W[L - 1]; a.bias = head_bias; a.labels = labels; a.mask = m->mask[L - 2];
+  a.w1 = w1; a.b1 = b1; a.w2 = w2; a.b2 = b2; a.H = H;
+  a.prob = const_cast<float*>(m->prob); a.ce = ce; a.sd = const_cast<float*>(m->sd);
+  a.dtop = const_cast<float*>(m->delta[L - 1]); a.dprev = const_cast<float*>(m->delta[L - 2]); a.dprev_p = w.dpk[L - 2];
+  a.K = m->dims[L - 1]; a.C = m->dims[L]; a.B = m->B; a.rows = m->Bp;
+  return launch_mlp_tail(a, static_cast<hipStream_t>(stream));
+}
+
+int bhg_mlp_backward_packed_hidden(const bhg_mlp* m, void* fws, size_t fws_bytes, void* stream) {
+  if (int rc = packed_checks(m, fws, fws_bytes)) return rc;
+  FusedWs w;
+  carve_fused_ws(m, fws, &w);
+  backward_packed_hidden(m, w, static_cast<hipStream_t>(stream));
+  BHG_HIP_CHECK(hipGetLastError());
+  return BHG_OK;
+}
+
 int bhg_mlp_backward_packed(const bhg_mlp* m, const int64_t* labels, void* fws, size_t fws_bytes, void* stream) {
-  if (int rc = check_head_problem(m)) return rc;
-  BHG_REQUIRE(narrow_head(m), "the packed once-per-step passes need a narrow classifier head (<= 256 classes, feature width % 4 == 0)");
-  BHG_REQUIRE(labels && fws, "NULL argument");
-  BHG_REQUIRE(bhg_mlp_supports_packed_prepare(m), "this network does not take the packed form (bhg_mlp_supports_packed_prepare)");
-  BHG_REQUIRE(fws_bytes >= bhg_mlp_fused_ws_bytes(m), "fused workspace too small");
+  if (int rc = packed_checks(m, fws, fws_bytes)) return rc;
+  BHG_REQUIRE(labels, "NULL argument");
   hipStream_t st = static_cast<hipStream_t>(stream);
   const int L = m->L, Bp = m->Bp, B = m->B;
   const int C = m->dims[L];
@@ -2067,15 +2146,7 @@
     hipLaunchKernelGGL(k_head_backward, dim3(blocks), dim3(256), 0, st, (const float*)nullptr, m->delta[l], m->W[l],
                        (const float*)nullptr, m->mask[l - 1], const_cast<float*>(m->delta[l - 1]), N, K, B, Bp, w.dpk[l - 1]);
   }
-  for (int l = L - 2; l >= 1; --l) {
-    WskpBuilder wb;
-    WskpProb q{};
-    q.Ap = w.dpk[l]; q.Bq = w.Wb[l]; q.RA = Bp; q.RB = m->dims[l]; q.K = m->dims[l + 1]; q.B = B; q.nsplit = 1;
-    q.mask = m->mask[l - 1]; q.out = const_cast<float*>(m->delta[l - 1]);
-    q.outp = l >= 2 ? w.dpk[l - 1] : nullptr;
-    wb.add(q);
-    wb.launch(st);
-  }
+  backward_packed_hidden(m, w, st);
   BHG_HIP_CHECK(hipGetLastError());
   return BHG_OK;
 }
diff --git a/betty_amd/csrc/bhg_mlp_tail.hip b/betty_amd/csrc/bhg_mlp_tail.hip
--- /dev/null
+++ b/betty_amd/csrc/bhg_mlp_tail.hip
@@ -0,0 +1,179 @@
+#include "bhg_tail.hpp"
+
+namespace bhg {
+namespace {
+
+__device__ __forceinline__ float4 ldg16(const float* p) { return *reinterpret_cast<const float4*>(p); }
+
+template <int JMAX>
+__global__ __launch_bounds__(256) void k_mlp_tail(TailArgs a) {
+  extern __shared__ __attribute__((aligned(16))) float dyn[];
+  __shared__ float rz[kTailMaxC], pr[kTailMaxC], ex[kTailMaxC], dl[kTailMaxC];
+  __shared__ float scal[4];
+  constexpr bool PRE = JMAX == 3;
+  const int b = blockIdx.x, t = threadIdx.x;
+  const int lane = t & 63, wave = t >> 6;
+  const int K = a.K, C = a.C, B = a.B, H = a.H;
+  if (b >= B) {
+    if (t < C) { a.prob[(int64_t)b * C + t] = 0.f; a.dtop[(int64_t)b * C + t] = 0.f; }
+    if (t == 0) a.ce[b] = 0.f;
+    for (int k = 4 * t; k < K; k += 1024) {
+      *reinterpret_cast<float4*>(a.dprev + (int64_t)b * K + k) = make_float4(0.f, 0.f, 0.f, 0.f);
+      *reinterpret_cast<float4*>(a.dprev_p + ((int64_t)(k >> 4) * a.rows + b) * 16 + (k & 15)) = make_float4(0.f, 0.f, 0.f, 0.f);
+    }
+    return;
+  }
+  const int j0 = t < H ? t : 0;
+  const float pw1 = a.w1[j0], pb1 = a.b1[j0], pw2 = a.w2[j0];
+  const float pb2 = a.b2[0];
+  const int y = (int)a.labels[b];
+  const int kd = 4 * t < K ? 4 * t : 0;
+  const float4 pf_mk = ldg16(a.mask + (int64_t)b * K + kd);
+  float4 pf_W[12];
+  if (PRE) {
+#pragma unroll
+    for (int c = 0; c < 12; ++c) pf_W[c] = ldg16(a.W + (int64_t)(c < C ? c : C - 1) * K + kd);
+  }
+  const float* hb = a.h + (int64_t)b * K;
+  for (int cbase = 0; cbase < C; cbase += 4 * JMAX) {
+    float acc[JMAX], cbv[JMAX];
+    const float* wrow[JMAX];
+#pragma unroll
+    for (int j = 0; j < JMAX; ++j) {
+      const int cc = min(cbase + wave + 4 * j, C - 1);
+      acc[j] = 0.f;
+      wrow[j] = a.W + (int64_t)cc * K;
+      cbv[j] = a.bias[cc];
+    }
+    for (int k = 4 * lane; k < K; k += 256) {
+      const float4 hv = ldg16(hb + k);
+      float4 vv[JMAX];
+#pragma unroll
+      for (int j = 0; j < JMAX; ++j) vv[j] = ldg16(wrow[j] + k);
+#pragma unroll
+      for (int j = 0; j < JMAX; ++j) {
+        float s = acc[j];
+        s = fmaf(hv.x, vv[j].x, s); s = fmaf(hv.y, vv[j].y, s); s = fmaf(hv.z, vv[j].z, s); s = fmaf(hv.w, vv[j].w, s);
+        acc[j] = s;
+      }
+    }
+#pragma unroll
+    for (int j = 0; j < JMAX; ++j) {
+      const int c = cbase + wave + 4 * j;
+      const float s = wave_sum_f32(acc[j]);
+      if (lane == 0 && c < C) rz[c] = s + cbv[j];
+    }
+  }
+  __syncthreads();
+  if (C > 32) {
+    if (t == 0) {
+      float mx = rz[0];
+      for (int c = 1; c < C; ++c) mx = fmaxf(mx, rz[c]);
+      scal[2] = mx;
+    }
+    __syncthreads();
+    if (t < C) ex[t] = expf(rz[t] - scal[2]);
+    __syncthreads();
+    if (t == 0) {
+      float sum = 0.f;
+      for (int c = 0; c < C; ++c) sum += ex[c];
+      scal[3] = scal[2] + logf(sum);
+    }
+    __syncthreads();
+    if (t < C) {
+      const float p = expf(rz[t] - scal[3]);
+      a.prob[(int64_t)b * C + t] = p;
+      pr[t] = p;
+    }
+    if (t == 0) {
+      const float cev = scal[3] - rz[y];
+      a.ce[b] = cev;
+      scal[0] = cev;
+    }
+  } else if (t == 0) {
+    float mx = rz[0];
+    for (int c = 1; c < C; ++c) mx = fmaxf(mx, rz[c]);
+    float sum = 0.f;
+    for (int c = 0; c < C; ++c) sum += expf(rz[c] - mx);
+    const float lse = mx + logf(sum);
+    for (int c = 0; c < C; ++c) {
+      const float p = expf(rz[c] - lse);
+      a.prob[(int64_t)b * C + c] = p;
+      pr[c] = p;
+    }
+    const float cev = lse - rz[y];
+    a.ce[b] = cev;
+    scal[0] = cev;
+  }
+  __syncthreads();
+  {
+    const float cev = scal[0];
+    float* sa = dyn;
+    float* sw = dyn + H;
+    for (int j = t; j < H; j += 256) {
+      const float w1v = j < 256 ? pw1 : a.w1[j], b1v = j < 256 ? pb1 : a.b1[j], w2v = j < 256 ? pw2 : a.w2[j];
+      const float u = fmaf(w1v, cev, b1v);
+      sa[j] = u > 0.f ? u : 0.f;
+      sw[j] = w2v;
+    }
+    __syncthreads();
+    if (t == 0) {
+      float z = pb2;
+      for (int j = 0; j < H; ++j) z = fmaf(sw[j], sa[j], z);
+      const float v = mwn_sigmoid(z);
+      const float sdv = v / (float)B;
+      a.sd[b] = sdv;
+      scal[1] = sdv;
+    }
+    __syncthreads();
+  }
+  if (t < C) {
+    const float d = scal[1] * (pr[t] - (y == t ? 1.f : 0.f));
+    a.dtop[(int64_t)b * C + t] = d;
+    dl[t] = d;
+  }
+  __syncthreads();
+  for (int k = 4 * t; k < K; k += 1024) {
+    const bool first = k == 4 * t;
+    float4 acc = make_float4(0.f, 0.f, 0.f, 0.f);
+    float4 m;
+    if (PRE && first) {
+#pragma unroll
+      for (int c = 0; c < 12; ++c) {
+        if (c < C) {
+          const float r = dl[c];
+          const float4 w = pf_W[c];
+          acc.x += r * w.x; acc.y += r * w.y; acc.z += r * w.z; acc.w += r * w.w;
+        }
+      }
+      m = pf_mk;
+    } else {
+      for (int c = 0; c < C; ++c) {
+        const float r = dl[c];
+        const float4 w = ldg16(a.W + (int64_t)c * K + k);
+        acc.x += r * w.x; acc.y += r * w.y; acc.z += r * w.z; acc.w += r * w.w;
+      }
+      m = first ? pf_mk : ldg16(a.mask + (int64_t)b * K + k);
+    }
+    acc.x *= m.x; acc.y *= m.y; acc.z *= m.z; acc.w *= m.w;
+    *reinterpret_cast<float4*>(a.dprev + (int64_t)b * K + k) = acc;
+    *reinterpret_cast<float4*>(a.dprev_p + ((int64_t)(k >> 4) * a.rows + b) * 16 + (k & 15)) = acc;
+  }
+}
+
+}
+
+int launch_mlp_tail(const TailArgs& a, hipStream_t st) {
+  BHG_REQUIRE(a.h && a.W && a.bias && a.labels && a.mask && a.w1 && a.b1 && a.w2 && a.b2, "NULL input");
+  BHG_REQUIRE(a.prob && a.ce && a.sd && a.dtop && a.dprev && a.dprev_p, "NULL output");
+  BHG_REQUIRE(a.C >= 1 && a.C <= kTailMaxC && a.K >= 16 && a.K % 16 == 0, "the tail takes <= 256 classes and a feature width % 16 == 0");
+  BHG_REQUIRE(a.B >= 1 && a.B <= a.rows, "bad batch");
+  BHG_REQUIRE(a.H >= 1 && a.H <= kMwnMaxH, "the closed-form meta-weight-net takes 1 <= hidden width <= 2048");
+  const size_t lds = sizeof(float) * 2 * (size_t)a.H;
+  if (a.C <= 12) hipLaunchKernelGGL(k_mlp_tail<3>, dim3(a.rows), dim3(256), lds, st, a);
+  else hipLaunchKernelGGL(k_mlp_tail<8>, dim3(a.rows), dim3(256), lds, st, a);
+  BHG_HIP_CHECK(hipGetLastError());
+  return BHG_OK;
+}
+
+}
diff --git a/betty_amd/csrc/bhg_mwn.hip b/betty_amd/csrc/bhg_mwn.hip
--- a/betty_amd/csrc/bhg_mwn.hip
+++ b/betty_amd/csrc/bhg_mwn.hip
@@ -1,12 +1,31 @@
-#include "bhg_common.hpp"
+#include "bhg_tail.hpp"
 
 namespace bhg {
 namespace {
 
-constexpr int kMwnMaxH = 2048;
 constexpr int kMwnChunk = 1024;
 
-__device__ __forceinline__ float mwn_sigmoid(float z) { return 1.f / (1.f + expf(-z)); }
+__device__ __forceinline__ float coeff_from_rzx(const MwnRzx& q, const int b, const int B) {
+  const int C = q.C;
+  const int y = (int)q.labels[b];
+  const float* __restrict__ pb = q.prob + (int64_t)b * C;
+  const double* __restrict__ rb = q.rzx + (int64_t)b * C;
+  double acc = 0.0;
+  for (int c0 = 0; c0 < C; c0 += 4) {
+    float p[4];
+    double r[4];
+#pragma unroll
+    for (int u = 0; u < 4; ++u) {
+      const int cc = c0 + u < C ? c0 + u : C - 1;
+      p[u] = pb[cc];
+      r[u] = rb[cc];
+    }
+#pragma unroll
+    for (int u = 0; u < 4; ++u)
+      if (c0 + u < C) acc += ((double)p[u] - (c0 + u == y ? 1.0 : 0.0)) * r[u];
+  }
+  return (float)((double)q.scale * acc / (double)B);
+}
 
 __global__ __launch_bounds__(kThreads) void k_mwn_forward(const float* __restrict__ ce, int B, const float* __restrict__ w1,
                                                           const float* __restrict__ b1, const float* __restrict__ w2,
@@ -28,11 +47,12 @@
   if (sd) sd[i] = v / (float)B;
 }
 
+template <bool RZX>
 __global__ __launch_bounds__(kThreads) void k_mwn_backward(const float* __restrict__ ce, const float* __restrict__ coeff, int B,
                                                            const float* __restrict__ w1, const float* __restrict__ b1,
                                                            const float* __restrict__ w2, const float* __restrict__ b2, int H,
                                                            float scale, float* __restrict__ gw1, float* __restrict__ gb1,
-                                                           float* __restrict__ gw2, float* __restrict__ gb2) {
+                                                           float* __restrict__ gw2, float* __restrict__ gb2, MwnRzx rq) {
   extern __shared__ float sp[];
   __shared__ float red[kWaves];
   float* sdz = sp + 3 * H;
@@ -50,8 +70,11 @@
   for (int u = 0; u < kSPer; ++u) {
     const int t = threadIdx.x + kThreads * u;
     c_pre[u] = ce[t < B ? t : 0];
-    k_pre[u] = coeff[t < B ? t : 0];
+    if (RZX) k_pre[u] = t < B ? coeff_from_rzx(rq, t, B) : 0.f;
+    else k_pre[u] = coeff[t < B ? t : 0];
   }
+  if (RZX)
+    for (int t = B + threadIdx.x; t < rq.rows; t += kThreads) rq.coeff_out[t] = 0.f;
   __syncthreads();
   for (int i0 = 0; i0 < B; i0 += kMwnChunk) {
     const int n = B - i0 < kMwnChunk ? B - i0 : kMwnChunk;
@@ -60,7 +83,8 @@
       const int t = threadIdx.x + kThreads * u;
       if (t >= n) continue;
       const float c = i0 == 0 ? c_pre[u] : ce[i0 + t];
-      const float kc = i0 == 0 ? k_pre[u] : coeff[i0 + t];
+      const float kc = i0 == 0 ? k_pre[u] : (RZX ? coeff_from_rzx(rq, i0 + t, B) : coeff[i0 + t]);
+      if (RZX) rq.coeff_out[i0 + t] = kc;
       float z = bias2;
       for (int j = 0; j < H; ++j) {
         const float a = fmaf(sp[j], c, sp[H + j]);
@@ -110,6 +134,18 @@
 }
 
 }
+
+int launch_mwn_backward_rzx(const float* ce, const MwnRzx& q, int B, const float* w1, const float* b1, const float* w2, const float* b2,
+                            int H, float scale, float* gw1, float* gb1, float* gw2, float* gb2, hipStream_t st) {
+  if (int rc = check_mwn(ce, B, w1, b1, w2, b2, H)) return rc;
+  BHG_REQUIRE(q.rzx && q.prob && q.labels && q.coeff_out && gw1 && gb1 && gw2 && gb2, "NULL argument");
+  BHG_REQUIRE(q.C >= 1 && q.rows >= B, "bad coefficient shape");
+  hipLaunchKernelGGL(k_mwn_backward<true>, dim3(1), dim3(kThreads), sizeof(float) * (3 * (size_t)H + 2 * kMwnChunk), st, ce,
+                     (const float*)nullptr, B, w1, b1, w2, b2, H, scale, gw1, gb1, gw2, gb2, q);
+  BHG_HIP_CHECK(hipGetLastError());
+  return BHG_OK;
+}
+
 }
 
 using namespace bhg;
@@ -132,8 +168,8 @@
                      int H, float scale, float* gw1, float* gb1, float* gw2, float* gb2, void* stream) {
   if (int rc = check_mwn(ce, B, w1, b1, w2, b2, H)) return rc;
   BHG_REQUIRE(coeff && gw1 && gb1 && gw2 && gb2, "NULL argument");
-  hipLaunchKernelGGL(k_mwn_backward, dim3(1), dim3(kThreads), sizeof(float) * (3 * (size_t)H + 2 * kMwnChunk),
-                     static_cast<hipStream_t>(stream), ce, coeff, B, w1, b1, w2, b2, H, scale, gw1, gb1, gw2, gb2);
+  hipLaunchKernelGGL(k_mwn_backward<false>, dim3(1), dim3(kThreads), sizeof(float) * (3 * (size_t)H + 2 * kMwnChunk),
+                     static_cast<hipStream_t>(stream), ce, coeff, B, w1, b1, w2, b2, H, scale, gw1, gb1, gw2, gb2, MwnRzx{});
   BHG_HIP_CHECK(hipGetLastError());
   return BHG_OK;
 }
diff --git a/betty_amd/csrc/bhg_tail.hpp b/betty_amd/csrc/bhg_tail.hpp
--- /dev/null
+++ b/betty_amd/csrc/bhg_tail.hpp
@@ -0,0 +1,37 @@
+#pragma once
+#include "bhg_common.hpp"
+
+namespace bhg {
+
+constexpr int kMwnMaxH = 2048;
+constexpr int kTailMaxC = 256;
+
+#ifdef __HIPCC__
+__device__ __forceinline__ float mwn_sigmoid(float z) { return 1.f / (1.f + expf(-z)); }
+#endif
+
+struct TailArgs {
+  const float* h;
+  const float* W;
+  const float* bias;
+  const int64_t* labels;
+  const float* mask;
+  const float* w1; const float* b1; const float* w2; const float* b2; int H;
+  float* prob;
+  float* ce;
+  float* sd;
+  float* dtop;
+  float* dprev;
+  float* dprev_p;
+  int K, C, B, rows;
+};
+int launch_mlp_tail(const TailArgs& a, hipStream_t st);
+
+struct MwnRzx {
+  const double* rzx; const float* prob; const int64_t* labels; float* coeff_out;
+  int C, rows; float scale;
+};
+int launch_mwn_backward_rzx(const float* ce, const MwnRzx& q, int B, const float* w1, const float* b1, const float* w2, const float* b2,
+                            int H, float scale, float* gw1, float* gb1, float* gw2, float* gb2, hipStream_t st);
+
+}
diff --git a/betty_amd/hypergradient/_mlp_hip.py b/betty_amd/hypergradient/_mlp_hip.py
--- a/betty_amd/hypergradient/_mlp_hip.py
+++ b/betty_amd/hypergradient/_mlp_hip.py
@@ -79,11 +79,12 @@
 
 class FusedSolve:
 
-    __slots__ = ("kind", "alpha", "K", "layout", "v_last", "materialised", "projected")
+    __slots__ = ("kind", "alpha", "K", "layout", "v_last", "materialised", "projected", "single_call")
 
     def __init__(self, kind, alpha, K, layout, v_last=None, materialised=True, projected=0):
         self.kind, self.alpha, self.K, self.layout, self.v_last, self.materialised = kind, alpha, K, layout, v_last, materialised
         self.projected = projected
+        self.single_call = False
 
     def __bool__(self):
         return True
@@ -132,6 +133,33 @@
 
         d.prepacked = 0
         self.packed_prepare = bool(buf.native_prepare and lib.bhg_mlp_supports_packed_prepare(ctypes.byref(d)))
+        native = _native_weight_net(lib, spec.weight_net, spec.prev.trainable_parameters(), x.device)
+        self.native_upper, self.sample_weight = native is not None, None
+        if self.native_upper:
+            self._wn, self._upper_slots = native
+        self.fused_tail = bool(self.packed_prepare and self.native_upper and lib.bhg_mlp_supports_fused_tail(ctypes.byref(d)))
+        if self.fused_tail:
+            fws, ts = self._fused_ws(x.device), self._wn
+            bias_tab, self._bias_keep = _native.ptr_array([b.data_ptr() for b in bs])
+            _native.check(lib.bhg_mlp_forward_packed_hidden(ctypes.byref(d), bias_tab, fws.data_ptr(), fws.numel(), _stream()),
+                          "bhg_mlp_forward_packed_hidden")
+            _native.check(lib.bhg_mlp_tail_packed(ctypes.byref(d), bs[-1].data_ptr(), buf.labels.data_ptr(), buf.ce.data_ptr(),
+                                                  ts[0].data_ptr(), ts[1].data_ptr(), ts[2].data_ptr(), ts[3].data_ptr(), ts[0].shape[0],
+                                                  fws.data_ptr(), fws.numel(), _stream()), "bhg_mlp_tail_packed")
+            _native.check(lib.bhg_mlp_backward_packed_hidden(ctypes.byref(d), fws.data_ptr(), fws.numel(), _stream()),
+                          "bhg_mlp_backward_packed_hidden")
+            d.prepacked = 1
+        else:
+            self._prepare_by_passes(lib, spec, buf, d, bs, x, B)
+        if buf.out is None:
+            buf.out = []
+            for lin in spec.layers:
+                buf.out += [torch.empty_like(lin.weight), torch.empty_like(lin.bias)]
+            buf.out_tab, buf.out_keep = _native.ptr_array([t.data_ptr() for t in buf.out])
+        self.out = buf.out
+        self._out_tab = buf.out_tab
+
+    def _prepare_by_passes(self, lib, spec, buf, d, bs, x, B):
         if self.packed_prepare:
             fws = self._fused_ws(x.device)
             bias_tab, self._bias_keep = _native.ptr_array([b.data_ptr() for b in bs])
@@ -145,10 +173,7 @@
             ce = buf.ce[:B]
         else:
             raise _native.NativeLibraryError("bhg_mlp_supports_native_prepare refused this network (layer count / batch padding): there is no ATen path")
-        native = _native_weight_net(lib, spec.weight_net, spec.prev.trainable_parameters(), x.device)
-        self.native_upper, self.sample_weight = native is not None, None
         if self.native_upper:
-            self._wn, self._upper_slots = native
             ts = self._wn
             _native.check(lib.bhg_mwn_forward(buf.ce.data_ptr(), B, ts[0].data_ptr(), ts[1].data_ptr(), ts[2].data_ptr(), ts[3].data_ptr(),
                                               ts[0].shape[0], None, buf.sd.data_ptr(), _stream()), "bhg_mwn_forward")
@@ -161,13 +186,6 @@
             d.prepacked = 1
         else:
             _native.check(lib.bhg_mlp_backward(ctypes.byref(d), buf.labels.data_ptr(), _stream()), "bhg_mlp_backward")
-        if buf.out is None:
-            buf.out = []
-            for lin in spec.layers:
-                buf.out += [torch.empty_like(lin.weight), torch.empty_like(lin.bias)]
-            buf.out_tab, buf.out_keep = _native.ptr_array([t.data_ptr() for t in buf.out])
-        self.out = buf.out
-        self._out_tab = buf.out_tab
 
     def upper_vjp(self, coeff, upper, scale: float = 1.0, retain_graph: bool = False, with_flat: bool = False):
         if not self.native_upper:
@@ -184,6 +202,22 @@
                                       g[3].data_ptr(), _stream()), "bhg_mwn_backward")
         return (views, flat) if with_flat else views
 
+    def fused_hop(self, solve) -> bool:
+        return bool(solve is not None and solve.kind == "cg" and solve.single_call and self.native_upper and self.fused_tail)
+
+    def mixed_upper_vjp(self, solve, upper, scale: float = 1.0, with_flat: bool = False):
+        if solve is not getattr(self, "_solve", None):
+            raise RuntimeError("stale fused-solve token: another solve or a hand-driven HVP has reused this state's workspace")
+        buf, ts = self.buf, self._wn
+        flat, views, g = _flat_upper(upper, self._upper_slots, ts[0].device)
+        _native.check(
+            self.lib.bhg_mlp_cg_mixed_mwn_backward(ctypes.byref(self.desc), buf.labels.data_ptr(), buf.coeff.data_ptr(), solve.alpha,
+                                                   buf.fws.data_ptr(), buf.fws.numel(), buf.ce.data_ptr(), ts[0].data_ptr(),
+                                                   ts[1].data_ptr(), ts[2].data_ptr(), ts[3].data_ptr(), ts[0].shape[0], float(scale),
+                                                   g[0].data_ptr(), g[1].data_ptr(), g[2].data_ptr(), g[3].data_ptr(), _stream()),
+            "bhg_mlp_cg_mixed_mwn_backward")
+        return (views, flat) if with_flat else views
+
     @staticmethod
     def _dir_table(direction_views):
         dirs = []
@@ -248,6 +282,7 @@
         )
         self._rhs_keep = (rhs, _rhs_keep)
         self._solve = FusedSolve("cg", float(cg_alpha), int(K), layout, materialised=keep_x)
+        self._solve.single_call = True
         return self._solve
 
     solution_free = True
@@ -452,6 +487,12 @@
 
     def upper_vjp(self, *a, **k):
         return self.inner.upper_vjp(*a, **k)
+
+    def fused_hop(self, solve) -> bool:
+        return self.inner.fused_hop(solve)
+
+    def mixed_upper_vjp(self, *a, **k):
+        return self.inner.mixed_upper_vjp(*a, **k)
 
     def _pad(self, tensors, into):
         for t, dst, (rows, cols), ldd in zip(tensors, into, self.shapes, self.pcols):
diff --git a/betty_amd/hypergradient/structured.py b/betty_amd/hypergradient/structured.py
--- a/betty_amd/hypergradient/structured.py
+++ b/betty_amd/hypergradient/structured.py
@@ -442,7 +442,9 @@
 
     def mixed_vjp(self, neg_x_views, sync: bool, solve=None):
         st = self._state
-        coeff = st.mixed_coeff(neg_x_views, solve) if solve is not None else st.mixed_coeff(neg_x_views)
+        one_launch = solve is not None and getattr(st, "fused_hop", None) is not None and st.fused_hop(solve)
+        if not one_launch:
+            coeff = st.mixed_coeff(neg_x_views, solve) if solve is not None else st.mixed_coeff(neg_x_views)
         upper = self.prev.trainable_parameters()
         if st.native_upper:
             wn = self.weight_net
@@ -465,7 +467,10 @@
                                 "cg_global(sync=True) with a closed-form weight net: declare SigmoidMLPWeightNet(average_over=True) (or a "
                                 "process group) or wrap the upper module in DistributedDataParallel — otherwise every rank would "
                                 "accumulate the hypergradient of its own batch share only")
-            grads, flat = st.upper_vjp(coeff, upper, scale=1.0 / world, with_flat=True)
+            if one_launch:
+                grads, flat = st.mixed_upper_vjp(solve, upper, scale=1.0 / world, with_flat=True)
+            else:
+                grads, flat = st.upper_vjp(coeff, upper, scale=1.0 / world, with_flat=True)
             if sync:
                 from ..distributed import defer_grad_sync, fence_grads, install_optimizer_fence
 
diff --git a/include/bhg.h b/include/bhg.h
--- a/include/bhg.h
+++ b/include/bhg.h
@@ -179,6 +179,12 @@
                            void* stream);
 int bhg_mlp_backward_packed(const bhg_mlp* m, const int64_t* labels, void* fws, size_t fws_bytes, void* stream);
 
+int bhg_mlp_supports_fused_tail(const bhg_mlp* m);
+int bhg_mlp_forward_packed_hidden(const bhg_mlp* m, const void* const* bias, void* fws, size_t fws_bytes, void* stream);
+int bhg_mlp_tail_packed(const bhg_mlp* m, const float* head_bias, const int64_t* labels, float* ce, const float* w1, const float* b1,
+                        const float* w2, const float* b2, int H, void* fws, size_t fws_bytes, void* stream);
+int bhg_mlp_backward_packed_hidden(const bhg_mlp* m, void* fws, size_t fws_bytes, void* stream);
+
 void* bhg_mlp_timeout_flag_dev(const bhg_mlp* m, void* fws);
 
 int bhg_mwn_max_hidden(void);
@@ -186,6 +192,9 @@
                     float* sd, void* stream);
 int bhg_mwn_backward(const float* ce, const float* coeff, int B, const float* w1, const float* b1, const float* w2, const float* b2,
                      int H, float scale, float* gw1, float* gb1, float* gw2, float* gb2, void* stream);
+int bhg_mlp_cg_mixed_mwn_backward(const bhg_mlp* m, const int64_t* labels, float* coeff, float cg_alpha, void* fws, size_t fws_bytes,
+                                  const float* ce, const float* w1, const float* b1, const float* w2, const float* b2, int H,
+                                  float scale, float* gw1, float* gb1, float* gw2, float* gb2, void* stream);
 
 int bhg_mlp_plan_describe(const bhg_mlp* m, int algo, int keep_solution, char* buf, size_t buf_bytes);
 
```

Result: no change. 773.5, median of 6 (+0.7%).
